# Infinidat/slimfastq

Measured on AMD Instinct MI355X. Metric: MB/s FASTQ compressed, higher is better.
Workload: dtype u8/u32 integer; 1 GPU; synthetic 10M x 150 bp Illumina reads per GPU, full qlts+gens+recs, frozen tables (one chain per lane), -l 3; level=3, block_reads=1024, prior_step=-1, blocks_per_gpu=9766, tables=frozen, chains_per_gpu=253906, raw_bytes_per_gpu=3702038404, parallelism=1 GPU

## Files before the change

slimfastq_amd/csrc/api.cpp:

```cpp
#include <hip/hip_runtime.h>

#include <algorithm>
#include <cstdarg>
#include <cstdlib>
#include <cstdio>
#include <cstring>
#include <string>
#include <vector>
#include <chrono>
#include <functional>
#include <future>
#include <thread>
#include <atomic>
#include <mutex>
#include <condition_variable>

#include "kernels.h"

namespace {

struct HostTimes {
    bool on; std::chrono::steady_clock::time_point t0; std::vector<std::pair<const char*, double>> marks;
    HostTimes() : on(getenv("SFQ_HOST_TIMING") != nullptr), t0(std::chrono::steady_clock::now()) {}
    void mark(const char* what) { if (on) marks.push_back({ what, std::chrono::duration<double, std::milli>(std::chrono::steady_clock::now() - t0).count() }); }
    ~HostTimes() { if (on) { for (auto& m : marks) fprintf(stderr, "  [host] %-28s %8.3f ms\n", m.first, m.second); } }
};
struct DevBuf {
    void*  p = nullptr;
    size_t cap = 0;
};

struct Tables {
    DevBuf q_slots, q_hdr, p_slots, p_hdr, g_tab;
    u32 slots = 0;
    u32 q_rows = 0;
    u32 g_bits = 0;
};

}

struct HostWorker {
    std::thread th; std::mutex mu; std::condition_variable cv;
    std::function<int()> job; bool has_job = false, done = true, quit = false; int result = 0;
    void loop() {
        std::unique_lock<std::mutex> lk(mu);
        for (;;) {
            cv.wait(lk, [&] { return has_job || quit; });
            if (quit) return;
            std::function<int()> j = std::move(job); has_job = false;
            lk.unlock();
            int r;
            try { r = j(); }
            catch (const std::bad_alloc&) { r = SFQ_E_NOMEM; }
            catch (...) { r = SFQ_E_CORRUPT; }
            lk.lock();
            result = r; done = true;
            cv.notify_all();
        }
    }
    void submit(std::function<int()> j) {
        std::unique_lock<std::mutex> lk(mu);
        if (!th.joinable()) th = std::thread([this] { loop(); });
        job = std::move(j); has_job = true; done = false;
        cv.notify_all();
    }
    bool busy() { std::unique_lock<std::mutex> lk(mu); return !done; }
    int wait() { std::unique_lock<std::mutex> lk(mu); cv.wait(lk, [&] { return done; }); return result; }
    ~HostWorker() {
        { std::unique_lock<std::mutex> lk(mu); cv.wait(lk, [&] { return done; }); quit = true; cv.notify_all(); }
        if (th.joinable()) th.join();
    }
};
enum {
    EE_BEGIN,
    EE_HEAD_END,
    EE_M0_BEGIN, EE_M0_END, EE_M1_BEGIN, EE_M1_END, EE_M2_BEGIN, EE_M2_END, EE_M3_BEGIN, EE_M3_END,
    EE_PACK_BEGIN, EE_PACK_END,
    EE_FRAME_K_BEGIN,
    EE_TEXT_FORK,
    EE_QLT_CODE_BEGIN, EE_QLT_CODE_END,
    EE_GEN_CODE_BEGIN, EE_GEN_CODE_END,
    EE_REC_CODE_BEGIN,
    EE_NEVER_READ,
    EE_QLT_LIST_HOME,
    EE_QLT_ROWS_BUILT,
    EE_LINES_INDEXED,
    EE_FRAME_K_END,
    EE_REC_FREQS_HOME,
    EE_REC_CODE_END,
    EE_COUNT
};
enum {
    ED_BEGIN,
    ED_HEAD_END,
    ED_FORK,
    ED_QLT_END,
    ED_GEN_END,
    ED_REC_END,
    ED_END,
    ED_GEN_BEGIN,
    ED_OVER_FORK,
    ED_OVER_LINES_END,
    ED_LISTS_COPIED,
    ED_COUNT
};
enum { EV_COUNT = EE_COUNT > ED_COUNT ? (int)EE_COUNT : (int)ED_COUNT };
enum { CRC_EV_FORK, CRC_EV_DONE, CRC_EV_COUNT };
struct sfq_ctx {
    int dev = 0;
    HostWorker worker;
    hipStream_t st = nullptr;
    hipStream_t st_aux[3] = {nullptr, nullptr, nullptr};
    hipEvent_t ev[EV_COUNT] = {};
    bool rec_copy_pending = false;
    bool rec_blob_pending = false;
    std::string err;
    u64 table_budget = 0;
    u64 dev_total = 0;
    u32 wave_slots = 8192;
    u32 epoch_base = 0;
    Tables tab;
    DevBuf chunk_base, scan_tmp, line_off, status, blocks, arena, blk_stream_off, stream_total,
           lens, blob_off, blob, in_stage, out_stage;
    DevBuf slen, qlen, pfg, pfq, soff, qoff, seq_stage, qual_stage, hdr_stage, hlen, hoff, hso, hsc, rsize, roff, d_first;
    DevBuf hist, rows66, ptmp, prior_w, prior_wovf, prior_ls, prior_lh, tickets;
    DevBuf gm_T, gm_slen, gm_boff, gm_soff, gm_scan, gm_stage, gm_tok, gm_csz, gm_idx;
    DevBuf qrows, qdec, qesc, qw, csz, coff, gcnt, grows, glog, gcost, gbins, gfill, hcnt, hfreq, rrows, rdec, rmap, rflags, rtok, excf, cflags;
    DevBuf chn_len, chn_off, chn_out;
    DevBuf pslot, plist;
    DevBuf segn, segoff, segrec;
    DevBuf oflags, okbytes, ofpos, okoff, ofilt, orecmap, olist, line_off_o, ono, opiece, otxt[3], osize_all, oroff_all, oroff_k, ocnt;
    u32 r_hot = 0, r_hot_dec = 0;
    bool blobs_from_encode = false;
    bool unsettled = false;
    bool counts_only = false; u32 sample_scale = 1;
    struct { const u8* ptr = nullptr; u64 nbytes = 0, nrec = 0, print = 0; bool marks = false, valid = false; } framed;
    struct { bool valid = false, rec = false; u32 q_rows = 0; } counts;
    void* pin = nullptr; size_t pin_cap = 0;
    void* pin2 = nullptr; size_t pin2_cap = 0;
    std::vector<u8> chain_blob;
    std::vector<u8> rec_prior_blob;
    std::vector<u8> chain_tmp;
    bool prior_on = false;
    std::vector<u8> prior_blob;
    std::vector<sfq_block_info> index;
    std::vector<u8> first_hdrs;
    bool crc_on = false;
    hipStream_t st_crc = nullptr;
    hipEvent_t crc_ev[CRC_EV_COUNT] = {};
    DevBuf crc_tab, crc_tiles, crc_grps, crc_bounds, crc_out;
    void* crc_pin = nullptr; size_t crc_pin_cap = 0;
    std::vector<u32> crcs; u32 text_crc = 0;
    std::vector<u32> crc_expect; bool crc_expect_set = false;
};

namespace {

int fail(sfq_ctx* c, int code, const char* fmt, ...) {
    char b[512];
    va_list ap; va_start(ap, fmt); vsnprintf(b, sizeof b, fmt, ap); va_end(ap);
    if (c) c->err = b;
    return code;
}
#define HIPC(call) do { hipError_t e_ = (call); if (e_ != hipSuccess) \
    return fail(ctx, e_ == hipErrorOutOfMemory ? SFQ_E_NOMEM : SFQ_E_HIP, "%s: %s", #call, hipGetErrorString(e_)); } while (0)

int reserve(sfq_ctx* ctx, DevBuf& b, size_t bytes, bool zero_new = false) {
    if (bytes <= b.cap && b.p) return SFQ_OK;
    if (b.p) { HIPC(hipStreamSynchronize(ctx->st)); HIPC(hipFree(b.p)); b.p = nullptr; b.cap = 0; }
    size_t want = bytes < 256 ? 256 : bytes;
    HIPC(hipMalloc(&b.p, want));
    b.cap = want;
    if (zero_new) HIPC(hipMemsetAsync(b.p, 0, want, ctx->st));
    return SFQ_OK;
}
void release(DevBuf& b) { if (b.p) { (void)hipDeviceSynchronize(); (void)hipFree(b.p); } b.p = nullptr; b.cap = 0; }

int level_gen_bits(int level) {
    switch (level) { case 1: return 18; case 2: return 22; case 3: return 24; default: return 26; }
}
int clamp_level(int level) { return level > 4 ? 4 : level < 1 ? 1 : level; }

int reserve_pinned_buf(sfq_ctx* ctx, void*& p, size_t& cap, size_t bytes) {
    if (bytes <= cap && p) return SFQ_OK;
    if (p) { HIPC(hipDeviceSynchronize()); HIPC(hipHostFree(p)); p = nullptr; cap = 0; }
    bytes += bytes / 4;
    HIPC(hipHostMalloc(&p, bytes, hipHostMallocDefault));
    cap = bytes;
    return SFQ_OK;
}
int reserve_pinned(sfq_ctx* ctx, size_t bytes) { return reserve_pinned_buf(ctx, ctx->pin, ctx->pin_cap, bytes); }

int ensure_tables(sfq_ctx* ctx, u32 want, u32 q_rows, u32 g_bits, u32 models, u32* got) {
    const u64 per_q = (models & SFQ_M_QLT) ? (u64)q_rows * (L64_NSYM * 4 + sizeof(RowHdr)) : 0;
    const u64 per_p = (u64)PR_ROWS * (PW_NSYM * 4 + sizeof(RowHdr));
    const u64 per_g = (models & SFQ_M_GEN) ? ((u64)4 << g_bits) : 0;
    const u64 per = per_q + per_p + per_g;
    u64 fit = ctx->table_budget / per;
    if (fit == 0) return fail(ctx, SFQ_E_NOMEM, "table budget %llu B too small for one block slot (%llu B)",
                              (unsigned long long)ctx->table_budget, (unsigned long long)per);
    const u32 cap = 12288;
    u32 slots = (u32)std::min<u64>(std::min<u64>(want, fit), cap);
    Tables& t = ctx->tab;
    int rc;
    if (per_q) {
        const size_t need_s = (size_t)slots * q_rows * L64_NSYM * 4, need_h = (size_t)slots * q_rows * sizeof(RowHdr);
        if ((rc = reserve(ctx, t.q_slots, need_s, true))) return rc;
        if (need_h > t.q_hdr.cap || !t.q_hdr.p) { release(t.q_hdr); if ((rc = reserve(ctx, t.q_hdr, need_h, true))) return rc; }
        t.q_rows = q_rows;
    }
    {
        const size_t need_s = (size_t)slots * PR_ROWS * PW_NSYM * 4, need_h = (size_t)slots * PR_ROWS * sizeof(RowHdr);
        if ((rc = reserve(ctx, t.p_slots, need_s))) return rc;
        if (need_h > t.p_hdr.cap || !t.p_hdr.p) { release(t.p_hdr); if ((rc = reserve(ctx, t.p_hdr, need_h, true))) return rc; }
    }
    if (per_g) { if ((rc = reserve(ctx, t.g_tab, (size_t)slots * per_g))) return rc; t.g_bits = g_bits; }
    t.slots = slots;
    *got = slots;
    return SFQ_OK;
}

void fill_model_args(sfq_ctx* ctx, ModelArgs& a, u32 nblocks, int level, u32 g_bits, bool lossless) {
    memset(&a, 0, sizeof a);
    Tables& t = ctx->tab;
    a.line_off = (const u64*)ctx->line_off.p;
    a.blocks = (BlockDesc*)ctx->blocks.p;
    a.nblocks = nblocks;
    a.arena = (u8*)ctx->arena.p;
    a.level = level;
    a.lossless = lossless ? 1u : 0u;
    a.epoch_base = ctx->epoch_base;
    ctx->epoch_base += nblocks;
    a.q_slots = (u32*)t.q_slots.p; a.q_hdr = (RowHdr*)t.q_hdr.p; a.q_rows = t.q_rows;
    a.p_slots = (u32*)t.p_slots.p; a.p_hdr = (RowHdr*)t.p_hdr.p;
    a.g_tab = (u32*)t.g_tab.p; a.g_bits = g_bits;
    if (ctx->prior_on) {
        a.prior_w = (const u32*)ctx->prior_w.p; a.prior_wovf = (const u32*)ctx->prior_wovf.p;
        a.prior_ls = (const u32*)ctx->prior_ls.p; a.prior_lh = (const RowHdr*)ctx->prior_lh.p;
    }
}

int advance_epoch(sfq_ctx* ctx, u32 nblocks) {
    if ((u64)ctx->epoch_base + nblocks + 2 >= 0x3FFFFFFFull) {
        Tables& t = ctx->tab;
        if (t.q_slots.p) HIPC(hipMemsetAsync(t.q_slots.p, 0, t.q_slots.cap, ctx->st));
        if (t.q_hdr.p) HIPC(hipMemsetAsync(t.q_hdr.p, 0, t.q_hdr.cap, ctx->st));
        if (t.p_hdr.p) HIPC(hipMemsetAsync(t.p_hdr.p, 0, t.p_hdr.cap, ctx->st));
        ctx->epoch_base = 0;
    }
    return SFQ_OK;
}

void put_v(std::vector<u8>& o, u64 v) { while (v >= 0x80) { o.push_back((u8)(v | 0x80)); v >>= 7; } o.push_back((u8)v); }
bool get_v(const u8* b, size_t n, size_t& p, u64& v) {
    v = 0;
    for (int sh = 0; sh < 64; sh += 7) { if (p >= n) return false; u8 c = b[p++]; v |= (u64)(c & 0x7f) << sh; if (!(c & 0x80)) return true; }
    return false;
}
bool read_sizes(const u8* b, size_t nb, size_t& p, bool deltas, u32* out, size_t n) {
    u64 prev = 0;
    size_t i = 0;
    while (i < n) {
        if (deltas && p + 8 <= nb && n - i >= 8) {
            u64 w; memcpy(&w, b + p, 8);
            if (!(w & 0x8080808080808080ull)) {
                for (int j = 0; j < 8; j++) {
                    const u32 x = (u32)(w >> (8 * j)) & 0x7fu;
                    const i64 v = (i64)prev + ((i64)(x >> 1) ^ -(i64)(x & 1));
                    if (v < 0 || v > 0xFFFFFFFFll) return false;
                    prev = (u64)v; out[i + j] = (u32)v;
                }
                p += 8; i += 8;
                continue;
            }
        }
        u64 raw;
        if (p < nb && b[p] < 0x80u) raw = b[p++];
        else if (p + 1 < nb && b[p + 1] < 0x80u) { raw = (u64)(b[p] & 0x7fu) | ((u64)b[p + 1] << 7); p += 2; }
        else if (!get_v(b, nb, p, raw)) return false;
        if (deltas) {
            if (raw > 0x1FFFFFFFFull) return false;
            const i64 v = (i64)prev + ((i64)(raw >> 1) ^ -(i64)(raw & 1));
            if (v < 0 || v > 0xFFFFFFFFll) return false;
            raw = (u64)v;
        }
        if (raw > 0xFFFFFFFFull) return false;
        prev = raw; out[i++] = (u32)raw;
    }
    return true;
}
#define PRIOR_LIST_ROW 67u
#define PRIOR_LIST_HEAD 4u
#define PRIOR_LIST_EAGER 16384u
std::vector<u8> pack_prior(const u32* list, u32 q_rows) {
    const u32 n = list[0];
    std::vector<u8> o((size_t)n * (5 + 2 + 64 * 4) + 16);
    u8* w = o.data();
    auto put = [&](u64 v) { while (v >= 0x80) { *w++ = (u8)(v | 0x80); v >>= 7; } *w++ = (u8)v; };
    put(q_rows);
    u32 prev = 0;
    for (u32 i = 0; i < n; i++) {
        const u32* r = list + PRIOR_LIST_HEAD + (size_t)i * PRIOR_LIST_ROW;
        const u32 c = r[0], iend = r[66];
        r++;
        u32 nnz = 0;
        while (nnz < iend && (r[nnz] & 0xffff)) nnz++;
        put(c - prev + 1); prev = c;
        *w++ = (u8)iend; *w++ = (u8)nnz;
        for (u32 j = 0; j < nnz; j++) { *w++ = (u8)(r[j] >> 16); put(r[j] & 0xffff); }
    }
    put(0);
    o.resize((size_t)(w - o.data()));
    return o;
}
bool unpack_prior(const u8* b, size_t n, u32 q_rows, std::vector<u32>& ctxs, std::vector<u32>& rows) {
    size_t p = 0; u64 v;
    if (!get_v(b, n, p, v) || v != q_rows) return false;
    ctxs.clear(); rows.clear();
    u64 c = 0; bool first = true;
    for (;;) {
        if (!get_v(b, n, p, v)) return false;
        if (v == 0) break;
        if (!first && v == 1) return false;
        c = first ? v - 1 : c + v - 1; first = false;
        if (c >= q_rows || p + 2 > n) return false;
        ctxs.push_back((u32)c);
        rows.resize(rows.size() + 66, 0);
        u32* r = rows.data() + rows.size() - 66;
        const u32 iend = b[p++], nnz = b[p++];
        if (iend > 64 || nnz > iend) return false;
        bool used[64] = {false};
        u32 total = 0;
        for (u32 j = 0; j < nnz; j++) {
            if (p >= n) return false;
            const u32 sym = b[p++];
            if (sym >= iend || used[sym] || !get_v(b, n, p, v) || v > 0xffff) return false;
            used[sym] = true; r[j] = (u32)v | (sym << 16); total += (u32)v;
        }
        u32 j = nnz;
        for (u32 s = 0; s < iend; s++) if (!used[s]) r[j++] = s << 16;
        r[64] = total; r[65] = iend;
    }
    return true;
}
int ensure_prior_buffers(sfq_ctx* ctx, u32 q_rows) {
    int rc;
    if ((rc = reserve(ctx, ctx->hist, (size_t)q_rows * 64 * 4))) return rc;
    if ((rc = reserve(ctx, ctx->rows66, (size_t)q_rows * 66 * 4))) return rc;
    if ((rc = reserve(ctx, ctx->prior_w, (size_t)q_rows * 64 * 4))) return rc;
    if ((rc = reserve(ctx, ctx->prior_wovf, (size_t)q_rows * 4 * 4))) return rc;
    if ((rc = reserve(ctx, ctx->prior_ls, (size_t)q_rows * 64 * 4))) return rc;
    if ((rc = reserve(ctx, ctx->prior_lh, (size_t)q_rows * sizeof(RowHdr)))) return rc;
    return SFQ_OK;
}

int upload_prior(sfq_ctx* ctx, u32 q_rows, hipStream_t st, bool spread = true) {
    std::vector<u32> ctxs, rows;
    if (!unpack_prior(ctx->prior_blob.data(), ctx->prior_blob.size(), q_rows, ctxs, rows)) return fail(ctx, SFQ_E_CORRUPT, "bad quality prior (qlt.pri)");
    int rc;
    if ((rc = ensure_prior_buffers(ctx, q_rows))) return rc;
    HIPC(hipMemsetAsync(ctx->rows66.p, 0, (size_t)q_rows * 66 * 4, st));
    if (!ctxs.empty()) {
        if ((rc = reserve(ctx, ctx->ptmp, (ctxs.size() + rows.size()) * 4))) return rc;
        u32* d_ctx = (u32*)ctx->ptmp.p; u32* d_rows = d_ctx + ctxs.size();
        HIPC(hipMemcpyAsync(d_ctx, ctxs.data(), ctxs.size() * 4, hipMemcpyHostToDevice, st));
        HIPC(hipMemcpyAsync(d_rows, rows.data(), rows.size() * 4, hipMemcpyHostToDevice, st));
        launch_prior_scatter(d_ctx, d_rows, (u32)ctxs.size(), (u32*)ctx->rows66.p, st);
    }
    if (spread) launch_prior_spread((const u32*)ctx->rows66.p, q_rows, (u32*)ctx->prior_w.p, (u32*)ctx->prior_wovf.p, (u32*)ctx->prior_ls.p, (RowHdr*)ctx->prior_lh.p, st);
    HIPC(hipStreamSynchronize(st));
    return SFQ_OK;
}

std::vector<u8> pack_rec_prior_f(const u32* f) {
    std::vector<u8> o;
    put_v(o, PR_REC_ROWS);
    u32 prev = 0;
    for (u32 r = 0; r < PR_REC_ROWS; r++) {
        const u32* fr = f + (size_t)r * 256;
        u32 nnz = 0;
        for (u32 s = 0; s < 256; s++) nnz += fr[s] != 0;
        if (!nnz) continue;
        put_v(o, r - prev + 1); prev = r;
        put_v(o, nnz);
        for (u32 s = 0; s < 256; s++) if (fr[s]) { o.push_back((u8)s); put_v(o, fr[s]); }
    }
    put_v(o, 0);
    return o;
}
bool unpack_rec_prior(const u8* b, size_t n, std::vector<u32>& f) {
    size_t p = 0; u64 v;
    if (!get_v(b, n, p, v) || v != PR_REC_ROWS) return false;
// ... 501 lines not shown
    HIPC(hipEventRecord(ctx->ev[EE_BEGIN], st));
    if ((rc = reserve(ctx, ctx->status, 256))) return rc;
    const u32 q_rows0 = p.level == 1 ? (1u << 12) : (1u << 16);
    bool hist_cleared = false;
    if (p.block_reads && (models & SFQ_M_QLT) && (p.prior_step || p.tables == SFQ_TABLES_FROZEN) && p.kernel == 0 && p.prior_step != SFQ_PRIOR_COUNTS) {
        if ((rc = ensure_prior_buffers(ctx, q_rows0))) return rc;
        HIPC(hipMemsetAsync(ctx->hist.p, 0, (size_t)q_rows0 * 64 * 4, st));
        hist_cleared = true;
    }
    const bool legacy = p.block_reads == 0;
    const bool want_marks = p.tables == SFQ_TABLES_FROZEN && p.block_reads != 0 && p.kernel == 0 && (models & SFQ_M_GEN) && (!priors_only || ctx->counts_only);
    u64 nrec = 0;
    hipStream_t vst = legacy ? st : ctx->st_aux[0];
    auto frame = [&]() -> int {
        int rc;
        const u32 tiles = frame_tiles(nbytes);
        if ((rc = reserve(ctx, ctx->chunk_base, (size_t)tiles * 8))) return rc;
        if ((rc = reserve(ctx, ctx->scan_tmp, ((size_t)(nbytes / 16384) / 1024 + 4) * 8 + 65536))) return rc;
        u64 cap = std::max<u64>(ctx->line_off.cap / 8 > 2 ? ctx->line_off.cap / 8 - 2 : 0, nbytes / 64 + 1024);
        u64 nlines = 0;
        for (int attempt = 0; ; attempt++) {
            if ((rc = reserve(ctx, ctx->line_off, (size_t)(cap + 2) * 8))) return rc;
            const u64 ecap = cap / 4 + 2;
            if (want_marks) {
                if ((rc = reserve(ctx, ctx->excf, (size_t)ecap))) return rc;
                HIPC(hipMemsetAsync(ctx->excf.p, 0, (size_t)ecap, st));
            }
            HIPC(hipMemsetAsync(ctx->status.p, 0, 256, st));
            HIPC(hipMemsetAsync(ctx->chunk_base.p, 0, (size_t)tiles * 8, st));
            void* d_fo = (u8*)ctx->status.p + 224;
            HIPC(hipEventRecord(ctx->ev[EE_FRAME_K_BEGIN], st));
            launch_frame(d_fastq, nbytes, (u64*)ctx->chunk_base.p, (u64*)ctx->line_off.p, cap, (u32*)ctx->status.p, want_marks ? (u8*)ctx->excf.p : nullptr, ecap, d_fo, st);
            HIPC(hipEventRecord(ctx->ev[EE_FRAME_K_END], st));
            struct { u64 nlines; u32 tripped, pad; } fo = {0, 0, 0};
            u8 last_byte = 0;
            HIPC(hipMemcpyAsync(&fo, d_fo, 16, hipMemcpyDeviceToHost, st));
            HIPC(hipMemcpyAsync(&last_byte, d_fastq + nbytes - 1, 1, hipMemcpyDeviceToHost, st));
            HIPC(hipStreamSynchronize(st));
            if (fo.tripped) return fail(ctx, SFQ_E_HIP, "framing: a tile waited in vain for the tiles before it");
            if (last_byte != '\n') return fail(ctx, SFQ_E_FORMAT, "fastq file: record seems truncated (no final newline)");
            nlines = fo.nlines;
            if (nlines <= cap) break;
            if (attempt) return fail(ctx, SFQ_E_HIP, "framing: %llu lines after a pass that counted fewer", (unsigned long long)nlines);
            cap = nlines;
        }
        if (nlines == 0 || (nlines & 3)) return fail(ctx, SFQ_E_FORMAT, "fastq file: %llu lines is not a multiple of 4", (unsigned long long)nlines);
        nrec = nlines / 4;
        if (nrec >= 3000000000ULL) return fail(ctx, SFQ_E_UNSUPPORTED, "more than 3e9 records (usrs.cpp:394)");
        if (vst != st) { HIPC(hipEventRecord(ctx->ev[EE_LINES_INDEXED], st)); HIPC(hipStreamWaitEvent(vst, ctx->ev[EE_LINES_INDEXED], 0)); }
        launch_validate_lines((const u64*)ctx->line_off.p, nrec, legacy ? 0x3ffffffeu : 0x1ffeu, 0x3ffffffeu, (u32*)ctx->status.p, vst);
        return SFQ_OK;
    };
    bool reframe = !(p.prior_step == SFQ_PRIOR_COUNTS && !legacy && ctx->framed.valid && ctx->framed.ptr == d_fastq && ctx->framed.nbytes == nbytes &&
                     (!want_marks || ctx->framed.marks));
    if (!reframe) {
        u64 print = 0;
        if ((rc = text_fingerprint(ctx, d_fastq, nbytes, st, &print))) return rc;
        if (print != ctx->framed.print) reframe = true;
    }
    ctx->framed.valid = false;
    if (!reframe) nrec = ctx->framed.nrec;
    else if ((rc = frame())) return rc;
    u64 nrec_file = nrec;
    u32 n_over = 0;
    const u8* d_file = d_fastq;
    if (legacy) {
        u32 h4[4] = {0, 0, 0, 0};
        HIPC(hipMemcpyAsync(h4, ctx->status.p, 16, hipMemcpyDeviceToHost, st));
        HIPC(hipStreamSynchronize(st));
        if (h4[0] == 0 && h4[3] != 0) {
            if (nrec > 0xFFFFFFF0ull) return fail(ctx, SFQ_E_UNSUPPORTED, "oversize records in a file of more than 2^32 records");
            u32* d_first = (u32*)ctx->status.p + 8; u32* d_solid = d_first + 1; u32* d_bad = d_first + 2;
            u32 init3[3] = { 0xFFFFFFFFu, 0, 0 };
            HIPC(hipMemcpyAsync(d_first, init3, 12, hipMemcpyHostToDevice, st));
            launch_over_first((const u64*)ctx->line_off.p, nrec, d_first, st);
            u32 first = 0;
            HIPC(hipMemcpyAsync(&first, d_first, 4, hipMemcpyDeviceToHost, st));
            HIPC(hipStreamSynchronize(st));
            if (first == 0xFFFFFFFFu) return fail(ctx, SFQ_E_UNSUPPORTED, "every record is over the reference's line limits (usrs.cpp:190-197: \"all records were oversized\")");
            launch_over_solid(d_fastq, (const u64*)ctx->line_off.p, first, d_solid, st);
            u32 solid = 0;
            HIPC(hipMemcpyAsync(&solid, d_solid, 4, hipMemcpyDeviceToHost, st));
            HIPC(hipStreamSynchronize(st));
            if ((rc = reserve(ctx, ctx->oflags, (size_t)nrec * 4))) return rc;
            if ((rc = reserve(ctx, ctx->okbytes, (size_t)nrec * 4))) return rc;
            if ((rc = reserve(ctx, ctx->ofpos, ((size_t)nrec + 1) * 8))) return rc;
            if ((rc = reserve(ctx, ctx->okoff, ((size_t)nrec + 1) * 8))) return rc;
            if ((rc = reserve(ctx, ctx->scan_tmp, ((size_t)nrec / 1024 + 4) * 8 + 65536))) return rc;
            launch_over_flags((const u64*)ctx->line_off.p, nrec, solid, (u32*)ctx->oflags.p, (u32*)ctx->okbytes.p, d_bad, st);
            launch_scan_u32((const u32*)ctx->oflags.p, (u64*)ctx->ofpos.p, nrec, (u64*)ctx->scan_tmp.p, st);
            launch_scan_u32((const u32*)ctx->okbytes.p, (u64*)ctx->okoff.p, nrec, (u64*)ctx->scan_tmp.p, st);
            u64 h_nover = 0, h_kbytes = 0; u32 h_bad = 0, first_flag = 0;
            HIPC(hipMemcpyAsync(&h_nover, (u64*)ctx->ofpos.p + nrec, 8, hipMemcpyDeviceToHost, st));
            HIPC(hipMemcpyAsync(&h_kbytes, (u64*)ctx->okoff.p + nrec, 8, hipMemcpyDeviceToHost, st));
            HIPC(hipMemcpyAsync(&h_bad, d_bad, 4, hipMemcpyDeviceToHost, st));
            HIPC(hipMemcpyAsync(&first_flag, (u32*)ctx->oflags.p + first, 4, hipMemcpyDeviceToHost, st));
            HIPC(hipStreamSynchronize(st));
            if (h_bad) return fail(ctx, SFQ_E_UNSUPPORTED, "a quality line over 65534 bytes beside a base line within the limit: the reference's own archive of such a record does not decode (usrs.cpp:340-345 run before 372-373)");
            if (first_flag) return fail(ctx, SFQ_E_UNSUPPORTED, "the first record within determine_record's limits (usrs.cpp:218-229) is oversize for get_record (usrs.cpp:333-338): a base line of exactly 65535 bytes");
            if (h_nover == nrec) return fail(ctx, SFQ_E_UNSUPPORTED, "every record is over the reference's line limits");
            if (h_nover) {
                n_over = (u32)h_nover;
                if ((rc = reserve(ctx, ctx->ofilt, (size_t)h_kbytes + 16))) return rc;
                if ((rc = reserve(ctx, ctx->orecmap, (size_t)(nrec - h_nover) * 4 + 16))) return rc;
                if ((rc = reserve(ctx, ctx->olist, (size_t)h_nover * 4 + 16))) return rc;
                launch_over_split(d_fastq, (const u64*)ctx->line_off.p, nrec, (const u32*)ctx->oflags.p, (const u64*)ctx->ofpos.p, (const u64*)ctx->okoff.p,
                                  (u8*)ctx->ofilt.p, (u32*)ctx->orecmap.p, (u32*)ctx->olist.p, st);
                std::swap(ctx->line_off, ctx->line_off_o);
                d_fastq = (const u8*)ctx->ofilt.p; nbytes = h_kbytes;
                if ((rc = frame())) return rc;
                if (nrec + h_nover != nrec_file) return fail(ctx, SFQ_E_HIP, "oversize split: %llu + %llu records of %llu", (unsigned long long)nrec, (unsigned long long)h_nover, (unsigned long long)nrec_file);
            }
        }
    }

    if (p.block_reads == SFQ_BLOCK_AUTO) {
        const u64 r = std::max<u64>(1, (376ull << 10) / std::max<u64>(1, nbytes / nrec));
        p.block_reads = (u32)std::min<u64>(r >= 64 ? (r & ~63ull) : r, 4096);
    }
    const u32 block_reads = p.block_reads ? p.block_reads : (u32)std::min<u64>(nrec, 0xFFFFFFFFu);
    const u64 nblocks64 = (nrec + block_reads - 1) / block_reads;
    if (nblocks64 > (1u << 24)) return fail(ctx, SFQ_E_ARG, "too many blocks (%llu)", (unsigned long long)nblocks64);
    const u32 nblocks = (u32)nblocks64;
    const bool frozen = p.tables == SFQ_TABLES_FROZEN && p.block_reads != 0 && p.kernel == 0;
    int g_bits = p.gen_bits ? p.gen_bits : level_gen_bits(p.level);
    if (!p.gen_bits && p.block_reads) {
        const double bases = (frozen ? (double)nrec : (double)block_reads) * ((double)nbytes / (double)nrec) * 0.5;
        int cap = 12;
        while (cap < 26 && (double)(1u << cap) < bases) cap += 2;
        g_bits = std::min(g_bits, cap);
    }
    if (g_bits < 2 || g_bits > 26 ) return fail(ctx, SFQ_E_ARG, "gen_bits %d out of range", g_bits);
    if ((rc = reserve(ctx, ctx->blocks, (size_t)nblocks * sizeof(BlockDesc)))) return rc;
    launch_block_prepare(d_fastq, (const u64*)ctx->line_off.p, nrec, block_reads, (BlockDesc*)ctx->blocks.p, nblocks, nbytes, p.level, g_bits, st);
    const bool crc_pass = ctx->crc_on && !priors_only;
    if (crc_pass) {
        if ((rc = crc_reserve(ctx, d_fastq_in, 0, nbytes_in, nblocks))) return rc;
        HIPC(hipEventRecord(ctx->crc_ev[CRC_EV_FORK], st));
        HIPC(hipStreamWaitEvent(ctx->st_crc, ctx->crc_ev[CRC_EV_FORK], 0));
        launch_crc_block_bounds((const u64*)ctx->line_off.p, 4ull * block_reads, nblocks, nbytes_in, (u64*)ctx->crc_bounds.p, ctx->st_crc);
        if ((rc = crc_queue(ctx, d_fastq_in, nbytes_in, nblocks, ctx->st_crc))) return rc;
        HIPC(hipEventRecord(ctx->crc_ev[CRC_EV_DONE], ctx->st_crc));
    }
    const u64 arena_main = (((u64)nbytes * 17 / 2 + (u64)nblocks * 1024 + 4096) + 15) & ~15ull;
    const u64 over_bytes = n_over ? nbytes_in - nbytes : 0;
    const u64 over_cap = n_over ? ((over_bytes + over_bytes / 4 + 4096 + 15) & ~15ull) : 0;
    if (over_cap > 0xFFFFFFF0ull) return fail(ctx, SFQ_E_UNSUPPORTED, "more than 3.4 GB of oversize records");
    if ((rc = reserve(ctx, ctx->arena, (size_t)(arena_main + 3 * over_cap)))) return rc;
    const u32 q_rows = p.level == 1 ? (1u << 12) : (1u << 16);
    ctx->prior_on = false;
    u32 prior_step = p.block_reads ? p.prior_step : 0;
    const bool given = prior_step == SFQ_PRIOR_GIVEN;
    const bool counted = prior_step == SFQ_PRIOR_COUNTS;
    if (counted) {
        const bool need_rec = frozen && (models & SFQ_M_REC);
        if (!ctx->counts.valid || !ctx->hist.p || (need_rec && !ctx->hcnt.p))
            return fail(ctx, SFQ_E_ARG, "SFQ_PRIOR_COUNTS: no counts installed (sfq_set_prior_counts / sfq_count_priors come first; any other encode drops them)");
        if (ctx->counts.q_rows != q_rows) return fail(ctx, SFQ_E_ARG, "SFQ_PRIOR_COUNTS: the counts were installed for %u quality contexts, level %d has %u", ctx->counts.q_rows, p.level, q_rows);
        if (need_rec && !ctx->counts.rec) return fail(ctx, SFQ_E_ARG, "SFQ_PRIOR_COUNTS: the installed counts hold no header sample (they were counted for adaptive tables), frozen tables need one");
    }
    if (given && ctx->prior_blob.empty()) return fail(ctx, SFQ_E_ARG, "SFQ_PRIOR_GIVEN: no quality prior installed (sfq_set_qlt_prior)");
    if (given && frozen && (models & SFQ_M_REC) && ctx->rec_prior_blob.empty()) return fail(ctx, SFQ_E_ARG, "SFQ_PRIOR_GIVEN: no header prior installed (sfq_set_rec_prior)");
    if (!given) { ctx->prior_blob.clear(); ctx->rec_prior_blob.clear(); }
    ctx->rec_blob_pending = false; ctx->rec_copy_pending = false;
    ctx->chain_blob.clear();
    if (frozen && !prior_step) prior_step = SFQ_PRIOR_AUTO;
    u32 slots = 0;
    const u32 KR = 2;
    const u32 nblocks_r = (nblocks + KR - 1) / KR * KR;
    ModelArgs a;
    u32* tickets = nullptr;
    auto setup_tables = [&]() -> int {
        int rc;
        if ((rc = ensure_tables(ctx, nblocks_r, q_rows, (u32)g_bits, frozen ? (models & ~(SFQ_M_QLT | SFQ_M_GEN)) : models, &slots))) return rc;
        if (p.kernel == 0) {
            if (slots < KR) return fail(ctx, SFQ_E_NOMEM, "table budget %llu B holds %u block slot(s); the kernels need %u", (unsigned long long)ctx->table_budget, slots, KR);
            slots &= ~(KR - 1);
        }
        if ((rc = advance_epoch(ctx, nblocks))) return rc;
        fill_model_args(ctx, a, nblocks, p.level, (u32)g_bits, p.block_reads != 0);
        a.fq = d_fastq;
        a.rec_map = n_over ? (const u32*)ctx->orecmap.p : nullptr;
        if ((rc = reserve(ctx, ctx->tickets, 64))) return rc;
        HIPC(hipMemsetAsync(ctx->tickets.p, 0, 64, st));
        tickets = (u32*)ctx->tickets.p;
        return SFQ_OK;
    };
    const u32 order[4] = { SFQ_M_QLT, frozen ? SFQ_M_REC : SFQ_M_GEN, SFQ_M_USR, frozen ? SFQ_M_GEN : SFQ_M_REC };
    const int tslot[4] = { SFQ_T_QLT, frozen ? SFQ_T_REC : SFQ_T_GEN, SFQ_T_USR, frozen ? SFQ_T_GEN : SFQ_T_REC };
    hipStream_t mst[4] = { st, ctx->st_aux[0], ctx->st_aux[1], ctx->st_aux[2] };
    if (prior_step == SFQ_PRIOR_AUTO || (ctx->counts_only && prior_step == 0)) {
        const u64 per_rec = std::min<u64>(std::max<u64>(1, nbytes / nrec / 2), PRIOR_SYMBOLS);
        prior_step = (u32)std::min<u64>(std::max<u64>(1, nrec * per_rec / 24000000ull), 0x7FFFFFFFull);
        if (nbytes / nrec <= 4000) prior_step = (u32)std::max<u64>(prior_step, (nrec + 131071) / 131072);
    }
    if (ctx->counts_only && prior_step && prior_step < SFQ_PRIOR_COUNTS)
        prior_step = (u32)std::min<u64>((u64)prior_step * std::max<u32>(1u, ctx->sample_scale), 0x7FFFFFFFull);
    bool hist_launched = false;
    if (frozen && !given && !counted && prior_step && (models & SFQ_M_QLT)) {
        if ((rc = ensure_prior_buffers(ctx, q_rows))) return rc;
        if (!hist_cleared) { HIPC(hipMemsetAsync(ctx->hist.p, 0, (size_t)q_rows * 64 * 4, st)); hist_cleared = true; }
        launch_qlt_hist(d_fastq, nbytes, (const u64*)ctx->line_off.p, (const BlockDesc*)ctx->blocks.p, block_reads, nrec, prior_step, p.level, PRIOR_SYMBOLS, (u32*)ctx->hist.p, st);
        hist_launched = true;
    }
    u32 h_status2[5] = {0, 0, 0, 0, 0};
    HIPC(hipMemcpyAsync(h_status2, ctx->status.p, 20, hipMemcpyDeviceToHost, vst));
    HIPC(hipEventRecord(ctx->ev[EE_HEAD_END], st));
    if (vst != st) HIPC(hipStreamSynchronize(vst));
    else HIPC(hipStreamSynchronize(st));
    const u32 h_status = h_status2[0], max_hdr = h_status2[1], max_line = h_status2[2], min_hdr = ~h_status2[4];
    if (h_status == (u32)(-SFQ_E_FORMAT)) return fail(ctx, SFQ_E_FORMAT, "fastq file: expecting '@' / '+' line prefixes (usrs.cpp:162-167)");
    if (h_status) return fail(ctx, -(int)h_status, "record over the line limits: headers up to 8190 bytes; base and quality lines up to 65534 in format 6 (-B 0; the reference would write oversize side streams, usrs.cpp:269-301, which this library does not), up to 1 Gi in the block format; or an empty base line");

    ChainArgs ca;
    memset(&ca, 0, sizeof ca);
    u32 nchains = 0, nsub = 0;
    GenPlan gplan; GmPlan gmplan;
    ChainGeoArgs ggeo; memset(&ggeo, 0, sizeof ggeo);
    const u32* gen_csz = nullptr;
    const bool flat_quads_req = getenv("SFQ_FLAT_QUADS") != nullptr;
    const bool gm = frozen && !exc_classic;
    u32 seg_len = 0;
    std::vector<u32> seg_blk;
    if (frozen) {
        u32 cr = p.chain_reads ? p.chain_reads : (u32)default_chain_reads(nrec, nbytes);
        if (p.chain_reads & SFQ_CHAIN_SEGMENT_FLAG) { seg_len = p.chain_reads & ~SFQ_CHAIN_SEGMENT_FLAG; cr = 1; if (!seg_len) return fail(ctx, SFQ_E_ARG, "SFQ_CHAIN_SEGMENT(0)"); }
        else if (!p.chain_reads && cr == 1 && nrec < 204800) {
            const u64 segs_want = SFQ_CHAINS_WANT - 8192 - std::min<u64>(nrec / 2, 100000);
            const u64 want = std::min<u64>(std::max<u64>(4096, nbytes / 2 / segs_want), 1u << 20);
            if (max_line > want) seg_len = (u32)want;
        }
        if (!p.chain_reads && !seg_len)
            while (cr < block_reads && (u64)nblocks * ((block_reads + cr - 1) / cr) > SFQ_CHAINS_WANT) cr++;
        ca.geo.chain_reads = (u32)std::min<u64>(std::min(cr, block_reads), nrec);
        ca.geo.cpb = (block_reads + ca.geo.chain_reads - 1) / ca.geo.chain_reads;
        if (!p.chain_reads) ca.geo.chain_reads = std::max<u32>(1u, (u32)((std::min<u64>(block_reads, nrec) + ca.geo.cpb - 1) / ca.geo.cpb));
        const u32 last_nrec = (u32)(nrec - (u64)(nblocks - 1) * block_reads);
        const u64 nc = (u64)(nblocks - 1) * ca.geo.cpb + (last_nrec + ca.geo.chain_reads - 1) / ca.geo.chain_reads;
        if (nc > 0x7FFFFFFFull) return fail(ctx, SFQ_E_ARG, "too many chains (%llu)", (unsigned long long)nc);
        nchains = ca.geo.nchains = (u32)nc;
        ca.nbytes = nbytes; ca.block_reads = block_reads;
        if (seg_len) {
            if ((rc = reserve(ctx, ctx->segn, (size_t)nrec * 4))) return rc;
            if ((rc = reserve(ctx, ctx->segoff, ((size_t)nrec + 1) * 8))) return rc;
            if ((rc = reserve(ctx, ctx->scan_tmp, ((size_t)nrec / 1024 + 4) * 8 + 65536))) return rc;
            launch_seg_count((const u64*)ctx->line_off.p, (const BlockDesc*)ctx->blocks.p, block_reads, nrec, seg_len, (u32*)ctx->segn.p, st);
            launch_scan_u32((const u32*)ctx->segn.p, (u64*)ctx->segoff.p, nrec, (u64*)ctx->scan_tmp.p, st);
            std::vector<u64> h_off((size_t)nrec + 1);
            HIPC(hipMemcpyAsync(h_off.data(), ctx->segoff.p, ((size_t)nrec + 1) * 8, hipMemcpyDeviceToHost, st));
            HIPC(hipStreamSynchronize(st));
            if (h_off[nrec] > 0x7FFFFFFFull) return fail(ctx, SFQ_E_ARG, "too many chains (%llu segments)", (unsigned long long)h_off[nrec]);
            nchains = ca.geo.nchains = (u32)h_off[nrec];
            seg_blk.resize(nblocks);
            for (u32 b = 0; b < nblocks; b++) seg_blk[b] = (u32)(h_off[std::min<u64>((u64)(b + 1) * block_reads, nrec)] - h_off[(u64)b * block_reads]);
            if ((rc = reserve(ctx, ctx->segrec, (size_t)nchains * 4 + 16))) return rc;
            launch_seg_fill((const u64*)ctx->segoff.p, nrec, (u32*)ctx->segrec.p, st);
            ca.seg_len = seg_len; ca.seg_off = (const u64*)ctx->segoff.p; ca.seg_rec = (const u32*)ctx->segrec.p;
        }
        {
            const u32 cpb_want = std::max<u32>(1u, 61440u / nblocks);
            const u32 rfloor = nbytes / nrec > 4000 ? 16u : 128u;
            const u32 rcr0 = std::max<u32>(rfloor, (block_reads + cpb_want - 1) / cpb_want);
            const u32 rcr = (u32)std::min<u64>(std::min<u32>(std::max<u32>(rcr0, ca.geo.chain_reads), block_reads), nrec);
            ca.rgeo.chain_reads = rcr;
            ca.rgeo.cpb = (block_reads + rcr - 1) / rcr;
            nsub = ca.rgeo.nchains = (u32)((u64)(nblocks - 1) * ca.rgeo.cpb + (last_nrec + rcr - 1) / rcr);
        }
        if ((rc = reserve(ctx, ctx->csz, ((size_t)nchains * 2 + (size_t)nsub * 2) * 4))) return rc;
        HIPC(hipMemsetAsync(ctx->csz.p, 0, ((size_t)nchains * 2 + (size_t)nsub * 2) * 4, st));
        ggeo = ca.geo;
        if (gm && !seg_len) {
            const u64 per_rec = std::max<u64>(1, nbytes / std::max<u64>(1, nrec));
            const u64 gwant = std::max<u64>((GM_CHAIN_FLOOR + per_rec - 1) / per_rec, (nrec + GM_CHAIN_WANT - 1) / GM_CHAIN_WANT);
            const u32 gfloor = (u32)std::min<u64>(gwant, ca.geo.chain_reads);
            ggeo.cpb = (block_reads + gfloor - 1) / gfloor;
            ggeo.chain_reads = std::max<u32>(1u, (u32)((std::min<u64>(block_reads, nrec) + ggeo.cpb - 1) / ggeo.cpb));
            ggeo.cpb = (block_reads + ggeo.chain_reads - 1) / ggeo.chain_reads;
            const u64 ngc = (u64)(nblocks - 1) * ggeo.cpb + (last_nrec + ggeo.chain_reads - 1) / ggeo.chain_reads;
            if (ngc > 0x7FFFFFFFull || ggeo.chain_reads >= ca.geo.chain_reads) ggeo = ca.geo;
            else {
                ggeo.nchains = (u32)ngc;
                if ((rc = reserve(ctx, ctx->gm_csz, (size_t)ggeo.nchains * 4))) return rc;
                HIPC(hipMemsetAsync(ctx->gm_csz.p, 0, (size_t)ggeo.nchains * 4, st));
            }
        }
        if ((rc = reserve_pinned(ctx, PIN_BYTES + (size_t)q_rows * 66 * 4))) return rc;
        if ((rc = setup_tables())) return rc;
        HIPC(hipEventRecord(ctx->ev[EE_TEXT_FORK], st));
        if (!priors_only) {
            for (int m = 1; m < 4; m++) { HIPC(hipStreamWaitEvent(mst[m], ctx->ev[EE_TEXT_FORK], 0)); HIPC(hipEventRecord(ev_model_begin(ctx, m), mst[m])); }
            a.batch0 = 0; a.nbatch = std::min(slots, nblocks_r);
            ca.m = a;
            if (models & SFQ_M_REC) { if ((rc = rec_prior_begin(ctx, a, nrec, given, counted, mst[1], max_hdr))) return rc; }
            if (models & SFQ_M_GEN) {
                if (gm) { if ((rc = gm_begin(ctx, ca, nblocks, nrec, max_line, mst[3], gmplan))) return rc; }
                else if ((rc = gen_tables_begin(ctx, ca, nblocks, (u32)g_bits, max_line, mst[3], gplan))) return rc;
            }
        } else if (models & SFQ_M_REC) {
            HIPC(hipStreamWaitEvent(mst[1], ctx->ev[EE_TEXT_FORK], 0));
            if ((rc = rec_prior_begin(ctx, a, nrec, given, counted, mst[1], max_hdr))) return rc;
        }
    }
    u32* h_rows66 = nullptr;
    if (given && (models & SFQ_M_QLT)) {
        if ((rc = ensure_prior_buffers(ctx, q_rows))) return rc;
        if (!hist_cleared) HIPC(hipMemsetAsync(ctx->hist.p, 0, (size_t)q_rows * 64 * 4, st));
        if ((rc = upload_prior(ctx, q_rows, st, !frozen))) return rc;
        HIPC(hipEventRecord(ctx->ev[EE_HEAD_END], st));
        ctx->prior_on = true;
    } else if (prior_step && (models & SFQ_M_QLT)) {
        if ((rc = ensure_prior_buffers(ctx, q_rows))) return rc;
        if (!counted && !hist_launched) {
            if (!hist_cleared) HIPC(hipMemsetAsync(ctx->hist.p, 0, (size_t)q_rows * 64 * 4, st));
            launch_qlt_hist(d_fastq, nbytes, (const u64*)ctx->line_off.p, (const BlockDesc*)ctx->blocks.p, block_reads, nrec, prior_step, p.level, PRIOR_SYMBOLS, (u32*)ctx->hist.p, st);
        }
        if (ctx->counts_only) {
            HIPC(hipStreamSynchronize(mst[1]));
            HIPC(hipStreamSynchronize(st));
            res->n_records = nrec; res->n_blocks = nblocks;
            ctx->counts.valid = true; ctx->counts.q_rows = q_rows; ctx->counts.rec = frozen && (models & SFQ_M_REC);
            if (!legacy && !n_over) {
                u64 print = 0;
                if ((rc = text_fingerprint(ctx, d_fastq, nbytes, st, &print))) return rc;
                ctx->framed.ptr = d_fastq; ctx->framed.nbytes = nbytes; ctx->framed.nrec = nrec; ctx->framed.marks = want_marks; ctx->framed.print = print; ctx->framed.valid = true;
            }
            return SFQ_OK;
        }

        launch_prior_rows((const u32*)ctx->hist.p, q_rows, (u32*)ctx->rows66.p, (u32*)ctx->prior_w.p, (u32*)ctx->prior_wovf.p,
                          (u32*)ctx->prior_ls.p, (RowHdr*)ctx->prior_lh.p, st);
        if ((rc = reserve(ctx, ctx->pslot, (size_t)q_rows * 4))) return rc;
        if ((rc = reserve(ctx, ctx->plist, ((size_t)PRIOR_LIST_HEAD + (size_t)q_rows * PRIOR_LIST_ROW) * 4))) return rc;
        if ((rc = reserve_pinned(ctx, PIN_BYTES + ((size_t)PRIOR_LIST_HEAD + (size_t)q_rows * PRIOR_LIST_ROW) * 4))) return rc;
        h_rows66 = (u32*)((u8*)ctx->pin + PIN_BYTES);
        HIPC(hipEventRecord(ctx->ev[EE_QLT_ROWS_BUILT], st));
        HIPC(hipStreamWaitEvent(mst[2], ctx->ev[EE_QLT_ROWS_BUILT], 0));
        launch_prior_list((const u32*)ctx->rows66.p, q_rows, (u32*)ctx->pslot.p, (u32*)ctx->plist.p, mst[2]);
        HIPC(hipMemcpyAsync(h_rows66, ctx->plist.p, ((size_t)PRIOR_LIST_HEAD + (size_t)std::min<u32>(q_rows, PRIOR_LIST_EAGER) * PRIOR_LIST_ROW) * 4, hipMemcpyDeviceToHost, mst[2]));
        HIPC(hipEventRecord(ctx->ev[EE_QLT_LIST_HOME], mst[2]));
        HIPC(hipEventRecord(ctx->ev[EE_HEAD_END], st));
        ctx->prior_on = true;
    }
    if (frozen) {
        if (models & SFQ_M_QLT) {
            if ((rc = reserve(ctx, ctx->qrows, (size_t)q_rows * 64 * 4))) return rc;
            if ((rc = build_qesc(ctx, st))) return rc;
            launch_qlt_frozen_rows((const u32*)ctx->rows66.p, q_rows, (u32*)ctx->qrows.p, nullptr, st);
            ca.qrows = (const u32*)ctx->qrows.p; ca.qesc = (const u32*)ctx->qesc.p;
            ca.q_hot = 0; ca.q_rows = q_rows;
            const u32 want_hot = (p.lds_rows == SFQ_LDS_ROWS_NONE || given || !prior_step) ? 0u : p.lds_rows ? std::min<u32>(p.lds_rows, 1024u)
                                 : nchains >= 150000u ? 800u : 0u;
            if (want_hot) {
                const size_t img_bytes = (size_t)q_rows / 4 + (size_t)want_hot * 100 + 64;
                if ((rc = reserve(ctx, ctx->qw, img_bytes + (size_t)q_rows * 4 + 256))) return rc;
                u8* img = (u8*)ctx->qw.p; u32* info = (u32*)(img + ((img_bytes + 15) & ~(size_t)15)); u32* ctot = info + 16;
                launch_hot_rows((const u32*)ctx->hist.p, (const u32*)ctx->rows66.p, (const u32*)ctx->qrows.p, q_rows, want_hot, ctot, img, info, st);
                ca.q_hot = want_hot; ca.qh_img = img; ca.qh_info = info;
            }
            HIPC(hipEventRecord(ctx->ev[EE_HEAD_END], st));
        }
    }
    if (!frozen) { if ((rc = setup_tables())) return rc; }
    if (priors_only) {
        if (ctx->prior_on && !given) {
            if ((rc = qlt_prior_blob_now(ctx, h_rows66, q_rows, st))) return rc;
        }
        if (frozen && (models & SFQ_M_REC)) { if ((rc = rec_prior_finish(ctx, given, mst[1]))) return rc; if ((rc = rec_prior_copy_back(ctx, mst[1]))) return rc; if ((rc = rec_prior_blob_now(ctx))) return rc; }
        HIPC(hipStreamSynchronize(mst[1]));
        HIPC(hipStreamSynchronize(st));
        ctx->prior_on = false;
        res->n_records = nrec; res->n_blocks = nblocks;
        return SFQ_OK;
    }
    u32 gen_on = 0;
    const bool exc_rice = frozen && !exc_classic;
    if (frozen) {
        a.batch0 = 0; a.nbatch = std::min(slots, nblocks_r);
        HIPC(hipEventRecord(ev_model_begin(ctx, 0), st));
        if (models & SFQ_M_REC) {
            if ((rc = rec_prior_finish(ctx, given, mst[1]))) return rc;
            ca.m = a; ca.rrows = (const u32*)ctx->rrows.p; ca.rdec = (const u16*)ctx->rdec.p;
            ca.rmap = (const u16*)ctx->rmap.p; ca.rhot = ca.rmap + PR_REC_ROWS; ca.r_hot = ctx->r_hot;
            if ((rc = reserve(ctx, ctx->rflags, (size_t)nsub * 4 * 3))) return rc;
            if ((rc = reserve(ctx, ctx->rtok, rec_token_bytes(nrec)))) return rc;
            HIPC(hipMemsetAsync(ctx->rflags.p, 0, (size_t)nsub * 4 * 2, mst[1]));
            ca.csz = (u32*)ctx->csz.p + 2 * (size_t)nchains; ca.rhb = ca.csz + nsub;
            HIPC(hipEventRecord(ctx->ev[EE_REC_CODE_BEGIN], mst[1]));
            if (nbytes / nrec <= 4000) HIPC(hipStreamWaitEvent(st, ctx->ev[EE_REC_CODE_BEGIN], 0));
            launch_rec_encode_c(ca, (u32*)ctx->rflags.p, (u32*)ctx->rflags.p + nsub, (u32*)ctx->rtok.p, (u32*)ctx->rflags.p + 2 * (size_t)nsub, ctx->r_hot_dec, max_hdr, mst[1], min_hdr, min_hdr > 127 ? nullptr : ctx->ev[EE_REC_CODE_END]);
            HIPC(hipEventRecord(min_hdr > 127 ? ctx->ev[EE_REC_CODE_END] : ctx->ev[EE_NEVER_READ], mst[1]));
            HIPC(hipEventRecord(ev_model_end(ctx, 1), mst[1]));
            if ((rc = rec_prior_copy_back(ctx, mst[1]))) return rc;
        } else HIPC(hipEventRecord(ev_model_end(ctx, 1), mst[1]));
        if (models & SFQ_M_GEN) {
            ca.m = a; ca.csz = (u32*)ctx->csz.p + nchains;
            if (gm) {
                gmplan.ggeo = ggeo; gmplan.gcsz = ggeo.nchains != ca.geo.nchains ? (u32*)ctx->gm_csz.p : nullptr;
                if ((rc = gm_finish(ctx, ca, nrec, max_line, mst[3], gmplan, &gen_on))) return rc;
                if (!gen_on) ggeo = ca.geo;
            }
            else if ((rc = gen_tables_finish(ctx, ca, (u32)g_bits, max_line, mst[3], gplan, &gen_on))) return rc;
            gen_csz = (gm && gen_on && ggeo.nchains != ca.geo.nchains) ? (const u32*)ctx->gm_csz.p : (const u32*)ctx->csz.p + nchains;
            HIPC(hipEventRecord(ctx->ev[EE_GEN_CODE_BEGIN], mst[3]));
            if (gm && gen_on) launch_gm_code(gmplan.cg, (const u8*)ctx->gm_tok.p, mst[3]);
            else { ca.flat_quads = (gm && !gen_on && flat_quads_req) ? 1u : 0u; ca.flat_raw = (gm && !gen_on && !flat_quads_req) ? 1u : 0u; launch_gen_encode_c(ca, mst[3], 0, 0, !gen_on); }
            HIPC(hipEventRecord(ctx->ev[EE_GEN_CODE_END], mst[3]));
        }
        HIPC(hipEventRecord(ev_model_end(ctx, 3), mst[3]));
        if (models & SFQ_M_QLT) {
            ca.m = a; ca.csz = (u32*)ctx->csz.p;
            HIPC(hipEventRecord(ctx->ev[EE_QLT_CODE_BEGIN], st)); launch_qlt_encode_c(ca, st); HIPC(hipEventRecord(ctx->ev[EE_QLT_CODE_END], st));
        }
        HIPC(hipEventRecord(ev_model_end(ctx, 0), st));
        if (models & SFQ_M_GEN) {
            if (exc_rice) launch_gen_exc_r(a, want_marks ? (const u8*)ctx->excf.p : nullptr, tickets + 1, mst[2]);
            else launch_gen_exc_w(a, want_marks ? (const u8*)ctx->excf.p : nullptr, tickets + 1, mst[2]);
        }
        if (models & SFQ_M_USR)
            for (u32 b0 = 0; b0 < nblocks; b0 += slots) { ModelArgs ua = a; ua.batch0 = b0; ua.nbatch = std::min(slots, nblocks - b0); launch_usr_encode_w(ua, mst[2]); }
        HIPC(hipEventRecord(ev_model_end(ctx, 2), mst[2]));
        HIPC(hipStreamWaitEvent(st, ev_model_end(ctx, 1), 0));
        HIPC(hipStreamWaitEvent(st, ev_model_end(ctx, 3), 0));
        HIPC(hipStreamWaitEvent(st, ev_model_end(ctx, 2), 0));
    } else {
    if ((models & SFQ_M_GEN) && p.kernel == 1)
        launch_fill_u32((u32*)ctx->tab.g_tab.p, (u64)std::min(slots, nblocks) << g_bits, 0x03030303u, st);
    HIPC(hipEventRecord(ctx->ev[EE_HEAD_END], st));
    for (int m = 0; m < 4; m++) {
        if (m) HIPC(hipStreamWaitEvent(mst[m], ctx->ev[EE_HEAD_END], 0));
        HIPC(hipEventRecord(ev_model_begin(ctx, m), mst[m]));
        if (models & order[m]) {
            const bool batched = p.kernel == 1 || order[m] == SFQ_M_USR;
            if (!batched) {
                a.batch0 = 0; a.nbatch = std::min(slots, nblocks_r);
                if ((models & (SFQ_M_QLT | SFQ_M_GEN | SFQ_M_REC)) == (SFQ_M_QLT | SFQ_M_GEN | SFQ_M_REC) &&
                    (order[m] == SFQ_M_QLT || order[m] == SFQ_M_GEN))
                {
                    const u32 pct = order[m] == SFQ_M_GEN ? ADAPT_GEN_PCT : ADAPT_QLT_PCT;
                    a.nbatch = std::min<u32>(a.nbatch, std::max<u32>(KR, ((u32)((u64)ctx->wave_slots * pct / 100) * KR) & ~(KR - 1)));
                }
                switch (order[m]) {
                case SFQ_M_QLT: launch_qlt_encode_k(a, tickets + 0, mst[m]); break;
                case SFQ_M_GEN: launch_gen_encode_k(a, tickets + 1, mst[m]); break;
                case SFQ_M_REC: launch_rec_encode_w(a, tickets + 2, tickets + 3, mst[m]); break;
                }
            } else {
                for (u32 b0 = 0; b0 < nblocks; b0 += slots) {
                    a.batch0 = b0; a.nbatch = std::min(slots, nblocks - b0);
                    switch (order[m]) {
                    case SFQ_M_QLT: launch_qlt_encode_l(a, mst[m]); break;
                    case SFQ_M_GEN:
                        if (b0) launch_fill_u32((u32*)ctx->tab.g_tab.p, (u64)a.nbatch << g_bits, 0x03030303u, mst[m]);
                        launch_gen_encode_l(a, mst[m]);
                        break;
                    case SFQ_M_REC: launch_rec_encode_l(a, mst[m]); break;
                    case SFQ_M_USR: if (p.kernel == 1) launch_usr_encode_l(a, mst[m]); else launch_usr_encode_w(a, mst[m]); break;
                    }
                }
            }
        }
        if (order[m] == SFQ_M_USR && n_over) {
            const u64 ooff[3] = { arena_main, arena_main + over_cap, arena_main + 2 * over_cap };
            const u32 ocap[3] = { (u32)over_cap, (u32)over_cap, (u32)over_cap };
            launch_over_encode_w(a, d_file, (const u64*)ctx->line_off_o.p, (const u32*)ctx->olist.p, n_over, ooff, ocap, mst[m]);
        }
        HIPC(hipEventRecord(ev_model_end(ctx, m), mst[m]));
        if (m) HIPC(hipStreamWaitEvent(st, ev_model_end(ctx, m), 0));
    }
    }
    ht.mark("chains queued");
    HIPC(hipEventRecord(ctx->ev[EE_PACK_BEGIN], st));

    if ((rc = reserve(ctx, ctx->blk_stream_off, (size_t)nblocks * SFQ_NSTREAMS * 8))) return rc;
    if ((rc = reserve(ctx, ctx->stream_total, 2 * SFQ_NSTREAMS * 8 + 64))) return rc;
    u32 chain_streams = 0;
    if (frozen) {
        ca.m = a;
        if (models & SFQ_M_QLT) { launch_chain_block_sizes(ca, ca.geo, SFQ_S_QLT, (const u32*)ctx->csz.p, nullptr, st); chain_streams |= 1u << SFQ_S_QLT; }
        if (models & SFQ_M_GEN) { launch_chain_block_sizes(ca, ggeo, SFQ_S_GEN, gen_csz, nullptr, st); chain_streams |= 1u << SFQ_S_GEN; }
        if (models & SFQ_M_REC) {
            const u32* rs = (const u32*)ctx->csz.p + 2 * (size_t)nchains;
            launch_chain_block_sizes(ca, ca.rgeo, SFQ_S_REC, rs, rs + nsub, st); chain_streams |= 1u << SFQ_S_REC;
        }
    }
    launch_block_stream_offsets((BlockDesc*)ctx->blocks.p, nblocks, (u64*)ctx->blk_stream_off.p, (u64*)ctx->stream_total.p, st);
    if ((rc = reserve(ctx, ctx->lens, (size_t)nblocks * 4))) return rc;
    if ((rc = reserve(ctx, ctx->blob_off, ((size_t)nblocks + 1) * 8))) return rc;
    const u64 blob_cap = std::min<u64>(nbytes, (u64)nblocks * SFQ_MAX_ID_LLEN);
    if ((rc = reserve(ctx, ctx->blob, blob_cap))) return rc;
    launch_first_hdr_lens((const BlockDesc*)ctx->blocks.p, nblocks, (u32*)ctx->lens.p, st);
    launch_scan_u32((const u32*)ctx->lens.p, (u64*)ctx->blob_off.p, nblocks, (u64*)ctx->scan_tmp.p, st);
    launch_gather_first_hdrs((const BlockDesc*)ctx->blocks.p, nblocks, d_fastq, (const u64*)ctx->blob_off.p, (u8*)ctx->blob.p, blob_cap, st);
    const size_t p2_hb = 128, p2_off = p2_hb + (((size_t)nblocks * sizeof(BlockDesc) + 63) & ~(size_t)63);
    const size_t p2_csz = p2_off + ((((size_t)nblocks + 1) * 8 + 63) & ~(size_t)63);
    const u32 ngc = frozen ? ggeo.nchains : 0;
    const bool gsplit = frozen && ngc != nchains;
    const size_t n_sizes = (size_t)nchains + ngc + (size_t)nsub * 2;
    const u32* d_sizes = (const u32*)ctx->csz.p;
    if (gsplit) {
        if ((rc = reserve(ctx, ctx->gm_idx, n_sizes * 4 + 64))) return rc;
        u32* di = (u32*)ctx->gm_idx.p;
        HIPC(hipMemcpyAsync(di, ctx->csz.p, (size_t)nchains * 4, hipMemcpyDeviceToDevice, st));
        HIPC(hipMemcpyAsync(di + nchains, ctx->gm_csz.p, (size_t)ngc * 4, hipMemcpyDeviceToDevice, st));
        HIPC(hipMemcpyAsync(di + nchains + ngc, (const u32*)ctx->csz.p + 2 * (size_t)nchains, (size_t)nsub * 2 * 4, hipMemcpyDeviceToDevice, st));
        d_sizes = di;
    }
    const size_t p2_end = p2_csz + n_sizes * 4 + 64;
    if ((rc = reserve_pinned_buf(ctx, ctx->pin2, ctx->pin2_cap, p2_end))) return rc;
    u64* totals = (u64*)ctx->pin2;
    HIPC(hipMemcpyAsync(totals, ctx->stream_total.p, SFQ_NSTREAMS * 8, hipMemcpyDeviceToHost, st));
    auto pack_prior_now = [&]() -> int {
        if (ctx->prior_on && !given && h_rows66) {
            if ((rc = qlt_prior_blob_now(ctx, h_rows66, q_rows, mst[2]))) return rc;
            h_rows66 = nullptr;
        }
        return rec_prior_blob_now(ctx);
    };
    BlockDesc* hb = (BlockDesc*)((u8*)ctx->pin2 + p2_hb);
    u64* hboff = (u64*)((u8*)ctx->pin2 + p2_off);
    u32* h_csz = (u32*)((u8*)ctx->pin2 + p2_csz);
    const bool rec_chains = (chain_streams >> SFQ_S_REC) & 1;
    const u32 chn_n = frozen ? nchains + ngc + (rec_chains ? nsub * 2 : 0u) : 0u;
    const size_t chn_eager = std::min<size_t>((size_t)chn_n * 5, n_sizes * 4 + 64 - 16);
    u32* d_gate = (u32*)((u64*)ctx->stream_total.p + 2 * SFQ_NSTREAMS);
    const u64 blob_guess = std::min<u64>(blob_cap, (u64)nblocks * 256);
    launch_stream_gate((const BlockDesc*)ctx->blocks.p, nblocks, (const u64*)ctx->stream_total.p, out_cap, (u64*)ctx->stream_total.p + SFQ_NSTREAMS, d_gate, st);
    launch_compact((const BlockDesc*)ctx->blocks.p, nblocks, (const u8*)ctx->arena.p, (const u64*)ctx->blk_stream_off.p,
                   (const u64*)ctx->stream_total.p + SFQ_NSTREAMS, d_out, chain_streams, st, d_gate);
    if (frozen) {
        if (chain_streams & (1u << SFQ_S_QLT))
            launch_compact_chains(ca, ca.geo, SFQ_S_QLT, 2, 1, (const u32*)ctx->csz.p, (const u64*)ctx->blk_stream_off.p, (const u64*)ctx->stream_total.p + SFQ_NSTREAMS, d_out, st, d_gate);
        if (chain_streams & (1u << SFQ_S_GEN))
            launch_compact_chains(ca, ggeo, SFQ_S_GEN, 3, 4, gen_csz, (const u64*)ctx->blk_stream_off.p, (const u64*)ctx->stream_total.p + SFQ_NSTREAMS, d_out, st, d_gate);
        if (chain_streams & (1u << SFQ_S_REC))
            launch_compact_chains(ca, ca.rgeo, SFQ_S_REC, 3, 2, (const u32*)ctx->csz.p + 2 * (size_t)nchains, (const u64*)ctx->blk_stream_off.p, (const u64*)ctx->stream_total.p + SFQ_NSTREAMS, d_out, st, d_gate);
        {
            const u32 b1 = nchains, b2 = nchains + ngc, b3 = rec_chains ? nchains + ngc + nsub : chn_n;
            if ((rc = reserve(ctx, ctx->chn_len, (size_t)chn_n * 4 + 16))) return rc;
            if ((rc = reserve(ctx, ctx->chn_off, ((size_t)chn_n + 4) * 8))) return rc;
            if ((rc = reserve(ctx, ctx->chn_out, (size_t)chn_n * 5 + 64))) return rc;
            if ((rc = reserve(ctx, ctx->scan_tmp, ((size_t)chn_n / 1024 + 4) * 8 + 65536))) return rc;
            u64* d_info = (u64*)ctx->chn_off.p + chn_n + 1;
            launch_chain_index_bytes(d_sizes, chn_n, b1, b2 > chn_n ? chn_n : b2, b3, (u32*)ctx->chn_len.p, (u64*)ctx->chn_off.p, (u64*)ctx->scan_tmp.p,
                                     (u8*)ctx->chn_out.p, d_info, st);
            HIPC(hipMemcpyAsync(h_csz, d_info, 16, hipMemcpyDeviceToHost, st));
            if (chn_eager) HIPC(hipMemcpyAsync((u8*)h_csz + 16, ctx->chn_out.p, chn_eager, hipMemcpyDeviceToHost, st));
        }
    }
    HIPC(hipEventRecord(ctx->ev[EE_PACK_END], st));
    if ((rc = pack_prior_now())) return rc;
    ctx->first_hdrs.resize((size_t)blob_guess);
    if (blob_guess) HIPC(hipMemcpyAsync(ctx->first_hdrs.data(), ctx->blob.p, (size_t)blob_guess, hipMemcpyDeviceToHost, st));
    HIPC(hipMemcpyAsync(hb, ctx->blocks.p, (size_t)nblocks * sizeof(BlockDesc), hipMemcpyDeviceToHost, st));
    HIPC(hipMemcpyAsync(hboff, ctx->blob_off.p, ((size_t)nblocks + 1) * 8, hipMemcpyDeviceToHost, st));
    ht.mark("packing queued");
    if ((rc = pack_prior_now())) return rc;
    ht.mark("priors packed");
    HIPC(hipStreamSynchronize(st));
    ht.mark("device through");
    u64 bases[SFQ_NSTREAMS], run = 0;
    for (int s = 0; s < SFQ_NSTREAMS; s++) { bases[s] = run; run += totals[s]; res->stream_bytes[s] = totals[s]; res->stream_offset[s] = bases[s]; }
    res->total_bytes = run;
    int worst = 0;
    for (u32 b = 0; b < nblocks; b++) if (hb[b].status) worst = std::max<int>(worst, (int)hb[b].status);
    if (worst) return fail(ctx, -worst, "block kernel reported error %d (%s)", -worst,
                           -worst == SFQ_E_OVERFLOW ? "stream arena too small" : -worst == SFQ_E_GENCHAR ? "unexpected genome char / switched N byte" :
                           -worst == SFQ_E_UNSUPPORTED ? "a '+' line that is neither empty nor its record's header: the block format refuses what it could not give back (usrs.cpp:236-239)" : "see status codes");
    ht.mark("  statuses looked at");
    if (run > out_cap) return fail(ctx, SFQ_E_OVERFLOW, "output needs %llu bytes, caller gave %llu", (unsigned long long)run, (unsigned long long)out_cap);
    if (hboff[nblocks] > blob_cap) return fail(ctx, SFQ_E_OVERFLOW, "first-header blob overflow");
    if (hboff[nblocks] > blob_guess) {
        ctx->first_hdrs.resize((size_t)hboff[nblocks]);
        HIPC(hipMemcpyAsync(ctx->first_hdrs.data() + blob_guess, (const u8*)ctx->blob.p + blob_guess, (size_t)(hboff[nblocks] - blob_guess), hipMemcpyDeviceToHost, st));
        HIPC(hipStreamSynchronize(st));
    } else ctx->first_hdrs.resize((size_t)hboff[nblocks]);

    ht.mark("  first headers home");
    ctx->prior_on = false;
    ctx->chain_blob.clear();
    if (frozen) {
        std::vector<u8>& o = ctx->chain_tmp;
        const size_t o_need = ((size_t)nchains + ngc + (size_t)nsub * 2 + (seg_len ? nblocks : 0)) * 5 + 64;
        if (o.size() < o_need) o.resize(o_need);
        u8* w = o.data();
        auto put = [&w](u32 v) { while (v >= 0x80) { *w++ = (u8)(v | 0x80); v >>= 7; } *w++ = (u8)v; };
        put(ca.geo.chain_reads);
        put((gen_on ? CHN_GEN_ON : 0u) | (rec_chains ? CHN_REC_CHAINS : 0u) | CHN_DELTAS | (seg_len ? CHN_SEGMENTS : 0u) | (exc_rice ? CHN_EXC_RICE : 0u) | ((gm && gen_on) ? CHN_GEN_MATCH : 0u)
            | ((gm && !gen_on) ? (flat_quads_req ? CHN_FLAT_QUADS : CHN_FLAT_RAW) : 0u));
        if (gm && gen_on) { put(gmplan.tb); put(ggeo.chain_reads); put(ngc); }
        put(nchains);
        if (seg_len) { put(seg_len); for (u32 b = 0; b < nblocks; b++) put(seg_blk[b]); }
        const u64* info = (const u64*)h_csz;
        const u8* lb = (const u8*)h_csz + 16;
        const u64 la = info[0], lall = info[1];
        if (la > lall || lall > (u64)chn_n * 5) return fail(ctx, SFQ_E_HIP, "chain index: %llu / %llu bytes of lists for %u sizes", (unsigned long long)la, (unsigned long long)lall, chn_n);
        std::vector<u8> rest;
        if (lall > chn_eager) {
            rest.resize((size_t)lall);
            HIPC(hipMemcpyAsync(rest.data(), ctx->chn_out.p, (size_t)lall, hipMemcpyDeviceToHost, st));
            HIPC(hipStreamSynchronize(st));
            lb = rest.data();
        }
        if (o.size() < o_need + (size_t)lall) { const size_t used = (size_t)(w - o.data()); o.resize(o_need + (size_t)lall); w = o.data() + used; }
        memcpy(w, lb, (size_t)la); w += la;
        if (rec_chains) { put(ca.rgeo.chain_reads); put(nsub); memcpy(w, lb + la, (size_t)(lall - la)); w += lall - la; }
        ctx->chain_blob.assign(o.data(), w);
    }
    ht.mark("chain index written");
    res->n_chains = nchains;
    ctx->index.resize(nblocks);
    for (u32 b = 0; b < nblocks; b++) {
        sfq_block_info& bi = ctx->index[b];
        const BlockDesc& d = hb[b];
        memset(&bi, 0, sizeof bi);
        bi.first_record = d.rec0; bi.n_records = n_over ? (u32)nrec_file : d.nrec; bi.llen = d.llen;
        bi.solid = d.solid; bi.two_id = d.two_id; bi.n_byte = (u8)d.n_byte; bi.gen_bits = d.gen_bits;
        bi.extra_hi = d.extra_hi; bi.first_hdr_len = d.first_hdr_len; bi.first_hdr_off = hboff[b];
        for (int s = 0; s < SFQ_NSTREAMS; s++) bi.size[s] = d.size[s];
        bi.status = 0; bi.hdr_bytes = d.hdr_bytes;
    }
    res->n_records = nrec_file; res->n_blocks = nblocks; res->first_hdr_bytes = hboff[nblocks];
    res->kernel_ms[SFQ_T_FRAME] = ev_ms(ctx->ev[EE_BEGIN], ctx->ev[EE_HEAD_END]);
    for (int m = 0; m < 4; m++) res->kernel_ms[tslot[m]] = ev_ms(ev_model_begin(ctx, m), ev_model_end(ctx, m));
    res->kernel_ms[SFQ_T_PACK] = ev_ms(ctx->ev[EE_PACK_BEGIN], ctx->ev[EE_PACK_END]);
    res->kernel_ms[SFQ_T_TOTAL] = ev_ms(ctx->ev[EE_BEGIN], ctx->ev[EE_PACK_END]);
    if (reframe) res->coder_ms[3] = ev_ms(ctx->ev[EE_FRAME_K_BEGIN], ctx->ev[EE_FRAME_K_END]);
    ht.mark("block index built");
    if (frozen) {
        if (models & SFQ_M_QLT) res->coder_ms[0] = ev_ms(ctx->ev[EE_QLT_CODE_BEGIN], ctx->ev[EE_QLT_CODE_END]);
        if (models & SFQ_M_GEN) res->coder_ms[1] = ev_ms(ctx->ev[EE_GEN_CODE_BEGIN], ctx->ev[EE_GEN_CODE_END]);
        if (models & SFQ_M_REC) res->coder_ms[2] = ev_ms(ctx->ev[EE_REC_CODE_BEGIN], ctx->ev[EE_REC_CODE_END]);
    } else {
        res->coder_ms[0] = res->kernel_ms[SFQ_T_QLT]; res->coder_ms[1] = res->kernel_ms[SFQ_T_GEN]; res->coder_ms[2] = res->kernel_ms[SFQ_T_REC];
    }
    if (crc_pass) {
        HIPC(hipEventSynchronize(ctx->crc_ev[CRC_EV_DONE]));
        crc_take(ctx, nblocks);
    }
    return SFQ_OK;
}

int sfq_encode_blocks(sfq_ctx* ctx, const uint8_t* d_fastq, uint64_t nbytes, const sfq_params* params,
                      uint8_t* d_out, uint64_t out_cap, sfq_result* result) {
    return encode_impl(ctx, d_fastq, nbytes, params, d_out, out_cap, result, 0);
}
int sfq_encode_qlt_blocks(sfq_ctx* ctx, const uint8_t* d_fastq, uint64_t nbytes, const sfq_params* params,
                          uint8_t* d_out, uint64_t out_cap, sfq_result* result) {
    return encode_impl(ctx, d_fastq, nbytes, params, d_out, out_cap, result, SFQ_M_QLT);
}
int sfq_build_priors(sfq_ctx* ctx, const uint8_t* d_fastq, uint64_t nbytes, const sfq_params* params) {
    sfq_result res;
    return encode_impl(ctx, d_fastq, nbytes, params, nullptr, 0, &res, 0, true);
}
int sfq_count_priors(sfq_ctx* ctx, const uint8_t* d_fastq, uint64_t nbytes, const sfq_params* params, uint32_t sample_scale) {
    if (!ctx || !params) return fail(ctx, SFQ_E_ARG, "null argument");
    if (params->prior_step == SFQ_PRIOR_GIVEN || params->prior_step == SFQ_PRIOR_COUNTS || !params->block_reads)
        return fail(ctx, SFQ_E_ARG, "sfq_count_priors: a sample of this text's own, in the block format (prior_step: a step or SFQ_PRIOR_AUTO)");
    sfq_result res;
    ctx->counts_only = true; ctx->sample_scale = sample_scale ? sample_scale : 1;
    const int rc = encode_impl(ctx, d_fastq, nbytes, params, nullptr, 0, &res, 0, true);
    ctx->counts_only = false; ctx->sample_scale = 1;
    return rc;
}
void sfq_prior_counts_words(int level, uint64_t* qlt_words, uint64_t* rec_words) {
    if (qlt_words) *qlt_words = (uint64_t)(clamp_level(level) == 1 ? (1u << 12) : (1u << 16)) * 64;
    if (rec_words) *rec_words = (uint64_t)PR_REC_ROWS * 256;
}
int sfq_get_prior_counts(sfq_ctx* ctx, int level, uint32_t* d_qlt, uint32_t* d_rec) {
    if (!ctx || !d_qlt || !d_rec) return fail(ctx, SFQ_E_ARG, "null argument");
    uint64_t nq, nr; sfq_prior_counts_words(level, &nq, &nr);
    if (!ctx->counts.valid || !ctx->hist.p || ctx->counts.q_rows != (u32)(nq / 64)) return fail(ctx, SFQ_E_ARG, "no counts for level %d (sfq_count_priors comes first)", level);
    HIPC(hipSetDevice(ctx->dev));
    HIPC(hipMemcpyAsync(d_qlt, ctx->hist.p, nq * 4, hipMemcpyDeviceToDevice, ctx->st));
    if (ctx->counts.rec && ctx->hcnt.p) HIPC(hipMemcpyAsync(d_rec, ctx->hcnt.p, nr * 4, hipMemcpyDeviceToDevice, ctx->st));
    else HIPC(hipMemsetAsync(d_rec, 0, nr * 4, ctx->st));
    HIPC(hipStreamSynchronize(ctx->st));
    return SFQ_OK;
}
int sfq_set_prior_counts(sfq_ctx* ctx, int level, const uint32_t* d_qlt, const uint32_t* d_rec) {
    if (!ctx || !d_qlt || !d_rec) return fail(ctx, SFQ_E_ARG, "null argument");
    uint64_t nq, nr; sfq_prior_counts_words(level, &nq, &nr);
    HIPC(hipSetDevice(ctx->dev));
    int rc;
    const bool own_rec = ctx->counts.valid && ctx->counts.q_rows == (u32)(nq / 64) ? ctx->counts.rec : true;
    ctx->counts.valid = false;
    if ((rc = ensure_prior_buffers(ctx, (u32)(nq / 64)))) return rc;
    if ((rc = reserve(ctx, ctx->hcnt, (size_t)REC_COUNT_COPIES * PR_REC_ROWS * 256 * 4))) return rc;
    HIPC(hipMemcpyAsync(ctx->hist.p, d_qlt, nq * 4, hipMemcpyDeviceToDevice, ctx->st));
    HIPC(hipMemcpyAsync(ctx->hcnt.p, d_rec, nr * 4, hipMemcpyDeviceToDevice, ctx->st));
    HIPC(hipStreamSynchronize(ctx->st));
    ctx->counts.valid = true; ctx->counts.q_rows = (u32)(nq / 64); ctx->counts.rec = own_rec;
    return SFQ_OK;
}
int sfq_encode_blocks_host(sfq_ctx* ctx, const uint8_t* h_fastq, uint64_t nbytes, const sfq_params* params,
                           uint8_t* h_out, uint64_t out_cap, sfq_result* result) {
    if (!ctx || !h_fastq || !h_out) return fail(ctx, SFQ_E_ARG, "null argument");
    HIPC(hipSetDevice(ctx->dev));
    int rc;
    if ((rc = reserve(ctx, ctx->in_stage, (size_t)nbytes + 16))) return rc;
    const u64 bound = sfq_encode_bound(nbytes);
    if ((rc = reserve(ctx, ctx->out_stage, (size_t)bound))) return rc;
    HIPC(hipMemcpyAsync(ctx->in_stage.p, h_fastq, (size_t)nbytes, hipMemcpyHostToDevice, ctx->st));
    rc = encode_impl(ctx, (const u8*)ctx->in_stage.p, nbytes, params, (u8*)ctx->out_stage.p, bound, result, 0);
    if (rc) return rc;
    if (result->total_bytes > out_cap) return fail(ctx, SFQ_E_OVERFLOW, "output needs %llu bytes", (unsigned long long)result->total_bytes);
    HIPC(hipMemcpyAsync(h_out, ctx->out_stage.p, (size_t)result->total_bytes, hipMemcpyDeviceToHost, ctx->st));
    HIPC(hipStreamSynchronize(ctx->st));
    return SFQ_OK;
}

int sfq_get_block_index(sfq_ctx* ctx, sfq_block_info* h_blocks, uint32_t cap) {
    if (!ctx || !h_blocks) return SFQ_E_ARG;
    if (cap < ctx->index.size()) return fail(ctx, SFQ_E_ARG, "index has %zu blocks", ctx->index.size());
    if (!ctx->index.empty()) memcpy(h_blocks, ctx->index.data(), ctx->index.size() * sizeof(sfq_block_info));
    return (int)ctx->index.size();
}
int sfq_get_first_headers(sfq_ctx* ctx, uint8_t* h_blob, uint64_t cap) {
    if (!ctx || !h_blob) return SFQ_E_ARG;
    if (cap < ctx->first_hdrs.size()) return fail(ctx, SFQ_E_ARG, "blob has %zu bytes", ctx->first_hdrs.size());
    if (!ctx->first_hdrs.empty()) memcpy(h_blob, ctx->first_hdrs.data(), ctx->first_hdrs.size());
    return SFQ_OK;
}

int64_t sfq_get_qlt_prior(sfq_ctx* ctx, uint8_t* h_blob, uint64_t cap) {
    if (!ctx) return SFQ_E_ARG;
    if (h_blob && cap >= ctx->prior_blob.size() && !ctx->prior_blob.empty()) memcpy(h_blob, ctx->prior_blob.data(), ctx->prior_blob.size());
    return (int64_t)ctx->prior_blob.size();
}
static void drop_encode_blobs(sfq_ctx* ctx) {
    if (!ctx->blobs_from_encode) return;
    ctx->prior_blob.clear(); ctx->rec_prior_blob.clear(); ctx->chain_blob.clear();
    ctx->blobs_from_encode = false;
}
int sfq_set_qlt_prior(sfq_ctx* ctx, const uint8_t* h_blob, uint64_t n) {
    if (!ctx || (n && !h_blob)) return SFQ_E_ARG;
    drop_encode_blobs(ctx);
    ctx->prior_blob.assign(h_blob, h_blob + n);
    return SFQ_OK;
}
int64_t sfq_get_rec_prior(sfq_ctx* ctx, uint8_t* h_blob, uint64_t cap) {
    if (!ctx) return SFQ_E_ARG;
    if (h_blob && cap >= ctx->rec_prior_blob.size() && !ctx->rec_prior_blob.empty()) memcpy(h_blob, ctx->rec_prior_blob.data(), ctx->rec_prior_blob.size());
    return (int64_t)ctx->rec_prior_blob.size();
}
int sfq_set_rec_prior(sfq_ctx* ctx, const uint8_t* h_blob, uint64_t n) {
    if (!ctx || (n && !h_blob)) return SFQ_E_ARG;
    drop_encode_blobs(ctx);
    ctx->rec_prior_blob.assign(h_blob, h_blob + n);
    return SFQ_OK;
}
int64_t sfq_get_chain_index(sfq_ctx* ctx, uint8_t* h_blob, uint64_t cap) {
    if (!ctx) return SFQ_E_ARG;
    if (h_blob && cap >= ctx->chain_blob.size() && !ctx->chain_blob.empty()) memcpy(h_blob, ctx->chain_blob.data(), ctx->chain_blob.size());
    return (int64_t)ctx->chain_blob.size();
}
int sfq_set_chain_index(sfq_ctx* ctx, const uint8_t* h_blob, uint64_t n) {
    if (!ctx || (n && !h_blob)) return SFQ_E_ARG;
    drop_encode_blobs(ctx);
    ctx->chain_blob.assign(h_blob, h_blob + n);
    return SFQ_OK;
}

static int decode_body(sfq_ctx* ctx, const sfq_params* pp, const sfq_block_info* h_blocks, uint32_t nblocks,
                       const uint8_t* h_first_hdrs, uint64_t first_hdr_bytes,
                       const uint8_t* d_streams, const uint64_t stream_offset[SFQ_NSTREAMS],
                       uint8_t* d_out, uint64_t out_cap, uint64_t* out_bytes, sfq_result* res, const u32* expect);
struct Expected {
    std::vector<u32> crc; bool set = false;
    explicit Expected(sfq_ctx* ctx) { crc.swap(ctx->crc_expect); set = ctx->crc_expect_set; ctx->crc_expect_set = false; }
};
static int decode_device(sfq_ctx* ctx, const sfq_params* pp, const sfq_block_info* h_blocks, uint32_t nblocks,
                         const uint8_t* h_first_hdrs, uint64_t first_hdr_bytes,
                         const uint8_t* d_streams, const uint64_t stream_offset[SFQ_NSTREAMS],
                         uint8_t* d_out, uint64_t out_cap, uint64_t* out_bytes, sfq_result* res, const Expected& ex) {
    if (!pp || !h_blocks || !nblocks || !d_streams || !stream_offset || !d_out || !out_bytes)
        return fail(ctx, SFQ_E_ARG, "null argument");
    HIPC(hipSetDevice(ctx->dev));
    Settle settle(ctx);
    drop_encode_blobs(ctx);
    ctx->crcs.clear(); ctx->text_crc = 0;
    const bool check = ex.set;
    const std::vector<u32>& expect = ex.crc;
    if (check && expect.size() != nblocks) return fail(ctx, SFQ_E_ARG, "%zu block checksums installed for a call of %u blocks", expect.size(), nblocks);
    const int rc = decode_body(ctx, pp, h_blocks, nblocks, h_first_hdrs, first_hdr_bytes, d_streams, stream_offset, d_out, out_cap, out_bytes, res,
                               check ? expect.data() : nullptr);
    settle.ok = rc == SFQ_OK;
    return rc;
}
int sfq_decode_blocks(sfq_ctx* ctx, const sfq_params* pp, const sfq_block_info* h_blocks, uint32_t nblocks,
                      const uint8_t* h_first_hdrs, uint64_t first_hdr_bytes,
                      const uint8_t* d_streams, const uint64_t stream_offset[SFQ_NSTREAMS],
                      uint8_t* d_out, uint64_t out_cap, uint64_t* out_bytes, sfq_result* res) {
    if (!ctx) return SFQ_E_ARG;
    const Expected ex(ctx);
    return decode_device(ctx, pp, h_blocks, nblocks, h_first_hdrs, first_hdr_bytes, d_streams, stream_offset, d_out, out_cap, out_bytes, res, ex);
}
static int decode_body(sfq_ctx* ctx, const sfq_params* pp, const sfq_block_info* h_blocks, uint32_t nblocks,
                       const uint8_t* h_first_hdrs, uint64_t first_hdr_bytes,
                       const uint8_t* d_streams, const uint64_t stream_offset[SFQ_NSTREAMS],
                       uint8_t* d_out, uint64_t out_cap, uint64_t* out_bytes, sfq_result* res, const u32* expect) {
    sfq_params p = *pp;
    HostTimes ht;
    p.level = clamp_level(p.level);
    ctx->framed.valid = false;
    const u32 version = p.version ? p.version : 6;
    if (p.kernel == 2) p.kernel = 0;
    if (p.kernel > 1) return fail(ctx, SFQ_E_ARG, "kernel %u: 0 = default kernels, 1 = lane-per-block cross-check kernels", p.kernel);
    if (version > 6) return fail(ctx, SFQ_E_UNSUPPORTED, "archive version %u is newer than 6 (config.cpp:373-377)", version);
    hipStream_t st = ctx->st;
    int rc;
    sfq_result local; if (!res) res = &local;
    memset(res, 0, sizeof *res);
    res->abi_version = SFQ_ABI_VERSION;
    HIPC(hipEventRecord(ctx->ev[ED_BEGIN], st));

    Bump bump;
    {
        const size_t cn = ctx->chain_blob.size();
        const size_t need = (size_t)nblocks * (sizeof(BlockDesc) + 8 * SFQ_NSTREAMS + 12) + (cn + 64) * 24 + 4096;
        if ((rc = reserve_pinned_buf(ctx, ctx->pin2, ctx->pin2_cap, need))) return rc;
        bump.p = (u8*)ctx->pin2; bump.off = 0; bump.cap = need;
    }
    BlockDesc* hb = bump.take<BlockDesc>(nblocks);
    const size_t nbso = (size_t)nblocks * SFQ_NSTREAMS;
    u64* bso = bump.take<u64>(nbso);
    if (!hb || !bso) return fail(ctx, SFQ_E_NOMEM, "decode: host scratch");
    u64 run[SFQ_NSTREAMS];
    for (int s = 0; s < SFQ_NSTREAMS; s++) run[s] = stream_offset[s];
    u64 nrec = 0; u32 block_reads = h_blocks[0].n_records; int g_bits = 0, g_bits_min = 64;
    for (u32 b = 0; b < nblocks; b++) {
        const sfq_block_info& bi = h_blocks[b];
        BlockDesc& d = hb[b];
        memset(&d, 0, sizeof d);
        if (bi.first_record != nrec) return fail(ctx, SFQ_E_ARG, "block %u: first_record %llu, expected %llu", b, (unsigned long long)bi.first_record, (unsigned long long)nrec);
        if (b + 1 < nblocks && bi.n_records != block_reads) return fail(ctx, SFQ_E_ARG, "block %u: non-uniform block size", b);
        if (bi.n_records == 0 || (b + 1 == nblocks && bi.n_records > block_reads)) return fail(ctx, SFQ_E_ARG, "block %u: bad record count", b);
        if (bi.first_hdr_off + bi.first_hdr_len > first_hdr_bytes) return fail(ctx, SFQ_E_ARG, "block %u: first header outside the blob", b);
        if (bi.first_hdr_len > SFQ_MAX_ID_LLEN) return fail(ctx, SFQ_E_CORRUPT, "block %u: first header of %u bytes (limit %u, usrs.hpp:34)", b, bi.first_hdr_len, (u32)SFQ_MAX_ID_LLEN);
        if (bi.gen_bits < 2 || bi.gen_bits > 26) return fail(ctx, SFQ_E_ARG, "block %u: gen_bits %u", b, bi.gen_bits);
        d.rec0 = nrec; d.nrec = bi.n_records; d.llen = bi.llen; d.solid = bi.solid; d.two_id = bi.two_id;
        d.gen_bits = bi.gen_bits; d.n_byte = bi.n_byte; d.first_hdr_off = bi.first_hdr_off; d.first_hdr_len = bi.first_hdr_len;
        g_bits = std::max<int>(g_bits, bi.gen_bits); g_bits_min = std::min<int>(g_bits_min, bi.gen_bits);
        for (int s = 0; s < SFQ_NSTREAMS; s++) {
            if (bi.size[s] > 0xFFFFFFFFull) return fail(ctx, SFQ_E_UNSUPPORTED, "block %u: stream %s has %llu bytes (the kernels take streams below 4 GiB)", b, sfq_stream_name(s), (unsigned long long)bi.size[s]);
            d.size[s] = (u32)bi.size[s]; bso[(size_t)b * SFQ_NSTREAMS + s] = run[s]; run[s] += bi.size[s];
        }
        nrec += bi.n_records;
    }
    const bool has_over = h_blocks[0].size[SFQ_S_USR_LREC] != 0;
    for (u32 b = has_over ? 1u : 0u; b < nblocks; b++)
        if (h_blocks[b].size[SFQ_S_USR_LREC] | h_blocks[b].size[SFQ_S_USR_LGEN] | h_blocks[b].size[SFQ_S_USR_LQLT])
            return fail(ctx, SFQ_E_UNSUPPORTED, "block %u holds oversize records (usr.lrec): only a one-block (format 6) archive does", b);
    if (has_over && nblocks != 1) return fail(ctx, SFQ_E_UNSUPPORTED, "oversize records (usr.lrec) in an archive of %u blocks: only a one-block (format 6) archive has them", nblocks);
    ht.mark("blocks checked");
    const bool frozen = !ctx->chain_blob.empty();
    u32 chain_reads = 0, cpb = 0, nchains = 0, gen_on = 0, rec_chains = 0, rchain_reads = 0, rcpb = 0, nsub = 0, gm_on = 0, gm_tb = 0;
    u32 flat_quads = 0, flat_raw = 0;
    u32 gchain_reads = 0, gcpb = 0, ngc = 0; u64 gm_ngc = 0;
    bool exc_rice = false;
    u32 seg_len = 0; std::vector<u32> seg_c0;
    std::vector<u32> h_rsz, h_rhb, rec_prior_f;
// ... 589 lines not shown
```

slimfastq_amd/csrc/chains.hip:

```cpp
#include "kernels.h"
#include "dev_chain.h"
#include "dev_walk.h"
typedef u32 __attribute__((aligned(1))) u32_any;

#define LAST_QLT 63u
#define QROW_BYTES 256u
#define B2_INIT 0x03030303u

#define QDEC_ROW 72u
__device__ __forceinline__ void qdec_store(u16* row, u32 s, u32 cum) {
    if (s) row[8 + s - 1] = (u16)cum;
    if ((s & 7u) == 0) row[s >> 3] = (u16)cum;
    if (s == 63) row[8 + 63] = 0;
}
__global__ __launch_bounds__(256) void k_qlt_frozen_rows(const u32* __restrict__ rows66, u32 q_rows, u32* __restrict__ qrows, u16* __restrict__ qdec) {
    const u32 lane = threadIdx.x & 63;
    const u32 ctx = blockIdx.x * 4 + (threadIdx.x >> 6);
    if (ctx >= q_rows) return;
    const u32* r = rows66 + (size_t)ctx * 66;
    const u32 slot = r[lane], iend = r[65];
    if (iend == 0) {
        qrows[(size_t)ctx * 64 + lane] = (lane << 10) | (1024u << 16);
        if (qdec) qdec_store(qdec + (size_t)ctx * QDEC_ROW, lane, lane << 10);
        return;
    }
    const u32 sym = slot >> 16, fslot = lane < iend ? (slot & 0xffffu) : 0u;
    const u32 f = (u32)__builtin_amdgcn_ds_permute((int)((lane < iend ? sym : lane) * 4), (int)fslot);
    const u32 x = f + 1;
    u32 S = x;
#pragma unroll
    for (int d = 32; d > 0; d >>= 1) S += (u32)__shfl_xor((int)S, d, 64);
    u32 g = (x << 16) / S;
    g = g ? g : 1u;
    u32 sum = g, best = (g << 6) | (63u - lane);
#pragma unroll
    for (int d = 32; d > 0; d >>= 1) {
        sum += (u32)__shfl_xor((int)sum, d, 64);
        const u32 o = (u32)__shfl_xor((int)best, d, 64); best = o > best ? o : best;
    }
    if (lane == 63u - (best & 63u)) g += 65536u - sum;
    u32 incl = g;
#pragma unroll
    for (int d = 1; d < 64; d <<= 1) { const u32 o = (u32)__shfl_up((int)incl, d, 64); if (lane >= (u32)d) incl += o; }
    qrows[(size_t)ctx * 64 + lane] = (incl - g) | (g << 16);
    if (qdec) qdec_store(qdec + (size_t)ctx * QDEC_ROW, lane, incl - g);
}
void launch_qlt_frozen_rows(const u32* rows66, u32 q_rows, u32* qrows, u16* qdec, hipStream_t st) {
    hipLaunchKernelGGL(k_qlt_frozen_rows, dim3((q_rows + 3) / 4), dim3(256), 0, st, rows66, q_rows, qrows, qdec);
}

#define QH_SYMS 48u
#define QH_ROW_U16 50u
#define QH_MAP_BYTES(q_rows) ((q_rows) / 32u * 8u)
#define QH_EMPTY 0xFFFFFFFFu
__global__ __launch_bounds__(256) void k_hot_totals(const u32* __restrict__ hist, const u32* __restrict__ rows66, u32 q_rows, u32* __restrict__ ctot) {
    const u32 lane = threadIdx.x & 63;
    const u32 ctx = blockIdx.x * 4 + (threadIdx.x >> 6);
    if (ctx >= q_rows) return;
    u32 c = hist[(size_t)ctx * 64 + lane];
#pragma unroll
    for (int d = 32; d > 0; d >>= 1) c += (u32)__shfl_xor((int)c, d, 64);
    const u32 iend = rows66[(size_t)ctx * 66 + 65];
    if (lane == 0) ctot[ctx] = (iend != 0 && iend <= QH_SYMS) ? c : 0u;
}
__global__ __launch_bounds__(1024) void k_hot_select(const u32* __restrict__ ctot, u32 q_rows, u32 want, uint2* __restrict__ map, u32* __restrict__ info) {
    __shared__ u32 red[16];
    __shared__ u32 wbits[2048];
    const u32 t = threadIdx.x, lane = t & 63, wave = t >> 6;
    const u32 nwords = q_rows / 32u;
    u32 c[64];
    u32 mx = 0;
#pragma unroll
    for (u32 k = 0; k < 64; k++) {
        const u32 ctx = k * 1024u + t;
        c[k] = ctx < q_rows ? ctot[ctx] : 0u;
        mx = c[k] > mx ? c[k] : mx;
    }
    auto block_sum = [&](u32 v) {
#pragma unroll
        for (int d = 32; d > 0; d >>= 1) v += (u32)__shfl_xor((int)v, d, 64);
        __syncthreads();
        if (lane == 0) red[wave] = v;
        __syncthreads();
        u32 s2 = 0;
        for (u32 w = 0; w < 16; w++) s2 += red[w];
        return s2;
    };
    auto block_max = [&](u32 v) {
#pragma unroll
        for (int d = 32; d > 0; d >>= 1) { const u32 o = (u32)__shfl_xor((int)v, d, 64); v = o > v ? o : v; }
        __syncthreads();
        if (lane == 0) red[wave] = v;
        __syncthreads();
        u32 s2 = 0;
        for (u32 w = 0; w < 16; w++) s2 = red[w] > s2 ? red[w] : s2;
        return s2;
    };
    u32 lo = 1, hi = block_max(mx) + 1u;
    while (lo < hi) {
        const u32 mid = lo + (hi - lo) / 2u;
        u32 n = 0;
#pragma unroll
        for (u32 k = 0; k < 64; k++) n += c[k] >= mid;
        if (block_sum(n) <= want) hi = mid; else lo = mid + 1u;
    }
    const u32 T = lo;
#pragma unroll
    for (u32 k = 0; k < 64; k++) {
        const u64 m = __ballot(c[k] >= T);
        if (lane == 0) { wbits[k * 32u + wave * 2u] = (u32)m; wbits[k * 32u + wave * 2u + 1u] = (u32)(m >> 32); }
    }
    __syncthreads();
    const u32 b0 = 2u * t < nwords ? wbits[2u * t] : 0u, b1 = 2u * t + 1u < nwords ? wbits[2u * t + 1u] : 0u;
    const u32 mine = (u32)__popc(b0) + (u32)__popc(b1);
    u32 inc = mine;
#pragma unroll
    for (int d = 1; d < 64; d <<= 1) { const u32 o = (u32)__shfl_up((int)inc, d, 64); if (lane >= (u32)d) inc += o; }
    __syncthreads();
    if (lane == 63) red[wave] = inc;
    __syncthreads();
    u32 before = 0, all = 0;
    for (u32 w = 0; w < 16; w++) { const u32 v = red[w]; before += w < wave ? v : 0u; all += v; }
    const u32 rank = before + inc - mine;
    if (t == 0) info[0] = all;
    if (2u * t < nwords) map[2u * t] = make_uint2(b0, rank);
    if (2u * t + 1u < nwords) map[2u * t + 1u] = make_uint2(b1, rank + (u32)__popc(b0));
}
__global__ __launch_bounds__(256) void k_hot_image(const uint2* __restrict__ map, const u32* __restrict__ qrows, u32 q_rows, u16* __restrict__ rows) {
    const u32 lane = threadIdx.x & 63;
    const u32 ctx = blockIdx.x * 4 + (threadIdx.x >> 6);
    if (ctx >= q_rows) return;
    const uint2 mr = map[ctx >> 5];
    const u32 bit = 1u << (ctx & 31u);
    if (!(mr.x & bit)) return;
    const u32 slot = mr.y + (u32)__popc(mr.x & (bit - 1u));
    if (lane < QH_ROW_U16) rows[(size_t)slot * QH_ROW_U16 + lane] = lane <= QH_SYMS ? (u16)FZ_CUM(qrows[(size_t)ctx * 64 + lane]) : (u16)0;
}
void launch_hot_rows(const u32* hist, const u32* rows66, const u32* qrows, u32 q_rows, u32 want, u32* ctot, u8* img, u32* info, hipStream_t st) {
    hipLaunchKernelGGL(k_hot_totals, dim3((q_rows + 3) / 4), dim3(256), 0, st, hist, rows66, q_rows, ctot);
    hipLaunchKernelGGL(k_hot_select, dim3(1), dim3(1024), 0, st, (const u32*)ctot, q_rows, want, reinterpret_cast<uint2*>(img), info);
    hipLaunchKernelGGL(k_hot_image, dim3((q_rows + 3) / 4), dim3(256), 0, st, reinterpret_cast<const uint2*>(img), qrows, q_rows,
                       reinterpret_cast<u16*>(img + QH_MAP_BYTES(q_rows)));
}

#define QHD_ROW_U16 8u
#define QHD_MAX_ROWS 6000u
__global__ __launch_bounds__(256) void k_hot_totals_prior(const u32* __restrict__ rows66, u32 q_rows, u32* __restrict__ ctot) {
    const u32 ctx = blockIdx.x * 256 + threadIdx.x;
    if (ctx >= q_rows) return;
    const u32 iend = rows66[(size_t)ctx * 66 + 65];
    ctot[ctx] = iend != 0 ? rows66[(size_t)ctx * 66 + 64] + 1u : 0u;
}
__global__ __launch_bounds__(256) void k_hot_image_dec(const uint2* __restrict__ map, const u16* __restrict__ qdec, u32 q_rows, u16* __restrict__ rows) {
    const u32 ctx = blockIdx.x * 256 + threadIdx.x;
    if (ctx >= q_rows) return;
    const uint2 mr = map[ctx >> 5];
    const u32 bit = 1u << (ctx & 31u);
    if (!(mr.x & bit)) return;
    const u32 slot = mr.y + (u32)__popc(mr.x & (bit - 1u));
    *reinterpret_cast<uint4*>(rows + (size_t)slot * QHD_ROW_U16) = *reinterpret_cast<const uint4*>(qdec + (size_t)ctx * QDEC_ROW);
}
void launch_hot_rows_dec(const u32* rows66, const u16* qdec, u32 q_rows, u32 want, u32* ctot, u8* img, u32* info, hipStream_t st) {
    hipLaunchKernelGGL(k_hot_totals_prior, dim3((q_rows + 255) / 256), dim3(256), 0, st, rows66, q_rows, ctot);
    hipLaunchKernelGGL(k_hot_select, dim3(1), dim3(1024), 0, st, (const u32*)ctot, q_rows, want, reinterpret_cast<uint2*>(img), info);
    hipLaunchKernelGGL(k_hot_image_dec, dim3((q_rows + 255) / 256), dim3(256), 0, st, reinterpret_cast<const uint2*>(img), qdec, q_rows,
                       reinterpret_cast<u16*>(img + QH_MAP_BYTES(q_rows)));
}
u32 hot_rows_dec_max(void) { return QHD_MAX_ROWS; }

__global__ __launch_bounds__(256) void k_seg_count(const u64* __restrict__ line_off, const BlockDesc* __restrict__ blocks, u32 block_reads, u64 nrec, u32 seg_len, u32* __restrict__ nseg) {
    const u64 r = (u64)blockIdx.x * 256 + threadIdx.x;
    if (r >= nrec) return;
    nseg[r] = seg_count_of(rec_symbols(line_off, r, blocks[r / block_reads].solid), seg_len);
}
__global__ __launch_bounds__(256) void k_seg_count_dec(const u32* __restrict__ slen, const u32* __restrict__ qlen, u64 nrec, u32 seg_len, u32* __restrict__ nseg) {
    const u64 r = (u64)blockIdx.x * 256 + threadIdx.x;
    if (r >= nrec) return;
    nseg[r] = seg_count_of(slen[r] > qlen[r] ? slen[r] : qlen[r], seg_len);
}
__global__ __launch_bounds__(256) void k_seg_fill(const u64* __restrict__ seg_off, u64 nrec, u32* __restrict__ seg_rec) {
    const u64 r = (u64)blockIdx.x * 256 + threadIdx.x;
    if (r >= nrec) return;
    for (u64 c = seg_off[r]; c < seg_off[r + 1]; c++) seg_rec[c] = (u32)r;
}
void launch_seg_count(const u64* line_off, const BlockDesc* blocks, u32 block_reads, u64 nrec, u32 seg_len, u32* nseg, hipStream_t st) {
    hipLaunchKernelGGL(k_seg_count, dim3((u32)((nrec + 255) / 256)), dim3(256), 0, st, line_off, blocks, block_reads, nrec, seg_len, nseg);
}
void launch_seg_count_dec(const u32* slen, const u32* qlen, u64 nrec, u32 seg_len, u32* nseg, hipStream_t st) {
    hipLaunchKernelGGL(k_seg_count_dec, dim3((u32)((nrec + 255) / 256)), dim3(256), 0, st, slen, qlen, nrec, seg_len, nseg);
}
void launch_seg_fill(const u64* seg_off, u64 nrec, u32* seg_rec, hipStream_t st) {
    hipLaunchKernelGGL(k_seg_fill, dim3((u32)((nrec + 255) / 256)), dim3(256), 0, st, seg_off, nrec, seg_rec);
}

#ifndef QLT_STEP
#define QLT_STEP 2u
#endif
#define QLT_RING 8
template <int THREADS, bool LDS, bool MARK>
__global__ __launch_bounds__(THREADS) void k_qlt_encode_c(ChainArgs a) {
    __shared__ u32 ring[LaneEncB<THREADS, QLT_RING>::LDS_DWORDS];
    extern __shared__ u32 lds[];
    const uint2* const lmap = reinterpret_cast<const uint2*>(lds);
    const u16* const lrows = reinterpret_cast<const u16*>(lds + QH_MAP_BYTES(a.q_rows) / 4u);
    if constexpr (LDS) {
        const u32 nd = (QH_MAP_BYTES(a.q_rows) + a.qh_info[0] * QH_ROW_U16 * 2u + 3u) / 4u;
        const u32* src = reinterpret_cast<const u32*>(a.qh_img);
        for (u32 i = threadIdx.x; i < nd; i += THREADS) lds[i] = src[i];
        __syncthreads();
    }
    const u32 c = blockIdx.x * THREADS + threadIdx.x;
    const bool live = c < a.geo.nchains;
    ChainPos cp; cp.b = 0; cp.r0 = 0; cp.nrec = 0; cp.sub_lo = cp.sub_len = 0; cp.seg = 0; cp.nseg = 1;
    if (live) { cp = chain_pos(a, c); chain_seg_encode(a, cp); }
    const BlockDesc* d = &a.m.blocks[cp.b];
    LaneEncB<THREADS, QLT_RING> rc; u32 cap = 0;
    u8* outp = live ? chain_region(a, cp, SFQ_S_QLT, 2, 1, cap) : nullptr;
    rc.init(ring, threadIdx.x, outp, cap);
    const int level = a.m.level;
    const u32 mask12 = level == 1 ? 0xFFFu : 0xFFFFu;
    LineWalk lw; lw.init(a, cp.r0, cp.nrec, 3, live ? d->solid : 0u, cp.sub_lo, cp.sub_len);
    u32 last = 0, p1 = 0, p2 = 0, delta = 5;
    u32 extra = 0;
    const __amdgpu_buffer_rsrc_t qtab = __builtin_amdgcn_make_buffer_rsrc((void*)a.qrows, 0, (int)(a.q_rows * 256u), 0x00020000);
    auto look8 = [&](const Piece& p, const uint4& f, const u32 j0, u32 (&e)[QLT_STEP], u32 (&eg)[QLT_STEP], u32& lowest, u32& top) {
        if (j0 == 0 && p.newline) { last = 0; p1 = p2 = 0; delta = 5; }
        const u32 len = p.j1;
        lowest = 255; top = 0;
#pragma unroll
        for (u32 jj = 0; jj < QLT_STEP; jj++) {
            const u32 j = j0 + jj;
            const u32 vm = j < len ? ~0u : 0u;
            const u32 b = (piece_byte(f, j) - '!') & 0xffu;
            const u32 sym = b < LAST_QLT ? b : LAST_QLT;
            if constexpr (MARK) lowest = min(lowest, b | ~vm);
            top = max(top, b & vm);
            if constexpr (LDS) {
                const uint2 mr = lmap[last >> 5];
                const u32 bit = 1u << (last & 31u);
                const u32 hm = ((mr.x & bit) && sym < QH_SYMS) ? ~0u : 0u;
                const u32 ridx = ((mr.y + (u32)__popc(mr.x & (bit - 1u))) * QH_ROW_U16 + sym) & hm;
                const u32 c0 = lrows[ridx], c1 = lrows[ridx + 1];
                const u32 g = (u32)__builtin_amdgcn_raw_buffer_load_b32(qtab, (int)(((last << 8) | (sym << 2)) | hm), 0, 0);
                e[jj] = (c0 | ((c1 - c0) << 16)) & hm; eg[jj] = g;
            } else { e[jj] = a.qrows[(size_t)last * 64 + sym]; eg[jj] = 0; }
            if (level <= 2) last = (b | (last << 6)) & mask12;
            else {
                delta += max(p1, b) - b;
                const u32 d3 = delta >> 3;
                last = (b | ((p1 < p2 ? p2 : p1) << 6) | ((u32)(p1 == p2) << 12) | ((d3 < 7 ? d3 : 7) << 13)) & 0xFFFFu;
                p2 = p1; p1 = b;
            }
        }
    };
    auto code8 = [&](const Piece& p, const uint4& f, const u32 j0, const u32 (&e)[QLT_STEP], u32 lowest, u32 top) {
        const u32 len = p.j1;
        if constexpr (MARK) if (lowest == 0 && p.valid) a.exc_flag[cp.r0 + p.rk] = 1;
        if (!__any(top >= LAST_QLT)) {
#pragma unroll
            for (u32 jj = 0; jj < QLT_STEP; jj++) {
                rc.encode16_if(j0 + jj < len ? ~0u : 0u, FZ_CUM(e[jj]), FZ_FREQ(e[jj]));
                if (((j0 + jj) & 3u) == 3u) rc.drain();
            }
        } else {
#pragma unroll
            for (u32 jj = 0; jj < QLT_STEP; jj++) {
                const u32 j = j0 + jj;
                const u32 vm = j < len ? ~0u : 0u;
                rc.encode16_if(vm, FZ_CUM(e[jj]), FZ_FREQ(e[jj]));
                const u32 b = (piece_byte(f, j) - '!') & 0xffu;
                const u32 em = (b >= LAST_QLT ? ~0u : 0u) & vm;
                if (__any(em != 0)) {
                    const u32 ee = a.qesc[b];
                    rc.encode16_if(em, FZ_CUM(ee), FZ_FREQ(ee));
                    extra -= em;
                }
                if ((j & 3u) == 3u) rc.drain();
            }
        }
    };
    Piece pc = lw.next();
    uint4 w = lw.fetch(pc);
    Piece pn = lw.next();
    uint4 wn = lw.fetch(pn);
    constexpr u32 NS = 16u / QLT_STEP;
    u32 E[NS][QLT_STEP], lows[MARK ? NS : 1u], esc = 0;
#pragma unroll
    for (u32 k = 0; k < NS; k++) {
        u32 G[QLT_STEP], lowt, topt;
        look8(pc, w, k * QLT_STEP, E[k], G, lowt, topt);
#pragma unroll
        for (u32 j = 0; j < QLT_STEP; j++) E[k][j] |= G[j];
        if (__any(topt >= LAST_QLT)) esc |= 1u << k;
        if constexpr (MARK) lows[k] = lowt;
    }
    while (__any(pc.valid)) {
        const Piece pnn = lw.next();
        const uint4 wnn = lw.fetch(pnn);
        u32 escn = 0;
#pragma unroll
        for (u32 k = 0; k < NS; k++) {
            u32 T[QLT_STEP], G[QLT_STEP], lowt, topt;
            look8(pn, wn, k * QLT_STEP, T, G, lowt, topt);
            code8(pc, w, k * QLT_STEP, E[k], MARK ? lows[MARK ? k : 0u] : 255u, ((esc >> k) & 1u) ? LAST_QLT : 0u);
#pragma unroll
            for (u32 j = 0; j < QLT_STEP; j++) E[k][j] = T[j] | G[j];
            if (__any(topt >= LAST_QLT)) escn |= 1u << k;
            if constexpr (MARK) lows[k] = lowt;
        }
        esc = escn;
        pc = pn; w = wn; pn = pnn; wn = wnn;
    }
    if (live) {
        const u32 size = rc.finish();
        a.csz[c] = size;
        if (extra) atomicAdd(&a.m.blocks[cp.b].extra_hi, extra);
        if (rc.err & 2) atomicMax(&a.m.blocks[cp.b].status, (u32)(-SFQ_E_OVERFLOW));
        else if (rc.err) atomicMax(&a.m.blocks[cp.b].status, (u32)(-SFQ_E_CORRUPT));
    }
}
template <int T>
static void launch_qlt_lds(const ChainArgs& a, u32 dyn, hipStream_t st) {
    static u32 allowed = 0;
    if (dyn > allowed) { (void)hipFuncSetAttribute(reinterpret_cast<const void*>(&k_qlt_encode_c<T, true, false>), hipFuncAttributeMaxDynamicSharedMemorySize, (int)dyn); allowed = dyn; }
    hipLaunchKernelGGL((k_qlt_encode_c<T, true, false>), dim3((a.geo.nchains + T - 1) / T), dim3(T), dyn, st, a);
}
void launch_qlt_encode_c(const ChainArgs& a, hipStream_t st) {
    if (a.exc_flag) { hipLaunchKernelGGL((k_qlt_encode_c<256, false, true>), dim3((a.geo.nchains + 255) / 256), dim3(256), 0, st, a); return; }
    if (a.q_hot) {
        const u32 dyn = QH_MAP_BYTES(a.q_rows) + a.q_hot * QH_ROW_U16 * 2u;
        launch_qlt_lds<1024>(a, dyn, st);
    } else hipLaunchKernelGGL((k_qlt_encode_c<256, false, false>), dim3((a.geo.nchains + 255) / 256), dim3(256), 0, st, a);
}

template <int THREADS, bool LDS>
__global__ __launch_bounds__(THREADS) void k_qlt_decode_c(ChainArgs a, DecodeArgs da) {
    extern __shared__ u32 lds[];
    const uint2* const lmap = reinterpret_cast<const uint2*>(lds);
    const u16* const lrows = reinterpret_cast<const u16*>(lds + QH_MAP_BYTES(a.q_rows) / 4u);
    if constexpr (LDS) {
        const u32 nd = (QH_MAP_BYTES(a.q_rows) + a.qh_info[0] * QHD_ROW_U16 * 2u + 3u) / 4u;
        const u32* src = reinterpret_cast<const u32*>(a.qh_img);
        for (u32 i = threadIdx.x; i < nd; i += THREADS) lds[i] = src[i];
        __syncthreads();
    }
    const u32 c = blockIdx.x * THREADS + threadIdx.x;
    if (c >= a.geo.nchains) return;
    LaneDecQ rc; rc.init(da.streams + a.coff[c], a.csz[c], reinterpret_cast<const u8*>(a.qesc));
    const int level = a.m.level;
    const u32 mask12 = level == 1 ? 0xFFFu : 0xFFFFu;
    ChainPos cp = chain_pos(a, c);
    u32 n_next = cp.nrec ? da.qlen[cp.r0] : 0u; u64 off_next = cp.nrec ? da.qoff[cp.r0] : 0ull;
    if (a.seg_len) {
        const u32 sl = da.slen[cp.r0];
        seg_range(cp, sl > n_next ? sl : n_next);
        const u64 lo = cp.sub_lo < n_next ? cp.sub_lo : n_next;
        n_next = (u32)(n_next - lo < cp.sub_len ? n_next - lo : cp.sub_len); off_next += lo;
    }
    for (u32 k = 0; k < cp.nrec; k++) {
        const u32 n = n_next; const u64 off = off_next;
        if (k + 1 < cp.nrec) { n_next = da.qlen[cp.r0 + k + 1]; off_next = da.qoff[cp.r0 + k + 1]; }
        LaneOut32 out; out.begin(da.qual_stage + off);
        u32 last = 0, p1 = 0, p2 = 0, delta = 5;
        for (u32 i = 0; i < n; i++) {
            const u16* qd = a.qdec + (size_t)last * QDEC_ROW;
            u32 hot = ~0u;
            if constexpr (LDS) {
                const uint2 mr = lmap[last >> 5];
                asm volatile("" :: "v"(mr.x), "v"(mr.y));
                const u32 bit = 1u << (last & 31u);
                if (mr.x & bit) hot = (mr.y + (u32)__popc(mr.x & (bit - 1u))) * QHD_ROW_U16;
            }
            uint4 cv;
            if constexpr (LDS) {
                const uint4 cl = *reinterpret_cast<const uint4*>(lrows + (hot != ~0u ? hot : 0u));
                uint4 cg = make_uint4(0, 0, 0, 0);
                if (hot == ~0u) cg = *reinterpret_cast<const uint4*>(qd);
                asm volatile("" :: "v"(cl.x), "v"(cl.y), "v"(cl.z), "v"(cl.w));
                const bool st = hot != ~0u;
                cv.x = st ? cl.x : cg.x; cv.y = st ? cl.y : cg.y; cv.z = st ? cl.z : cg.z; cv.w = st ? cl.w : cg.w;
            } else cv = *reinterpret_cast<const uint4*>(qd);
            rc.top_up();
            u32 r;
            const u32 prob = rc.get_freq16(r);
            const bool t4 = (cv.z & 0xffffu) <= prob;
            const u32 A0 = t4 ? cv.z : cv.x, A1 = t4 ? cv.w : cv.y;
            const bool t2 = (A1 & 0xffffu) <= prob;
            const u32 B = t2 ? A1 : A0;
            const bool t1 = (B >> 16) <= prob;
            const u32 k8 = (t4 ? 4u : 0u) | (t2 ? 2u : 0u) | (t1 ? 1u : 0u);
            const u32 ff0 = t1 ? B >> 16 : B & 0xffffu;
            const uint4 w = *reinterpret_cast<const uint4*>(qd + 8 + k8 * 8u);
            const bool u4 = (w.y >> 16) <= prob;
            const u32 x = u4 ? w.y >> 16 : ff0, y0 = u4 ? w.z : w.x, y1 = u4 ? w.w : w.y;
            const bool u2 = (y0 >> 16) <= prob;
            const u32 x2 = u2 ? y0 >> 16 : x, z = u2 ? y1 : y0;
            const bool u1 = (z & 0xffffu) <= prob;
            const u32 win = u1 ? z : (x2 | (z << 16));
            const u32 s = k8 * 8u + ((u4 ? 4u : 0u) | (u2 ? 2u : 0u) | (u1 ? 1u : 0u));
            const u32 cum = win & 0xffffu;
            rc.decode(r, cum, ((win >> 16) - cum) & 0xffffu);
            u32 b = s;
            if (s == LAST_QLT) {
                rc.top_up();
                u32 re;
                const u32 pe = rc.get_freq16(re);
                b = pe >> 8; b = b > 255u ? 255u : b;
                rc.decode(re, b << 8, 256u);
            }
            out.put(('!' + b) & 0xffu);
            if (level <= 2) last = (b | (last << 6)) & mask12;
            else {
                delta += max(p1, b) - b;
                const u32 d3 = delta >> 3;
                last = (b | ((p1 < p2 ? p2 : p1) << 6) | ((u32)(p1 == p2) << 12) | ((d3 < 7 ? d3 : 7) << 13)) & 0xFFFFu;
                p2 = p1; p1 = b;
            }
        }
        out.end();
    }
    if (rc.err) atomicMax(&a.m.blocks[cp.b].status, (u32)(-SFQ_E_CORRUPT));
}
void launch_qlt_decode_c(const ChainArgs& a, const DecodeArgs& da, hipStream_t st) {
    if (a.q_hot) {
        constexpr int T = 1024;
        const u32 dyn = QH_MAP_BYTES(a.q_rows) + a.q_hot * QHD_ROW_U16 * 2u;
        static u32 allowed = 0;
        if (dyn > allowed) { (void)hipFuncSetAttribute(reinterpret_cast<const void*>(&k_qlt_decode_c<T, true>), hipFuncAttributeMaxDynamicSharedMemorySize, (int)dyn); allowed = dyn; }
        hipLaunchKernelGGL((k_qlt_decode_c<T, true>), dim3((a.geo.nchains + T - 1) / T), dim3(T), dyn, st, a, da);
    } else {
        constexpr int T = 256;
        hipLaunchKernelGGL((k_qlt_decode_c<T, false>), dim3((a.geo.nchains + T - 1) / T), dim3(T), 0, st, a, da);
    }
}

__global__ __launch_bounds__(256) void k_chain_block_sizes(ChainArgs a, ChainGeoArgs geo, int stream, const u32* csz, const u32* rhb) {
    const u32 b = blockIdx.x * 4 + (threadIdx.x >> 6), lane = threadIdx.x & 63;
    if (b >= a.m.nblocks) return;
    u32 sum = 0, hb = 0;
    const bool seg = a.seg_len && stream != SFQ_S_REC;
    const u64 c0 = seg ? block_chain0(a, geo, b) : (u64)b * geo.cpb;
    u64 c1 = seg ? block_chain1(a, geo, b) : c0 + geo.cpb;
    if (c1 > geo.nchains) c1 = geo.nchains;
    for (u64 cc = c0 + lane; cc < c1; cc += 64) { sum += csz[cc]; if (rhb) hb += rhb[cc]; }
#pragma unroll
    for (int d = 32; d > 0; d >>= 1) { sum += (u32)__shfl_xor((int)sum, d, 64); hb += (u32)__shfl_xor((int)hb, d, 64); }
    if (lane == 0) {
        a.m.blocks[b].size[stream] = sum;
        if (rhb) a.m.blocks[b].hdr_bytes = hb;
    }
}
void launch_chain_block_sizes(const ChainArgs& a, const ChainGeoArgs& geo, int stream, const u32* csz, const u32* rhb, hipStream_t st) {
    hipLaunchKernelGGL(k_chain_block_sizes, dim3((a.m.nblocks + 3) / 4), dim3(256), 0, st, a, geo, stream, csz, rhb);
}
__global__ __launch_bounds__(256) void k_compact_chains(ChainArgs a, ChainGeoArgs geo, int stream, u32 num, u32 den, const u32* csz,
                                                        const u64* blk_stream_off, const u64* stream_base, u8* out, const u32* gate) {
    const u32 c = blockIdx.x * 4 + (threadIdx.x >> 6), lane = threadIdx.x & 63;
    if (c >= geo.nchains) return;
    if (gate && !gate[0]) return;
    const bool seg = a.seg_len && stream != SFQ_S_REC;
    if (!seg) a.seg_len = 0;
    a.geo = geo;
    ChainPos cp = chain_pos(a, c);
    const u32 n = csz[c];
    if (!n) return;
    u32 before = 0;
    for (u64 cc = block_chain0(a, geo, cp.b) + lane; cc < c; cc += 64) before += csz[cc];
#pragma unroll
    for (int d = 32; d > 0; d >>= 1) before += (u32)__shfl_xor((int)before, d, 64);
    u32 cap;
    const u8* src = chain_region(a, cp, stream, num, den, cap);
    u8* dst = out + stream_base[stream] + blk_stream_off[(u64)cp.b * SFQ_NSTREAMS + stream] + before;
    const u32 n16 = n >> 4;
    for (u32 i = lane; i < n16; i += 64) {
        const u32* q = reinterpret_cast<const u32*>(src + 16 * i);
        const uint4 v = make_uint4(q[0], q[1], q[2], q[3]);
        u32* w = reinterpret_cast<u32*>(dst + 16 * i);
        w[0] = v.x; w[1] = v.y; w[2] = v.z; w[3] = v.w;
    }
    for (u32 i = (n16 << 4) + lane; i < n; i += 64) dst[i] = src[i];
}
void launch_compact_chains(const ChainArgs& a, const ChainGeoArgs& geo, int stream, u32 num, u32 den, const u32* csz, const u64* blk_stream_off,
                           const u64* stream_base, u8* out, hipStream_t st, const u32* gate) {
    hipLaunchKernelGGL(k_compact_chains, dim3((geo.nchains + 3) / 4), dim3(256), 0, st, a, geo, stream, num, den, csz, blk_stream_off, stream_base, out, gate);
}

template <typename LOOK, typename CODE>
__device__ __forceinline__ void walk_bases(const ChainArgs& a, u64 r0, u32 nrec, u32 solid, u32 mask, LOOK&& look, CODE&& code, u32 seg = 0, u32 seg_len = 0) {
    const u32 warm = (seg_len && seg) ? 16u : 0u;
    LineWalk lw;
    if (seg_len) lw.init(a, r0, nrec, 1, solid, (u64)seg * seg_len - warm, (u64)seg_len + warm);
    else lw.init(a, r0, nrec, 1, solid);
    u32 last = 0, seen = 0;
    Piece pc = lw.next();
    uint4 w = lw.fetch(pc);
    while (__any(pc.valid)) {
        const Piece pn = lw.next();
        const uint4 wn = lw.fetch(pn);
        if (pc.newline) last = 0x007616c7u;
        u32 codes = 0;
        const u32 seen0 = seen;
#pragma unroll
        for (u32 j = 0; j < 16; j++) {
            if (j >= pc.j0 && j < pc.j1) {
                const u32 cd = gen_code_of(piece_byte(w, j)) & 3u;
                if (seen >= warm) look(j, last & mask);
                seen++;
                last = (last << 2) | cd;
                codes |= cd << (2 * j);
            }
        }
        seen = seen0;
#pragma unroll
        for (u32 j = 0; j < 16; j++) if (j >= pc.j0 && j < pc.j1) { if (seen >= warm) code(j, (codes >> (2 * j)) & 3u); seen++; }
        pc = pn; w = wn;
    }
}

template <typename LOOK, typename CODE, typename PEND>
__device__ __forceinline__ u32 walk_bases_b(const ChainArgs& a, u64 r0, u32 nrec, u32 solid, u32 mask, const u8* lut, LOOK&& look, CODE&& code, PEND&& piece_end, u8* exc_flag,
                                            u64 sub_lo = 0, u64 sub_len = 0) {
    LineWalk lw; lw.init(a, r0, nrec, 1, solid, sub_lo, sub_len);
    u32 last = 0, illegal = 0;
    Piece pc = lw.next();
    uint4 w = lw.fetch(pc);
    while (__any(pc.valid)) {
        const Piece pn = lw.next();
        const uint4 wn = lw.fetch(pn);
        if (pc.newline) last = 0x007616c7u;
        const uint4& f = w;
        const u32 len = pc.j1;
        u32 cd4[16];
#pragma unroll
        for (u32 j = 0; j < 16; j++) cd4[j] = lut[piece_byte(f, j)];
        u32 codes = 0, odd = 0;
#pragma unroll
        for (u32 j = 0; j < 16; j++) {
            look(j, last & mask);
            last = (last << 2) | (cd4[j] & 3u);
            codes |= (cd4[j] & 3u) << (2 * j);
            odd |= cd4[j] & (j < len ? ~0u : 0u);
        }
        if (exc_flag && (odd & 0x34u) && pc.valid) exc_flag[r0 + pc.rk] = 1;
        illegal |= odd & 0x10u;
#pragma unroll
        for (u32 j = 0; j < 16; j++) {
            code(j, (codes >> (2 * j)) & 3u, j < len ? ~0u : 0u);
            if ((j & 3u) == 3u) piece_end();
        }
        pc = pn; w = wn;
    }
    return illegal;
}

template <typename QUAD>
__device__ __forceinline__ u32 walk_bases_q(const ChainArgs& a, u64 r0, u32 nrec, u32 solid, const u8* lut, QUAD&& quad, u8* exc_flag, u64 sub_lo = 0, u64 sub_len = 0) {
    LineWalk lw; lw.init(a, r0, nrec, 1, solid, sub_lo, sub_len);
    u32 illegal = 0;
    Piece pc = lw.next();
    uint4 w = lw.fetch(pc);
    while (__any(pc.valid)) {
        const Piece pn = lw.next();
        const uint4 wn = lw.fetch(pn);
        const u32 len = pc.j1;
        u32 codes = 0, odd = 0;
#pragma unroll
        for (u32 j = 0; j < 16; j++) {
            const u32 cd = lut[piece_byte(w, j)];
            codes |= (cd & 3u) << (2 * j);
            odd |= cd & (j < len ? ~0u : 0u);
        }
        if (exc_flag && (odd & 0x34u) && pc.valid) exc_flag[r0 + pc.rk] = 1;
        illegal |= odd & 0x10u;
#pragma unroll
        for (u32 q = 0; q < 4; q++) {
            const u32 k = len > 4u * q ? (len - 4u * q < 4u ? len - 4u * q : 4u) : 0u;
            quad((codes >> (8u * q)) & 0xffu, k);
        }
        pc = pn; w = wn;
    }
    return illegal;
}

__global__ __launch_bounds__(256) void k_gen_count(ChainArgs a, u32 b0, u32 b1, u32 stride, u32 seg_len, u32 segs, u32* __restrict__ cnt, const u32* __restrict__ rows,
                                                  const u16* __restrict__ log2fp, u64* cost, u32 sub, u32 do_count) {
    const u64 first = a.m.blocks[b0].rec0, endr = a.m.blocks[b1 - 1].rec0 + a.m.blocks[b1 - 1].nrec;
    u32 mybases = 0;
    const u64 id = (u64)blockIdx.x * 256 + threadIdx.x;
    const u64 r = first + (id / segs) * stride;
    const u32 seg = (u32)(id % segs);
    const bool live = r < endr && (sub == 0 || (id / segs) % GEN_PRE != 0);
    u32 solid = 0, mask = 0;
    if (live) {
        const u32 b = (u32)(r / a.block_reads);
        solid = a.m.blocks[b].solid; mask = (1u << a.m.blocks[b].gen_bits) - 1u;
    }
    u64 mycost = 0;
    u32 cx[16], rv[16];
    walk_bases(a, r, live ? 1u : 0u, solid, mask,
        [&](u32 j, u32 ctx) { cx[j] = ctx; rv[j] = rows ? rows[ctx] : 0u; },
        [&](u32 j, u32 code) {
            if (do_count == 1) atomicAdd(&cnt[((size_t)cx[j] << 2) | code], 1u);
            if (rows) {
                const u32 v = rv[j];
                const u32 f0 = v & 0xff, f1 = (v >> 8) & 0xff, f2 = (v >> 16) & 0xff, f3 = v >> 24;
                if (do_count) {
                    mybases++;
                    mycost += (u32)log2fp[(f0 + f1) + (f2 + f3)] - (u32)log2fp[(v >> (8 * code)) & 0xff];
                } else if (v != 0x03030303u) {
                    const u32 m = ((f0 + f1) + (f2 + f3) - 12u) >> 2;
                    mybases += m;
                    mycost += (u64)(long long)((int)((v >> (8 * code)) & 0xff) - 3 - (int)m);
                }
            }
        }, seg, seg_len);
    if (rows) {
#pragma unroll
        for (int d = 32; d > 0; d >>= 1) mycost += __shfl_xor(mycost, d, 64);
#pragma unroll
        for (int d = 32; d > 0; d >>= 1) mybases += (u32)__shfl_xor((int)mybases, d, 64);
        if ((threadIdx.x & 63) == 0 && mybases) {
            atomicAdd((unsigned long long*)cost, (unsigned long long)mycost);
            atomicAdd((unsigned long long*)cost + 1, (unsigned long long)mybases);
        }
    }
}
void launch_gen_count(const ChainArgs& a, u32 b0, u32 b1, u64 nrec_range, u32 max_line, u32* cnt, const u32* rows, const u16* log2fp, u64* cost, hipStream_t st, u32 sub, u32 do_count) {
    if (!nrec_range) return;
    u32 stride = gen_count_stride(nrec_range);
    if (sub == 1) { stride *= GEN_PRE; sub = 0; }
    u32 seg_len = 0;
    if (max_line >= 64u) {
        const u64 nsel = (nrec_range + stride - 1) / stride;
        for (u32 sl = 32u; sl < max_line && sl <= 512u; sl *= 2u)
            if (nsel * ((max_line + sl - 1) / sl) <= 524288ull) { seg_len = sl; break; }
    }
    if (!seg_len && max_line > 1024u) seg_len = 512u;
    const u32 segs = seg_len ? (max_line + seg_len - 1) / seg_len : 1u;
    const u64 lanes = ((nrec_range + stride - 1) / stride) * segs;
    hipLaunchKernelGGL(k_gen_count, dim3((u32)((lanes + 255) / 256)), dim3(256), 0, st, a, b0, b1, stride, seg_len, segs, cnt, rows, log2fp, cost, sub, do_count);
}
#define GB_T 256u
#define GB_ROUNDS 2u
#define GB_TILE (GB_T * 16u * GB_ROUNDS)
#define GB_SLICE_BITS 14u
__host__ __device__ __forceinline__ u32 gb_slice_bits(u32 g_bits) { return g_bits < GB_SLICE_BITS ? g_bits : GB_SLICE_BITS; }

__global__ __launch_bounds__(GB_T) void k_gen_bin(ChainArgs a, u32 b0, u32 b1, u32 stride, u32 seg_len, u32 segs, u32 sub, u64 id0, u64 id1, u32 g_bits,
                                                  u16* __restrict__ bins, u32* __restrict__ fill, u32 cap, u32* __restrict__ cnt) {
    extern __shared__ u32 lds[];
    const u32 sb = gb_slice_bits(g_bits), nb = 1u << (g_bits - sb), sh = sb + 2u;
    u32* keys = lds;
    u32* hist = lds + GB_TILE;
    u32* base = hist + nb;
    const u32 tid = threadIdx.x;
    const u64 first = a.m.blocks[b0].rec0, endr = a.m.blocks[b1 - 1].rec0 + a.m.blocks[b1 - 1].nrec;
    const u64 id = id0 + (u64)blockIdx.x * GB_T + tid;
    const u64 r = first + (id / segs) * stride;
    const u32 seg = (u32)(id % segs);
    const bool live = id < id1 && r < endr && (sub == 0 || (id / segs) % GEN_PRE != 0);
    u32 solid = 0; const u32 mask = (1u << g_bits) - 1u;
    if (live) solid = a.m.blocks[(u32)(r / a.block_reads)].solid;
    const u32 warm = (seg_len && seg) ? 16u : 0u;
    LineWalk lw;
    if (seg_len) lw.init(a, r, live ? 1u : 0u, 1, solid, (u64)seg * seg_len - warm, (u64)seg_len + warm);
    else lw.init(a, r, live ? 1u : 0u, 1, solid);
    u32 last = 0, seen = 0;
    Piece pc = lw.next();
    uint4 w = lw.fetch(pc);
    for (;;) {
        for (u32 i = tid; i < nb; i += GB_T) hist[i] = 0;
        __syncthreads();
        int any = 0;
#pragma unroll
        for (u32 rd = 0; rd < GB_ROUNDS; rd++) {
            const Piece pn = lw.next();
            const uint4 wn = lw.fetch(pn);
            if (pc.newline) last = 0x007616c7u;
#pragma unroll
            for (u32 j = 0; j < 16; j++) {
                u32 k = ~0u;
                if (j < pc.j1) {
                    const u32 cd = gen_code_of(piece_byte(w, j)) & 3u;
                    if (seen >= warm) k = ((last & mask) << 2) | cd;
                    seen++;
                    last = (last << 2) | cd;
                }
                keys[(rd * 16u + j) * GB_T + tid] = k;
                if (k != ~0u) atomicAdd(&hist[k >> sh], 1u);
            }
            any |= pc.valid ? 1 : 0;
            pc = pn; w = wn;
        }
        if (!__syncthreads_or(any)) break;
        for (u32 i = tid; i < nb; i += GB_T) { const u32 n = hist[i]; base[i] = n ? atomicAdd(&fill[i], n) : 0u; hist[i] = 0; }
        __syncthreads();
        for (u32 i = tid; i < GB_TILE; i += GB_T) {
            const u32 k = keys[i];
            if (k == ~0u) continue;
            const u32 b = k >> sh;
            const u32 pos = base[b] + atomicAdd(&hist[b], 1u);
            if (pos < cap) bins[(size_t)b * cap + pos] = (u16)(k & ((1u << sh) - 1u));
            else atomicAdd(&cnt[k], 1u);
        }
        __syncthreads();
    }
}
__device__ __forceinline__ u32 gen_row_of(uint4 n, u32 step) {
    u64 f0 = 3 + (u64)step * n.x, f1 = 3 + (u64)step * n.y, f2 = 3 + (u64)step * n.z, f3 = 3 + (u64)step * n.w;
    while ((f0 | f1 | f2 | f3) > 255) {
        f0 = (f0 >> 1) | (f0 & 1); f1 = (f1 >> 1) | (f1 & 1); f2 = (f2 >> 1) | (f2 & 1); f3 = (f3 >> 1) | (f3 & 1);
    }
    return (u32)f0 | (u32)f1 << 8 | (u32)f2 << 16 | (u32)f3 << 24;
}
__global__ __launch_bounds__(1024) void k_gen_bin_count(const u16* __restrict__ bins, u32* __restrict__ fill, u32 cap, u32 g_bits, u32* __restrict__ cnt,
                                                        u32* __restrict__ rows_out, u32 step) {
    extern __shared__ u32 lds[];
    const u32 sb = gb_slice_bits(g_bits), nctx = 1u << sb, b = blockIdx.x, tid = threadIdx.x;
    u32 n = fill[b]; if (n > cap) n = cap;
    const u16* bin = bins + (size_t)b * cap;
    uint4* slice = reinterpret_cast<uint4*>(cnt + ((size_t)b << (sb + 2)));
    if (!n && !rows_out) return;
    for (u32 at = 0; ; at += 65535u) {
        for (u32 i = tid; i < 2u * nctx; i += 1024u) lds[i] = 0;
        __syncthreads();
        const u32 m = n - at < 65535u ? n - at : 65535u;
        for (u32 i = tid; i < m; i += 1024u) {
            const u32 k = bin[at + i];
            atomicAdd(&lds[k >> 1], 1u << ((k & 1u) * 16u));
        }
        __syncthreads();
        const bool last_chunk = at + m >= n;
        for (u32 i = tid; i < nctx; i += 1024u) {
            const u32 w0 = lds[2 * i], w1 = lds[2 * i + 1];
            if (!(w0 | w1) && !(rows_out && last_chunk)) continue;
            uint4 c = slice[i];
            c.x += w0 & 0xffffu; c.y += w0 >> 16; c.z += w1 & 0xffffu; c.w += w1 >> 16;
            if (w0 | w1) slice[i] = c;
            if (rows_out && last_chunk) rows_out[((size_t)b << sb) + i] = gen_row_of(c, step);
        }
        if (last_chunk) break;
        __syncthreads();
    }
    if (tid == 0) fill[b] = 0;
}
GenBins gen_bins_plan(u32 g_bits, u64 max_keys) {
    GenBins gb; gb.bins = nullptr; gb.fill = nullptr;
    gb.g_bits = g_bits;
    gb.batch = max_keys < GEN_BIN_BATCH ? (max_keys ? max_keys : 1) : GEN_BIN_BATCH;
    const u32 nb = 1u << (g_bits - gb_slice_bits(g_bits));
    gb.cap = (u32)((2ull * ((gb.batch + nb - 1) / nb) + 4096ull + 63ull) & ~63ull);
    gb.bins_bytes = (u64)gb.cap * 2ull * nb; gb.fill_bytes = 4ull * nb;
    return gb;
}
void launch_gen_count_binned(const ChainArgs& a, u32 b0, u32 b1, u64 nrec_range, u32 max_line, const GenBins& gb, u32* cnt, u32* rows_out, u32 step,
                             hipStream_t st, u32 sub) {
    const u32 g_bits = gb.g_bits, sb = gb_slice_bits(g_bits), nb = 1u << (g_bits - sb), cap = gb.cap;
    const u32 dyn2 = (2u << sb) * 4u;
    static u32 allowed = 0;
    if (dyn2 > 65536u && dyn2 > allowed) { (void)hipFuncSetAttribute(reinterpret_cast<const void*>(&k_gen_bin_count), hipFuncAttributeMaxDynamicSharedMemorySize, (int)dyn2); allowed = dyn2; }
    if (nrec_range) {
        u32 stride = gen_count_stride(nrec_range);
        if (sub == 1) { stride *= GEN_PRE; sub = 0; }
        u32 seg_len = 0;
        if (max_line >= 64u) {
            const u64 nsel = (nrec_range + stride - 1) / stride;
            for (u32 sl = 32u; sl < max_line && sl <= 512u; sl *= 2u)
                if (nsel * ((max_line + sl - 1) / sl) <= 524288ull) { seg_len = sl; break; }
        }
        if (!seg_len && max_line > 1024u) seg_len = 512u;
        const u32 segs = seg_len ? (max_line + seg_len - 1) / seg_len : 1u;
        const u64 lanes = ((nrec_range + stride - 1) / stride) * segs;
        const u64 per_lane = seg_len ? seg_len : (max_line ? max_line : 1u);
        u64 lanes_per_batch = gb.batch / per_lane; if (!lanes_per_batch) lanes_per_batch = 1;
        lanes_per_batch = (lanes_per_batch + GB_T - 1) / GB_T * GB_T;
        const u32 dyn1 = (GB_TILE + 2u * nb) * 4u;
        for (u64 id0 = 0; id0 < lanes; id0 += lanes_per_batch) {
            const u64 id1 = id0 + lanes_per_batch < lanes ? id0 + lanes_per_batch : lanes;
            const bool last = id1 >= lanes;
            hipLaunchKernelGGL(k_gen_bin, dim3((u32)((id1 - id0 + GB_T - 1) / GB_T)), dim3(GB_T), dyn1, st, a, b0, b1, stride, seg_len, segs, sub, id0, id1, g_bits, gb.bins, gb.fill, cap, cnt);
            hipLaunchKernelGGL(k_gen_bin_count, dim3(nb), dim3(1024), dyn2, st, (const u16*)gb.bins, gb.fill, cap, g_bits, cnt, last ? rows_out : nullptr, step);
        }
    } else if (rows_out) hipLaunchKernelGGL(k_gen_bin_count, dim3(nb), dim3(1024), dyn2, st, (const u16*)gb.bins, gb.fill, cap, g_bits, cnt, rows_out, step);
}

__global__ __launch_bounds__(256) void k_gen_rows(const u32* __restrict__ cnt, u32* __restrict__ rows, u64 nctx, u32 step) {
    const u64 c = (u64)blockIdx.x * 256 + threadIdx.x;
// ... 1485 lines not shown
```

slimfastq_amd/csrc/kernels.h:

```cpp
#pragma once
#include <hip/hip_runtime.h>
#include "dev_common.h"

struct ModelArgs {
    const u8*  fq;
    const u64* line_off;
    BlockDesc* blocks;
    u32 nblocks;
    u32 batch0, nbatch;
    u8* arena;
    i32 level;
    u32 lossless;
    u32 epoch_base;
    u32* q_slots; RowHdr* q_hdr; u32 q_rows;
    u32* p_slots; RowHdr* p_hdr;
    u32* g_tab;   u32 g_bits;
    const u32* prior_w; const u32* prior_wovf;
    const u32* prior_ls; const RowHdr* prior_lh;
    const u32* rec_map;
};
__device__ __forceinline__ u64 rec_count_of(const ModelArgs& a, u64 r, u64 base) { return a.rec_map ? (u64)a.rec_map[r] + 1 : r - base + 1; }

struct DecodeArgs {
    ModelArgs m;
    const u8*  streams;
    const u64* blk_stream_off;
    const u8*  first_hdrs;
    u32* slen; u32* qlen;
    u8*  pfg;  u8* pfq;
    const u64* soff; const u64* qoff;
    const u64* boff;
    u8*  seq_stage; u8* qual_stage;
    u8*  hdr_stage; u32* hlen;
    const u64* hdr_stage_off;
    const u32* hdr_stage_cap;
    u64* hoff;
    u32  block_reads;
    u32  version;
    u32  max_line;
};

struct ChainGeoArgs { u32 chain_reads, cpb, nchains; };
#define RDEC_LDS_ROWS 16u
#define GEN_MAX_GENERATIONS 40
struct ChainArgs {
    ModelArgs m;
    ChainGeoArgs geo;
    ChainGeoArgs rgeo;
    u32* rhb;
    u64 nbytes;
    u32 block_reads;
    u32* csz;
    const u64* coff;
    const u32* qrows;
    const u16* qdec;
    u32 q_rows;
    u32 q_hot;
    const u8* qh_img;
    const u32* qh_info;
    const u32* qesc;
    const u32* rrows;
    const u16* rdec;
    const u16* rmap; const u16* rhot; u32 r_hot;
    u8* exc_flag;
    u32 seg_len;
    const u64* seg_off;
    const u32* seg_rec;
    const u8* st_buf; u64 st_bytes; const u64* st_off; const u32* st_len;
    u32 g_ngen;
    u32 g_bound[GEN_MAX_GENERATIONS + 1];
    const u32* g_rows[GEN_MAX_GENERATIONS];
    const u32* g_init;
    u32 flat_quads;
    u32 flat_raw;
};
void launch_hot_rows(const u32* hist, const u32* rows66, const u32* qrows, u32 q_rows, u32 want, u32* ctot ,
                     u8* img , u32* info, hipStream_t st);
void launch_hot_rows_dec(const u32* rows66, const u16* qdec, u32 q_rows, u32 want, u32* ctot ,
                         u8* img , u32* info, hipStream_t st);
u32 hot_rows_dec_max(void);
void launch_qlt_frozen_rows(const u32* rows66, u32 q_rows, u32* qrows, u16* qdec , hipStream_t st);
void launch_qlt_encode_c(const ChainArgs& a, hipStream_t st);
void launch_gen_count(const ChainArgs& a, u32 b0, u32 b1, u64 nrec_range, u32 max_line ,
                      u32* cnt, const u32* rows, const u16* log2fp, u64* cost, hipStream_t st,
                      u32 sub = 0 , u32 do_count = 1 );
void launch_gen_rows(const u32* cnt, u32* rows, u64 nctx, u32 step, hipStream_t st);
void launch_gm_lens(const u64* line_off, const BlockDesc* blocks, u32 block_reads, u64 n, u32* slen, hipStream_t st);
void launch_gm_soff(const u64* boff, u64 n, u64* soff, hipStream_t st);
void launch_gm_sentinels(u8* stage, const u64* soff, const u32* slen, u64 n, hipStream_t st);
void launch_gm_stage(const ModelArgs& m, u32 block_reads, u64 r0, u64 r1, u64 nbytes , u8* stage, const u64* soff, const u32* slen, u8* exc_flag , hipStream_t st);
void launch_gm_insert(const ChainArgs& a, u32 b0, u32 b1, u64 nrec_range, u32 max_line, u64* T, u32 tb, hipStream_t st);
void launch_gm_plan(const ChainArgs& a, u64 nlanes , const u8* stage, u64 stage_bytes, const u64* soff, const u32* slen,
                    const u64* T, u32 tb, u8* tok, hipStream_t st);
void launch_gm_price(const ChainArgs& a, u64 r0, u64 r1, u64 step, u32 max_line , u64 lim_rec, const u8* stage, u64 stage_bytes, const u64* soff, const u32* slen, const u64* T, u32 tb,
                     const u16* costs , u64* cost , hipStream_t st);
void launch_gm_code(const ChainArgs& a, const u8* tok, hipStream_t st);
void launch_gm_decode_c(const ChainArgs& a, const struct DecodeArgs& da, u32 c0, u32 c1, u64 lim_rec, const u64* T, u32 tb, u64 stage_bytes, hipStream_t st);
#define GEN_BIN_BATCH (1ull << 27)
struct GenBins { u16* bins; u32* fill; u32 cap, g_bits; u64 batch, bins_bytes, fill_bytes; };
GenBins gen_bins_plan(u32 g_bits, u64 max_keys );
void launch_gen_count_binned(const ChainArgs& a, u32 b0, u32 b1, u64 nrec_range, u32 max_line, const GenBins& gb, u32* cnt, u32* rows_out, u32 step,
                             hipStream_t st, u32 sub = 0);
void launch_gen_encode_c(const ChainArgs& a, hipStream_t st, u32 c0 = 0, u32 c1 = 0 , bool flat = false );
enum ChnFlag : u32 {
    CHN_GEN_ON     = 1u << 0,
    CHN_REC_CHAINS = 1u << 1,
    CHN_DELTAS     = 1u << 2,
    CHN_SEGMENTS   = 1u << 3,
    CHN_EXC_RICE   = 1u << 4,
    CHN_GEN_MATCH  = 1u << 5,
    CHN_FLAT_QUADS = 1u << 6,
    CHN_FLAT_RAW   = 1u << 7,
    CHN_KNOWN      = (1u << 8) - 1
};
void launch_chain_index_bytes(const u32* csz, u32 n, u32 b1, u32 b2, u32 b3, u32* len, u64* off, u64* scan_tmp, u8* out, u64* info, hipStream_t st);
void launch_gen_exc_w(const ModelArgs& a, const u8* flags, u32* ticket, hipStream_t st);
void launch_gen_exc_r(const ModelArgs& a, const u8* flags, u32* ticket, hipStream_t st);
void launch_gen_exc_decode_r(const struct DecodeArgs& a, u32 nblocks, hipStream_t st);
#define REC_COUNT_COPIES 32u
void launch_rec_count(const ModelArgs& a, u64 nrec, u64 stride, u32 run, u32 nruns, u32* cnt ,
                      u32* flags , hipStream_t st);
void launch_rec_frozen_rows(const u32* f, u32 nrows, u32* rrows, u16* rdec , hipStream_t st);
void launch_rec_prior_freqs(const u32* cnt, u32 nrows, u32* f, u32* rtot, u32 nh, u16* map, u16* hot, hipStream_t st);
void launch_rec_encode_c(const ChainArgs& a, u32* flags , u32* flags2 , u32* tok , u32* ntok ,
                         u32 n_hot, u32 max_hdr, hipStream_t st,
                         u32 min_hdr = 0 ,
                         hipEvent_t after_tokens = nullptr );
u64 rec_token_bytes(u64 nrec);
void launch_seg_count(const u64* line_off, const BlockDesc* blocks, u32 block_reads, u64 nrec, u32 seg_len, u32* nseg, hipStream_t st);
void launch_seg_count_dec(const u32* slen, const u32* qlen, u64 nrec, u32 seg_len, u32* nseg, hipStream_t st);
void launch_seg_fill(const u64* seg_off, u64 nrec, u32* seg_rec, hipStream_t st);
void launch_chain_block_sizes(const ChainArgs& a, const ChainGeoArgs& geo, int stream, const u32* csz, const u32* rhb , hipStream_t st);
void launch_compact_chains(const ChainArgs& a, const ChainGeoArgs& geo, int stream, u32 num, u32 den, const u32* csz, const u64* blk_stream_off,
                           const u64* stream_base, u8* out, hipStream_t st, const u32* gate );
#define GEN_STEP 4u
#ifndef GEN_COUNT_CAP
#define GEN_COUNT_CAP 524288ull
#endif
#define GEN_PRE 8u
static inline u32 gen_count_stride(u64 n) { return (u32)((n + GEN_COUNT_CAP - 1) / GEN_COUNT_CAP ? (n + GEN_COUNT_CAP - 1) / GEN_COUNT_CAP : 1); }

void launch_max_u32(const u32* v, u64 n, u32* out , hipStream_t st);
void launch_over_first(const u64* line_off, u64 nrec, u32* first , hipStream_t st);
void launch_over_solid(const u8* fq, const u64* line_off, u64 r, u32* out, hipStream_t st);
void launch_over_flags(const u64* line_off, u64 nrec, u32 solid, u32* flags, u32* kbytes, u32* status, hipStream_t st);
void launch_over_split(const u8* fq, const u64* line_off, u64 nrec, const u32* flags, const u64* fpos, const u64* koff, u8* filt, u32* rec_map, u32* over_list, hipStream_t st);
void launch_over_encode_w(const ModelArgs& a, const u8* fq, const u64* line_off, const u32* over_list, u32 n_over, const u64 out_off[3], const u32 out_cap[3], hipStream_t st);
void launch_over_mark(const u64* over_no, u32 n_over, u64 total, u32* flags , u32* status, hipStream_t st);
void launch_over_map(const u32* flags, const u64* fpos, u64 total, u32* rec_map, hipStream_t st);
void launch_over_decode_w(const ModelArgs& a, const u8* stream, u32 size, u32 which, u32 store, u32 n_over, u64* cnt, u64* no, u64* piece, u8* txt, u64 cap, hipStream_t st);
void launch_over_place(u32 n_over, const u64* no, const u64* piece, const u8* lrec_txt, const u8* lgen_txt, const u8* lqlt_txt, const u64* roff_all, u8* out, hipStream_t st);
void launch_over_sizes(const u32* rec_map, const u32* rsize, u64 n_kept, const u64* no, const u64* piece, u32 n_over, u32* size_all, hipStream_t st);
void launch_gather_u64(const u64* src, const u32* idx, u64 n, u64* dst, hipStream_t st);
void launch_block_prepare(const u8* fq, const u64* line_off, u64 nrec, u32 block_reads, BlockDesc* blocks, u32 nblocks,
                          u64 nbytes, i32 level, i32 gen_bits_req, hipStream_t st);
u32 frame_tiles(u64 n);
void launch_frame(const u8* fq, u64 n, u64* tstat , u64* line_off, u64 cap, u32* status, u8* exc_flag , u64 ecap ,
                  void* frame_out , hipStream_t st);
void launch_validate_lines(const u64* line_off, u64 nrec, u32 max_hdr, u32 max_line, u32* status, hipStream_t st);
void launch_text_fingerprint(const u8* fq, u64 n, u64* out , hipStream_t st);
#define FRAME_CHUNK 16384u

void launch_scan_u32(const u32* in, u64* out, u64 n, u64* tmp , hipStream_t st, u32 pad = 0 );

void launch_qlt_encode_l(const ModelArgs& a, hipStream_t st);
void launch_gen_encode_l(const ModelArgs& a, hipStream_t st);
void launch_rec_encode_l(const ModelArgs& a, hipStream_t st);
void launch_usr_encode_l(const ModelArgs& a, hipStream_t st);
void launch_fill_u32(u32* p, u64 n, u32 v, hipStream_t st);

void launch_qlt_encode_k(const ModelArgs& a, u32* ticket, hipStream_t st);
void launch_gen_encode_k(const ModelArgs& a, u32* ticket, hipStream_t st);
void launch_rec_encode_w(const ModelArgs& a, u32* ticket_fast, u32* ticket_slow, hipStream_t st);
void launch_usr_encode_w(const ModelArgs& a, hipStream_t st);

void launch_qlt_decode_c(const ChainArgs& a, const DecodeArgs& da, hipStream_t st);
void launch_gen_decode_c(const ChainArgs& a, const DecodeArgs& da, u32 c0, u32 c1 , hipStream_t st);
void launch_rec_decode_c(const ChainArgs& a, const DecodeArgs& da, u32* flags , hipStream_t st,
                         u32* dtok = nullptr , u32* dtoff = nullptr , u32* dflags = nullptr );
u64 rec_dtok_bytes(u64 nrec);
void launch_gen_exc_decode_l(const DecodeArgs& a, hipStream_t st);
void launch_gen_exc_decode_w(const DecodeArgs& a, hipStream_t st);
void launch_usr_decode_l(const DecodeArgs& a, hipStream_t st, u32 prefilled = 0);
void launch_usr_decode_w(const DecodeArgs& a, hipStream_t st, u32 prefilled);
void launch_usr_fill(const DecodeArgs& a, u64 nrec, hipStream_t st);
void launch_qlt_decode_l(const DecodeArgs& a, hipStream_t st);
void launch_gen_decode_l(const DecodeArgs& a, hipStream_t st);
void launch_rec_decode_l(const DecodeArgs& a, hipStream_t st);
void launch_qlt_decode_w(const DecodeArgs& a, hipStream_t st);
void launch_gen_decode_w(const DecodeArgs& a, hipStream_t st);
void launch_rec_decode_w(const DecodeArgs& a, hipStream_t st);

void launch_block_stream_offsets(BlockDesc* blocks, u32 nblocks, u64* blk_stream_off, u64* stream_total, hipStream_t st);
void launch_compact(const BlockDesc* blocks, u32 nblocks, const u8* arena, const u64* blk_stream_off,
                    const u64* stream_base, u8* out, u32 skip_streams , hipStream_t st, const u32* gate);
void launch_stream_gate(const BlockDesc* blocks, u32 nblocks, const u64* stream_total, u64 out_cap, u64* stream_base , u32* gate , hipStream_t st);
void launch_record_sizes(const DecodeArgs& a, u64 nrec, u32* rsize, hipStream_t st);
void launch_assemble(const DecodeArgs& a, u64 nrec, const u64* roff, u8* out, hipStream_t st);
void launch_first_hdr_lens(const BlockDesc* blocks, u32 nblocks, u32* lens, hipStream_t st);
void launch_gather_first_hdrs(const BlockDesc* blocks, u32 nblocks, const u8* fq, const u64* blob_off, u8* blob, u64 cap, hipStream_t st);

void launch_qlt_hist(const u8* fq, u64 nbytes, const u64* line_off, const BlockDesc* blocks, u32 block_reads, u64 nrec, u32 step,
                     int level, u32 cap , u32* hist, hipStream_t st);
#define PRIOR_SYMBOLS 4096u
void launch_prior_rows(const u32* hist, u32 q_rows, u32* rows66, u32* w_rows, u32* w_ovf, u32* l_slots, RowHdr* l_hdr, hipStream_t st);
void launch_prior_list(const u32* rows66, u32 q_rows, u32* slot, u32* list, hipStream_t st);
void launch_prior_scatter(const u32* ctxs, const u32* rows , u32 n, u32* rows66 , hipStream_t st);
void launch_prior_spread(const u32* rows66, u32 q_rows, u32* w_rows, u32* w_ovf, u32* l_slots, RowHdr* l_hdr, hipStream_t st);

struct CrcScratch { u64 ntiles = 0, ngroups = 0; };
CrcScratch crc_scratch_words(u64 lo, u64 hi, const u8* d);
u32  crc_table_words();
void crc_build_tables(u32* tab);
u32  crc32_combine_host(u32 crc_a, u32 crc_b, u64 len_b);
void launch_crc32(const u8* d, const u64* d_bounds, u32 n_ranges, u32 whole, u64 lo, u64 hi, u32* tile_crc, u32* grp_crc, u32* out,
                  const u32* tab, hipStream_t st);
void launch_crc_block_bounds(const u64* offs, u64 stride, u32 nblocks, u64 total, u64* bounds, hipStream_t st);
```

slimfastq_amd/csrc/prior.hip:

```cpp
#include "kernels.h"
#include "dev_wave.h"

__device__ __forceinline__ u32 p_calc_last_delta(u32& delta, u32 q, u32 q1, u32 q2) {
    if (q1 > q) delta += q1 - q;
    u32 d3 = delta >> 3;
    return (q | ((q1 < q2 ? q2 : q1) << 6) | ((u32)(q1 == q2) << 12) | ((d3 < 7 ? d3 : 7) << 13)) & 0xFFFFu;
}
#ifndef HIST_S
#define HIST_S 16384u
#endif
#ifndef HIST_T
#define HIST_T 256
#endif
#define HIST_SLOTS HIST_S
#define HIST_EMPTY 0xFFFFFFFFu
#define HIST_CBITS 10u
#define HIST_CMASK ((1u << HIST_CBITS) - 1u)
#define HIST_HARVEST 256u
typedef __attribute__((address_space(3))) u32 lds_u32;
typedef __attribute__((address_space(1))) u32 glb_u32;
__device__ __forceinline__ void hist_add(lds_u32* slots, glb_u32* hist, u32 key) {
    u32 slot = ((key * 2654435761u) >> 16) & (HIST_SLOTS - 1);
    for (int probe = 0; probe < 128; probe++) {
        u32 v = slots[slot];
        if (v == HIST_EMPTY) {
            u32 expect = HIST_EMPTY;
            if (__hip_atomic_compare_exchange_strong(&slots[slot], &expect, (key << HIST_CBITS) | 1u, __ATOMIC_RELAXED, __ATOMIC_RELAXED, __HIP_MEMORY_SCOPE_WORKGROUP)) return;
            v = expect;
        }
        if ((v >> HIST_CBITS) == key) {
            if ((v & HIST_CMASK) >= 768u) { __hip_atomic_fetch_add(&hist[key], 1u, __ATOMIC_RELAXED, __HIP_MEMORY_SCOPE_AGENT); return; }
            const u32 old = __hip_atomic_fetch_add(&slots[slot], 1u, __ATOMIC_RELAXED, __HIP_MEMORY_SCOPE_WORKGROUP);
            if ((old & (HIST_HARVEST - 1u)) == HIST_HARVEST - 1u) {
                __hip_atomic_fetch_sub(&slots[slot], HIST_HARVEST, __ATOMIC_RELAXED, __HIP_MEMORY_SCOPE_WORKGROUP);
                __hip_atomic_fetch_add(&hist[key], HIST_HARVEST, __ATOMIC_RELAXED, __HIP_MEMORY_SCOPE_AGENT);
            }
            return;
        }
        slot = (slot + 1) & (HIST_SLOTS - 1);
    }
    __hip_atomic_fetch_add(&hist[key], 1u, __ATOMIC_RELAXED, __HIP_MEMORY_SCOPE_AGENT);
}
template <u32 THREADS, u32 READS_PER_LANE>
__global__ __launch_bounds__(THREADS) void k_qlt_hist(const u8* __restrict__ fq, u64 nbytes, const u64* __restrict__ line_off,
                                                 const BlockDesc* __restrict__ blocks, u32 block_reads,
                                                 u64 nrec, u32 step, int level, u32 cap, u32* __restrict__ hist) {
#ifndef NO_SETPRIO
    __builtin_amdgcn_s_setprio(3);
#endif
    __shared__ u32 slots[HIST_SLOTS];
    for (u32 i = threadIdx.x; i < HIST_SLOTS; i += THREADS) slots[i] = HIST_EMPTY;
    __syncthreads();
    for (u32 rr = 0; rr < READS_PER_LANE; rr++) {
        const u64 r = (((u64)blockIdx.x * READS_PER_LANE + rr) * THREADS + threadIdx.x) * step;
        if (r >= nrec) break;
        const u32 solid = blocks[r / block_reads].solid;
        const u64 q0 = line_off[4 * r + 3] + solid, q1e = line_off[4 * r + 4] - 1;
        const u32 nfull = q1e > q0 ? (u32)(q1e - q0) : 0;
        const u32 n = nfull < cap ? nfull : cap;
        const u64 a0 = q0 & ~3ull;
        const u32 skip = (u32)(q0 - a0);
        const u32* wp = reinterpret_cast<const u32*>(fq + a0);
        const u64 wmax = (nbytes - a0) / 4;
        u32 last = 0, delta = 5, q1 = 0, q2 = 0, di = 0;
        u32 done = 0;
        for (u64 w = 0; done < n; w += 4) {
            u32 wd[4];
#pragma unroll
            for (int k = 0; k < 4; k++) {
                if (w + k < wmax) wd[k] = wp[w + k];
                else { wd[k] = 0; for (int j = 0; j < 4; j++) { const u64 at = a0 + (w + k) * 4 + j; if (at < nbytes) wd[k] |= (u32)fq[at] << (8 * j); } }
            }
#pragma unroll
            for (int k = 0; k < 4; k++) {
#pragma unroll
                for (int j = 0; j < 4; j++) {
                    const u32 pos = (u32)(w + k) * 4 + j;
                    if (pos < skip || done >= n) continue;
                    const u32 b = (u32)(u8)(((wd[k] >> (8 * j)) & 0xff) - '!');
                    hist_add((lds_u32*)slots, (glb_u32*)hist, last * 64 + (b < 63u ? b : 63u));
                    if (level == 1)      last = (b | (last << 6)) & 0xFFFu;
                    else if (level == 2) last = (b | (last << 6)) & 0xFFFFu;
                    else if (++di & 1) { last = p_calc_last_delta(delta, b, q1, q2); q2 = b; }
                    else               { last = p_calc_last_delta(delta, b, q2, q1); q1 = b; }
                    done++;
                }
            }
        }
    }
    __syncthreads();
    for (u32 i = threadIdx.x; i < HIST_SLOTS; i += THREADS) { const u32 v = slots[i]; if (v != HIST_EMPTY && (v & HIST_CMASK)) atomicAdd(&hist[v >> HIST_CBITS], v & HIST_CMASK); }
}
__global__ __launch_bounds__(256) void k_qlt_hist_w(const u8* __restrict__ fq, const u64* __restrict__ line_off,
                                                    const BlockDesc* __restrict__ blocks, u32 block_reads,
                                                    u64 nrec, u32 step, int level, u32 cap, u32* __restrict__ hist) {
    __shared__ u32 slots[HIST_SLOTS];
    for (u32 i = threadIdx.x; i < HIST_SLOTS; i += 256) slots[i] = HIST_EMPTY;
    __syncthreads();
    const u32 lane = threadIdx.x & 63;
    const u64 r = ((u64)blockIdx.x * 4 + (threadIdx.x >> 6)) * step;
    if (r < nrec) {
        const u32 solid = blocks[r / block_reads].solid;
        const u64 q0 = line_off[4 * r + 3] + solid, q1e = line_off[4 * r + 4] - 1;
        const u32 nfull = q1e > q0 ? (u32)(q1e - q0) : 0;
        const u32 n = nfull < cap ? nfull : cap;
        const u32 mask = level == 1 ? 0xFFFu : 0xFFFFu;
        u32 c1 = 0, c2 = 0, c3 = 0, dsum = 5;
        for (u32 base = 0; base < n; base += 64) {
            const u32 i = base + lane;
            const bool in = i < n;
            const u32 b = in ? (u32)(u8)(fq[q0 + i] - '!') : 0u;
            const u32 b1 = wave_shr1(b, c1), b2 = wave_shr1(b1, c2), b3 = wave_shr1(b2, c3);
            u32 ctx;
            if (level <= 2) ctx = (b1 | (b2 << 6) | (b3 << 12)) & mask;
            else {
                const u32 t = b1 > b ? b1 - b : 0u;
                const u32 incl = wave_incl_scan(t);
                const u32 delta = dsum + incl - t;
                const u32 d3 = delta >> 3;
                ctx = (b1 | ((b2 < b3 ? b3 : b2) << 6) | ((u32)(b2 == b3) << 12) | ((d3 < 7 ? d3 : 7) << 13)) & 0xFFFFu;
                if (i == 0) ctx = 0;
                dsum += rl(incl, 63);
            }
            if (in) hist_add((lds_u32*)slots, (glb_u32*)hist, ctx * 64 + (b < 63u ? b : 63u));
            c1 = rl(b, 63); c2 = rl(b1, 63); c3 = rl(b2, 63);
        }
    }
    __syncthreads();
    for (u32 i = threadIdx.x; i < HIST_SLOTS; i += 256) { const u32 v = slots[i]; if (v != HIST_EMPTY && (v & HIST_CMASK)) atomicAdd(&hist[v >> HIST_CBITS], v & HIST_CMASK); }
}
void launch_qlt_hist(const u8* fq, u64 nbytes, const u64* line_off, const BlockDesc* blocks, u32 block_reads, u64 nrec, u32 step,
                     int level, u32 cap, u32* hist, hipStream_t st) {
    const u64 nsamp = (nrec + step - 1) / step;
    if (nbytes / (nrec ? nrec : 1) > 4000) {
        hipLaunchKernelGGL(k_qlt_hist_w, dim3((u32)((nsamp + 3) / 4)), dim3(256), 0, st, fq, line_off, blocks, block_reads, nrec, step, level, cap, hist);
    } else {
        const u64 per_wg = HIST_T;
        hipLaunchKernelGGL((k_qlt_hist<HIST_T, 1>), dim3((u32)((nsamp + per_wg - 1) / per_wg)), dim3(HIST_T), 0, st, fq, nbytes, line_off, blocks, block_reads, nrec, step, level, cap, hist);
    }
}

__device__ __forceinline__ u32 pr_sort64(u32 key, u32 lane) {
#pragma unroll
    for (u32 k = 2; k <= 64; k <<= 1) {
#pragma unroll
        for (u32 j = k >> 1; j > 0; j >>= 1) {
            const u32 other = (u32)__shfl_xor((int)key, j, 64);
            const bool up = (lane & k) == 0, lower = (lane & j) == 0;
            const u32 lo = key < other ? key : other, hi = key < other ? other : key;
            key = (lower == up) ? lo : hi;
        }
    }
    return key;
}
__global__ __launch_bounds__(256) void k_prior_rows(const u32* hist, u32 q_rows, u32* rows66, u32* w_rows, u32* w_ovf,
                                                   u32* l_slots, RowHdr* l_hdr) {
    const u32 lane = threadIdx.x & 63;
    const u32 ctx = blockIdx.x * 4 + (threadIdx.x >> 6);
    if (ctx >= q_rows) return;
    const u32 c = hist[(size_t)ctx * 64 + lane];
    const u64 seen = __ballot(c != 0);
    const u32 iend = seen ? 64u - (u32)__clzll((long long)seen) : 0u;
    u32 mx = c;
#pragma unroll
    for (int dd = 32; dd > 0; dd >>= 1) { const u32 o = (u32)__shfl_xor((int)mx, dd, 64); mx = o > mx ? o : mx; }
    u32 sh = 0;
    while ((((u64)mx * 6) >> sh) > 32000) sh++;
    const u32 fq = (u32)(((u64)c * 6) >> sh);
    const u32 key = lane < iend ? (((0xFFFFu - fq) << 6) | lane) : (0xFFFFFFC0u | lane);
    const u32 sk = pr_sort64(key, lane);
    const u32 f = lane < iend ? 0xFFFFu - (sk >> 6) : 0u;
    const u32 sym = sk & 63u;
    const u32 slot = lane < iend ? (f | (sym << 16)) : 0u;
    u32 tot = lane < iend ? f : 0u;
#pragma unroll
    for (int d = 32; d > 0; d >>= 1) tot += (u32)__shfl_xor((int)tot, d, 64);
    u32* r = rows66 + (size_t)ctx * 66;
    r[lane] = slot;
    if (lane == 0) { r[64] = tot; r[65] = iend; }
    l_slots[(size_t)ctx * 64 + lane] = slot;
    if (lane == 0) { RowHdr h; h.total = tot; h.iend = (u16)iend; h.count = 0; h.pad = 0; h.epoch = 0; h.pad2 = 0; l_hdr[ctx] = h; }
    u32* w = w_rows + (size_t)ctx * 64;
    if (lane < 60) w[4 + lane] = slot; else w_ovf[(size_t)ctx * 4 + (lane - 60)] = slot;
    if (lane == 0) { w[0] = tot; w[1] = iend; w[2] = 0; w[3] = 0; }
}
__global__ __launch_bounds__(256) void k_prior_flags(const u32* __restrict__ rows66, u32 q_rows, u32* __restrict__ slot) {
    const u32 c = blockIdx.x * 256 + threadIdx.x;
    if (c < q_rows) slot[c] = rows66[(size_t)c * 66 + 65] != 0 ? 1u : 0u;
}
__global__ __launch_bounds__(1024) void k_prior_slots(u32 q_rows, u32* __restrict__ slot, u32* __restrict__ list) {
    __shared__ u32 wsum[16];
    const u32 t = threadIdx.x, lane = t & 63, wave = t >> 6;
    const u32 per = (((q_rows + 1023u) / 1024u) + 3u) & ~3u, c0 = t * per;
    u32 mine = 0;
    for (u32 k = 0; k < per; k += 4) {
        if (c0 + k + 4 <= q_rows) { const uint4 v = *reinterpret_cast<const uint4*>(slot + c0 + k); mine += v.x + v.y + v.z + v.w; }
        else for (u32 j = 0; j < 4; j++) if (c0 + k + j < q_rows) mine += slot[c0 + k + j];
    }
    u32 inc = mine;
#pragma unroll
    for (int d = 1; d < 64; d <<= 1) { const u32 o = (u32)__shfl_up((int)inc, d, 64); if (lane >= (u32)d) inc += o; }
    if (lane == 63) wsum[wave] = inc;
    __syncthreads();
    u32 before = 0, all = 0;
    for (u32 w = 0; w < 16; w++) { const u32 v = wsum[w]; before += w < wave ? v : 0u; all += v; }
    u32 at = before + inc - mine;
    for (u32 k = 0; k < per; k++) {
        const u32 c = c0 + k;
        if (c >= q_rows) break;
        const bool on = slot[c] != 0;
        slot[c] = on ? at : ~0u;
        at += on ? 1u : 0u;
    }
    if (t == 0) { list[0] = all; list[1] = list[2] = list[3] = 0; }
}
__global__ __launch_bounds__(256) void k_prior_gather(const u32* __restrict__ rows66, u32 q_rows, const u32* __restrict__ slot, u32* __restrict__ list) {
    const u32 lane = threadIdx.x & 63;
    const u32 c = blockIdx.x * 4 + (threadIdx.x >> 6);
    if (c >= q_rows) return;
    const u32 s = slot[c];
    if (s == ~0u) return;
    const u32* r = rows66 + (size_t)c * 66;
    u32* o = list + 4 + (size_t)s * 67;
    if (lane == 0) o[0] = c;
    o[1 + lane] = r[lane];
    if (lane < 2) o[65 + lane] = r[64 + lane];
}
void launch_prior_list(const u32* rows66, u32 q_rows, u32* slot, u32* list, hipStream_t st) {
    hipLaunchKernelGGL(k_prior_flags, dim3((q_rows + 255) / 256), dim3(256), 0, st, rows66, q_rows, slot);
    hipLaunchKernelGGL(k_prior_slots, dim3(1), dim3(1024), 0, st, q_rows, slot, list);
    hipLaunchKernelGGL(k_prior_gather, dim3((q_rows + 3) / 4), dim3(256), 0, st, rows66, q_rows, (const u32*)slot, list);
}
void launch_prior_rows(const u32* hist, u32 q_rows, u32* rows66, u32* w_rows, u32* w_ovf, u32* l_slots, RowHdr* l_hdr, hipStream_t st) {
    hipLaunchKernelGGL(k_prior_rows, dim3((q_rows + 3) / 4), dim3(256), 0, st, hist, q_rows, rows66, w_rows, w_ovf, l_slots, l_hdr);
}

__global__ __launch_bounds__(256) void k_prior_spread(const u32* rows66, u32 q_rows, u32* w_rows, u32* w_ovf, u32* l_slots, RowHdr* l_hdr) {
    const u32 lane = threadIdx.x & 63;
    const u32 ctx = blockIdx.x * 4 + (threadIdx.x >> 6);
    if (ctx >= q_rows) return;
    const u32* r = rows66 + (size_t)ctx * 66;
    const u32 slot = r[lane], tot = r[64], iend = r[65];
    l_slots[(size_t)ctx * 64 + lane] = slot;
    if (lane == 0) { RowHdr h; h.total = tot; h.iend = (u16)iend; h.count = 0; h.pad = 0; h.epoch = 0; h.pad2 = 0; l_hdr[ctx] = h; }
    u32* w = w_rows + (size_t)ctx * 64;
    if (lane < 60) w[4 + lane] = slot; else w_ovf[(size_t)ctx * 4 + (lane - 60)] = slot;
    if (lane == 0) { w[0] = tot; w[1] = iend; w[2] = 0; w[3] = 0; }
}
__global__ __launch_bounds__(256) void k_prior_scatter(const u32* __restrict__ ctxs, const u32* __restrict__ rows, u32 n, u32* __restrict__ rows66) {
    const u32 i = blockIdx.x * 4 + (threadIdx.x >> 6), lane = threadIdx.x & 63;
    if (i >= n) return;
    u32* dst = rows66 + (size_t)ctxs[i] * 66;
    const u32* src = rows + (size_t)i * 66;
    dst[lane] = src[lane];
    if (lane < 2) dst[64 + lane] = src[64 + lane];
}
void launch_prior_scatter(const u32* ctxs, const u32* rows, u32 n, u32* rows66, hipStream_t st) {
    if (n) hipLaunchKernelGGL(k_prior_scatter, dim3((n + 3) / 4), dim3(256), 0, st, ctxs, rows, n, rows66);
}
void launch_prior_spread(const u32* rows66, u32 q_rows, u32* w_rows, u32* w_ovf, u32* l_slots, RowHdr* l_hdr, hipStream_t st) {
    hipLaunchKernelGGL(k_prior_spread, dim3((q_rows + 3) / 4), dim3(256), 0, st, rows66, q_rows, w_rows, w_ovf, l_slots, l_hdr);
}
```

Baseline: 330,800 MB/s.

## Fuse frozen prior row building and batch chain packing, overlap tail on side stream

After: 336,200 MB/s (median of 3 runs). About the same (+1.6%).

```diff
diff --git a/slimfastq_amd/csrc/api.cpp b/slimfastq_amd/csrc/api.cpp
--- a/slimfastq_amd/csrc/api.cpp
+++ b/slimfastq_amd/csrc/api.cpp
@@ -88,6 +88,9 @@
     EE_FRAME_K_END,
     EE_REC_FREQS_HOME,
     EE_REC_CODE_END,
+    EE_TAIL_FORK,
+    EE_SIZES_STAND,
+    EE_TAIL_SIDE_END,
     EE_COUNT
 };
 enum {
@@ -1195,6 +1198,11 @@
         }
     }
     u32* h_rows66 = nullptr;
+    auto hot_rows_wanted = [&](bool no_sample) -> u32 {
+        return (p.lds_rows == SFQ_LDS_ROWS_NONE || no_sample || !prior_step) ? 0u : p.lds_rows ? std::min<u32>(p.lds_rows, 1024u) : nchains >= 150000u ? 800u : 0u;
+    };
+    u32 want_hot = 0;
+    bool rows_fused = false;
     if (given && (models & SFQ_M_QLT)) {
         if ((rc = ensure_prior_buffers(ctx, q_rows))) return rc;
         if (!hist_cleared) HIPC(hipMemsetAsync(ctx->hist.p, 0, (size_t)q_rows * 64 * 4, st));
@@ -1220,6 +1228,20 @@
             return SFQ_OK;
         }
 
+        if (frozen) {
+            if ((rc = reserve(ctx, ctx->qrows, (size_t)q_rows * 64 * 4))) return rc;
+            want_hot = hot_rows_wanted(false);
+            u8* img = nullptr; u32* info = nullptr; u32* live = nullptr;
+            if (want_hot) {
+                const size_t img_bytes = (size_t)q_rows / 4 + (size_t)want_hot * 100 + 64;
+                if ((rc = reserve(ctx, ctx->qw, img_bytes + (size_t)q_rows * 8 + 256))) return rc;
+                img = (u8*)ctx->qw.p; info = (u32*)(img + ((img_bytes + 15) & ~(size_t)15)); live = info + 16;
+                HIPC(hipMemsetAsync(live, 0, 8, st));
+                ca.q_hot = want_hot; ca.qh_img = img; ca.qh_info = info;
+            }
+            launch_prior_frozen_rows((const u32*)ctx->hist.p, q_rows, (u32*)ctx->rows66.p, (u32*)ctx->qrows.p, want_hot, live, img, info, st);
+            rows_fused = true;
+        } else
         launch_prior_rows((const u32*)ctx->hist.p, q_rows, (u32*)ctx->rows66.p, (u32*)ctx->prior_w.p, (u32*)ctx->prior_wovf.p,
                           (u32*)ctx->prior_ls.p, (RowHdr*)ctx->prior_lh.p, st);
         if ((rc = reserve(ctx, ctx->pslot, (size_t)q_rows * 4))) return rc;
@@ -1236,20 +1258,14 @@
     }
     if (frozen) {
         if (models & SFQ_M_QLT) {
-            if ((rc = reserve(ctx, ctx->qrows, (size_t)q_rows * 64 * 4))) return rc;
             if ((rc = build_qesc(ctx, st))) return rc;
-            launch_qlt_frozen_rows((const u32*)ctx->rows66.p, q_rows, (u32*)ctx->qrows.p, nullptr, st);
+            if (!rows_fused) {
+                if ((rc = reserve(ctx, ctx->qrows, (size_t)q_rows * 64 * 4))) return rc;
+                launch_qlt_frozen_rows((const u32*)ctx->rows66.p, q_rows, (u32*)ctx->qrows.p, nullptr, st);
+                ca.q_hot = 0;
+            }
             ca.qrows = (const u32*)ctx->qrows.p; ca.qesc = (const u32*)ctx->qesc.p;
-            ca.q_hot = 0; ca.q_rows = q_rows;
-            const u32 want_hot = (p.lds_rows == SFQ_LDS_ROWS_NONE || given || !prior_step) ? 0u : p.lds_rows ? std::min<u32>(p.lds_rows, 1024u)
-                                 : nchains >= 150000u ? 800u : 0u;
-            if (want_hot) {
-                const size_t img_bytes = (size_t)q_rows / 4 + (size_t)want_hot * 100 + 64;
-                if ((rc = reserve(ctx, ctx->qw, img_bytes + (size_t)q_rows * 4 + 256))) return rc;
-                u8* img = (u8*)ctx->qw.p; u32* info = (u32*)(img + ((img_bytes + 15) & ~(size_t)15)); u32* ctot = info + 16;
-                launch_hot_rows((const u32*)ctx->hist.p, (const u32*)ctx->rows66.p, (const u32*)ctx->qrows.p, q_rows, want_hot, ctot, img, info, st);
-                ca.q_hot = want_hot; ca.qh_img = img; ca.qh_info = info;
-            }
+            ca.q_rows = q_rows;
             HIPC(hipEventRecord(ctx->ev[EE_HEAD_END], st));
         }
     }
@@ -1366,42 +1382,60 @@
 
     if ((rc = reserve(ctx, ctx->blk_stream_off, (size_t)nblocks * SFQ_NSTREAMS * 8))) return rc;
     if ((rc = reserve(ctx, ctx->stream_total, 2 * SFQ_NSTREAMS * 8 + 64))) return rc;
+    hipStream_t sst = mst[1];
+    HIPC(hipEventRecord(ctx->ev[EE_TAIL_FORK], st));
+    HIPC(hipStreamWaitEvent(sst, ctx->ev[EE_TAIL_FORK], 0));
     u32 chain_streams = 0;
+    ChainPackJobs jobs;
+    memset(&jobs, 0, sizeof jobs);
     if (frozen) {
         ca.m = a;
-        if (models & SFQ_M_QLT) { launch_chain_block_sizes(ca, ca.geo, SFQ_S_QLT, (const u32*)ctx->csz.p, nullptr, st); chain_streams |= 1u << SFQ_S_QLT; }
-        if (models & SFQ_M_GEN) { launch_chain_block_sizes(ca, ggeo, SFQ_S_GEN, gen_csz, nullptr, st); chain_streams |= 1u << SFQ_S_GEN; }
-        if (models & SFQ_M_REC) {
-            const u32* rs = (const u32*)ctx->csz.p + 2 * (size_t)nchains;
-            launch_chain_block_sizes(ca, ca.rgeo, SFQ_S_REC, rs, rs + nsub, st); chain_streams |= 1u << SFQ_S_REC;
-        }
+        auto job = [&](const ChainGeoArgs& geo, int stream, u32 num, u32 den, const u32* csz, const u32* rhb) {
+            ChainPackJob& j = jobs.j[jobs.n++];
+            j.geo = geo; j.stream = stream; j.num = num; j.den = den; j.csz = csz; j.rhb = rhb;
+            chain_streams |= 1u << stream;
+        };
+        const u32* rs = (const u32*)ctx->csz.p + 2 * (size_t)nchains;
+        if (models & SFQ_M_QLT) job(ca.geo, SFQ_S_QLT, 2, 1, (const u32*)ctx->csz.p, nullptr);
+        if (models & SFQ_M_GEN) job(ggeo, SFQ_S_GEN, 3, 4, gen_csz, nullptr);
+        if (models & SFQ_M_REC) job(ca.rgeo, SFQ_S_REC, 3, 2, rs, rs + nsub);
+        launch_chain_block_sizes(ca, jobs, st);
     }
     launch_block_stream_offsets((BlockDesc*)ctx->blocks.p, nblocks, (u64*)ctx->blk_stream_off.p, (u64*)ctx->stream_total.p, st);
+    u32* d_gate = (u32*)((u64*)ctx->stream_total.p + 2 * SFQ_NSTREAMS);
+    launch_stream_gate((const BlockDesc*)ctx->blocks.p, nblocks, (const u64*)ctx->stream_total.p, out_cap, (u64*)ctx->stream_total.p + SFQ_NSTREAMS, d_gate, st);
+    HIPC(hipEventRecord(ctx->ev[EE_SIZES_STAND], st));
+    launch_compact((const BlockDesc*)ctx->blocks.p, nblocks, (const u8*)ctx->arena.p, (const u64*)ctx->blk_stream_off.p,
+                   (const u64*)ctx->stream_total.p + SFQ_NSTREAMS, d_out, chain_streams, st, d_gate);
+    if (frozen) launch_compact_chains(ca, jobs, (const u64*)ctx->blk_stream_off.p, (const u64*)ctx->stream_total.p + SFQ_NSTREAMS, d_out, st, d_gate);
+
     if ((rc = reserve(ctx, ctx->lens, (size_t)nblocks * 4))) return rc;
     if ((rc = reserve(ctx, ctx->blob_off, ((size_t)nblocks + 1) * 8))) return rc;
     const u64 blob_cap = std::min<u64>(nbytes, (u64)nblocks * SFQ_MAX_ID_LLEN);
     if ((rc = reserve(ctx, ctx->blob, blob_cap))) return rc;
-    launch_first_hdr_lens((const BlockDesc*)ctx->blocks.p, nblocks, (u32*)ctx->lens.p, st);
-    launch_scan_u32((const u32*)ctx->lens.p, (u64*)ctx->blob_off.p, nblocks, (u64*)ctx->scan_tmp.p, st);
-    launch_gather_first_hdrs((const BlockDesc*)ctx->blocks.p, nblocks, d_fastq, (const u64*)ctx->blob_off.p, (u8*)ctx->blob.p, blob_cap, st);
-    const size_t p2_hb = 128, p2_off = p2_hb + (((size_t)nblocks * sizeof(BlockDesc) + 63) & ~(size_t)63);
-    const size_t p2_csz = p2_off + ((((size_t)nblocks + 1) * 8 + 63) & ~(size_t)63);
     const u32 ngc = frozen ? ggeo.nchains : 0;
     const bool gsplit = frozen && ngc != nchains;
     const size_t n_sizes = (size_t)nchains + ngc + (size_t)nsub * 2;
+    const bool rec_chains = (chain_streams >> SFQ_S_REC) & 1;
+    const u32 chn_n = frozen ? nchains + ngc + (rec_chains ? nsub * 2 : 0u) : 0u;
+    if ((rc = reserve(ctx, ctx->scan_tmp, ((size_t)std::max<u64>(chn_n, nblocks) / 1024 + 4) * 8 + 65536))) return rc;
+    launch_first_hdr_lens((const BlockDesc*)ctx->blocks.p, nblocks, (u32*)ctx->lens.p, sst);
+    launch_scan_u32((const u32*)ctx->lens.p, (u64*)ctx->blob_off.p, nblocks, (u64*)ctx->scan_tmp.p, sst);
+    launch_gather_first_hdrs((const BlockDesc*)ctx->blocks.p, nblocks, d_fastq, (const u64*)ctx->blob_off.p, (u8*)ctx->blob.p, blob_cap, sst);
+    const size_t p2_hb = 128, p2_off = p2_hb + (((size_t)nblocks * sizeof(BlockDesc) + 63) & ~(size_t)63);
+    const size_t p2_csz = p2_off + ((((size_t)nblocks + 1) * 8 + 63) & ~(size_t)63);
     const u32* d_sizes = (const u32*)ctx->csz.p;
     if (gsplit) {
         if ((rc = reserve(ctx, ctx->gm_idx, n_sizes * 4 + 64))) return rc;
         u32* di = (u32*)ctx->gm_idx.p;
-        HIPC(hipMemcpyAsync(di, ctx->csz.p, (size_t)nchains * 4, hipMemcpyDeviceToDevice, st));
-        HIPC(hipMemcpyAsync(di + nchains, ctx->gm_csz.p, (size_t)ngc * 4, hipMemcpyDeviceToDevice, st));
-        HIPC(hipMemcpyAsync(di + nchains + ngc, (const u32*)ctx->csz.p + 2 * (size_t)nchains, (size_t)nsub * 2 * 4, hipMemcpyDeviceToDevice, st));
+        HIPC(hipMemcpyAsync(di, ctx->csz.p, (size_t)nchains * 4, hipMemcpyDeviceToDevice, sst));
+        HIPC(hipMemcpyAsync(di + nchains, ctx->gm_csz.p, (size_t)ngc * 4, hipMemcpyDeviceToDevice, sst));
+        HIPC(hipMemcpyAsync(di + nchains + ngc, (const u32*)ctx->csz.p + 2 * (size_t)nchains, (size_t)nsub * 2 * 4, hipMemcpyDeviceToDevice, sst));
         d_sizes = di;
     }
     const size_t p2_end = p2_csz + n_sizes * 4 + 64;
     if ((rc = reserve_pinned_buf(ctx, ctx->pin2, ctx->pin2_cap, p2_end))) return rc;
     u64* totals = (u64*)ctx->pin2;
-    HIPC(hipMemcpyAsync(totals, ctx->stream_total.p, SFQ_NSTREAMS * 8, hipMemcpyDeviceToHost, st));
     auto pack_prior_now = [&]() -> int {
         if (ctx->prior_on && !given && h_rows66) {
             if ((rc = qlt_prior_blob_now(ctx, h_rows66, q_rows, mst[2]))) return rc;
@@ -1412,44 +1446,34 @@
     BlockDesc* hb = (BlockDesc*)((u8*)ctx->pin2 + p2_hb);
     u64* hboff = (u64*)((u8*)ctx->pin2 + p2_off);
     u32* h_csz = (u32*)((u8*)ctx->pin2 + p2_csz);
-    const bool rec_chains = (chain_streams >> SFQ_S_REC) & 1;
-    const u32 chn_n = frozen ? nchains + ngc + (rec_chains ? nsub * 2 : 0u) : 0u;
     const size_t chn_eager = std::min<size_t>((size_t)chn_n * 5, n_sizes * 4 + 64 - 16);
-    u32* d_gate = (u32*)((u64*)ctx->stream_total.p + 2 * SFQ_NSTREAMS);
     const u64 blob_guess = std::min<u64>(blob_cap, (u64)nblocks * 256);
-    launch_stream_gate((const BlockDesc*)ctx->blocks.p, nblocks, (const u64*)ctx->stream_total.p, out_cap, (u64*)ctx->stream_total.p + SFQ_NSTREAMS, d_gate, st);
-    launch_compact((const BlockDesc*)ctx->blocks.p, nblocks, (const u8*)ctx->arena.p, (const u64*)ctx->blk_stream_off.p,
-                   (const u64*)ctx->stream_total.p + SFQ_NSTREAMS, d_out, chain_streams, st, d_gate);
     if (frozen) {
-        if (chain_streams & (1u << SFQ_S_QLT))
-            launch_compact_chains(ca, ca.geo, SFQ_S_QLT, 2, 1, (const u32*)ctx->csz.p, (const u64*)ctx->blk_stream_off.p, (const u64*)ctx->stream_total.p + SFQ_NSTREAMS, d_out, st, d_gate);
-        if (chain_streams & (1u << SFQ_S_GEN))
-            launch_compact_chains(ca, ggeo, SFQ_S_GEN, 3, 4, gen_csz, (const u64*)ctx->blk_stream_off.p, (const u64*)ctx->stream_total.p + SFQ_NSTREAMS, d_out, st, d_gate);
-        if (chain_streams & (1u << SFQ_S_REC))
-            launch_compact_chains(ca, ca.rgeo, SFQ_S_REC, 3, 2, (const u32*)ctx->csz.p + 2 * (size_t)nchains, (const u64*)ctx->blk_stream_off.p, (const u64*)ctx->stream_total.p + SFQ_NSTREAMS, d_out, st, d_gate);
-        {
-            const u32 b1 = nchains, b2 = nchains + ngc, b3 = rec_chains ? nchains + ngc + nsub : chn_n;
-            if ((rc = reserve(ctx, ctx->chn_len, (size_t)chn_n * 4 + 16))) return rc;
-            if ((rc = reserve(ctx, ctx->chn_off, ((size_t)chn_n + 4) * 8))) return rc;
-            if ((rc = reserve(ctx, ctx->chn_out, (size_t)chn_n * 5 + 64))) return rc;
-            if ((rc = reserve(ctx, ctx->scan_tmp, ((size_t)chn_n / 1024 + 4) * 8 + 65536))) return rc;
-            u64* d_info = (u64*)ctx->chn_off.p + chn_n + 1;
-            launch_chain_index_bytes(d_sizes, chn_n, b1, b2 > chn_n ? chn_n : b2, b3, (u32*)ctx->chn_len.p, (u64*)ctx->chn_off.p, (u64*)ctx->scan_tmp.p,
-                                     (u8*)ctx->chn_out.p, d_info, st);
-            HIPC(hipMemcpyAsync(h_csz, d_info, 16, hipMemcpyDeviceToHost, st));
-            if (chn_eager) HIPC(hipMemcpyAsync((u8*)h_csz + 16, ctx->chn_out.p, chn_eager, hipMemcpyDeviceToHost, st));
-        }
-    }
+        const u32 b1 = nchains, b2 = nchains + ngc, b3 = rec_chains ? nchains + ngc + nsub : chn_n;
+        if ((rc = reserve(ctx, ctx->chn_len, (size_t)chn_n * 4 + 16))) return rc;
+        if ((rc = reserve(ctx, ctx->chn_off, ((size_t)chn_n + 4) * 8))) return rc;
+        if ((rc = reserve(ctx, ctx->chn_out, (size_t)chn_n * 5 + 64))) return rc;
+        u64* d_info = (u64*)ctx->chn_off.p + chn_n + 1;
+        launch_chain_index_bytes(d_sizes, chn_n, b1, b2 > chn_n ? chn_n : b2, b3, (u32*)ctx->chn_len.p, (u64*)ctx->chn_off.p, (u64*)ctx->scan_tmp.p,
+                                 (u8*)ctx->chn_out.p, d_info, sst);
+        HIPC(hipMemcpyAsync(h_csz, d_info, 16, hipMemcpyDeviceToHost, sst));
+        if (chn_eager) HIPC(hipMemcpyAsync((u8*)h_csz + 16, ctx->chn_out.p, chn_eager, hipMemcpyDeviceToHost, sst));
+    }
+    HIPC(hipMemcpyAsync(hboff, ctx->blob_off.p, ((size_t)nblocks + 1) * 8, hipMemcpyDeviceToHost, sst));
+    HIPC(hipStreamWaitEvent(sst, ctx->ev[EE_SIZES_STAND], 0));
+    HIPC(hipMemcpyAsync(totals, ctx->stream_total.p, SFQ_NSTREAMS * 8, hipMemcpyDeviceToHost, sst));
+    HIPC(hipMemcpyAsync(hb, ctx->blocks.p, (size_t)nblocks * sizeof(BlockDesc), hipMemcpyDeviceToHost, sst));
+    HIPC(hipEventRecord(ctx->ev[EE_TAIL_SIDE_END], sst));
+    HIPC(hipStreamWaitEvent(st, ctx->ev[EE_TAIL_SIDE_END], 0));
     HIPC(hipEventRecord(ctx->ev[EE_PACK_END], st));
     if ((rc = pack_prior_now())) return rc;
     ctx->first_hdrs.resize((size_t)blob_guess);
-    if (blob_guess) HIPC(hipMemcpyAsync(ctx->first_hdrs.data(), ctx->blob.p, (size_t)blob_guess, hipMemcpyDeviceToHost, st));
-    HIPC(hipMemcpyAsync(hb, ctx->blocks.p, (size_t)nblocks * sizeof(BlockDesc), hipMemcpyDeviceToHost, st));
-    HIPC(hipMemcpyAsync(hboff, ctx->blob_off.p, ((size_t)nblocks + 1) * 8, hipMemcpyDeviceToHost, st));
+    if (blob_guess) HIPC(hipMemcpyAsync(ctx->first_hdrs.data(), ctx->blob.p, (size_t)blob_guess, hipMemcpyDeviceToHost, sst));
     ht.mark("packing queued");
     if ((rc = pack_prior_now())) return rc;
     ht.mark("priors packed");
     HIPC(hipStreamSynchronize(st));
+    HIPC(hipStreamSynchronize(sst));
     ht.mark("device through");
     u64 bases[SFQ_NSTREAMS], run = 0;
     for (int s = 0; s < SFQ_NSTREAMS; s++) { bases[s] = run; run += totals[s]; res->stream_bytes[s] = totals[s]; res->stream_offset[s] = bases[s]; }
diff --git a/slimfastq_amd/csrc/chains.hip b/slimfastq_amd/csrc/chains.hip
--- a/slimfastq_amd/csrc/chains.hip
+++ b/slimfastq_amd/csrc/chains.hip
@@ -1,6 +1,7 @@
 #include "kernels.h"
 #include "dev_chain.h"
 #include "dev_walk.h"
+#include "dev_prior.h"
 typedef u32 __attribute__((aligned(1))) u32_any;
 
 #define LAST_QLT 63u
@@ -24,26 +25,10 @@
         if (qdec) qdec_store(qdec + (size_t)ctx * QDEC_ROW, lane, lane << 10);
         return;
     }
-    const u32 sym = slot >> 16, fslot = lane < iend ? (slot & 0xffffu) : 0u;
-    const u32 f = (u32)__builtin_amdgcn_ds_permute((int)((lane < iend ? sym : lane) * 4), (int)fslot);
-    const u32 x = f + 1;
-    u32 S = x;
-#pragma unroll
-    for (int d = 32; d > 0; d >>= 1) S += (u32)__shfl_xor((int)S, d, 64);
-    u32 g = (x << 16) / S;
-    g = g ? g : 1u;
-    u32 sum = g, best = (g << 6) | (63u - lane);
-#pragma unroll
-    for (int d = 32; d > 0; d >>= 1) {
-        sum += (u32)__shfl_xor((int)sum, d, 64);
-        const u32 o = (u32)__shfl_xor((int)best, d, 64); best = o > best ? o : best;
-    }
-    if (lane == 63u - (best & 63u)) g += 65536u - sum;
-    u32 incl = g;
-#pragma unroll
-    for (int d = 1; d < 64; d <<= 1) { const u32 o = (u32)__shfl_up((int)incl, d, 64); if (lane >= (u32)d) incl += o; }
-    qrows[(size_t)ctx * 64 + lane] = (incl - g) | (g << 16);
-    if (qdec) qdec_store(qdec + (size_t)ctx * QDEC_ROW, lane, incl - g);
+    u32 g;
+    const u32 cum = frozen_entry_of(slot, iend, lane, g);
+    qrows[(size_t)ctx * 64 + lane] = cum | (g << 16);
+    if (qdec) qdec_store(qdec + (size_t)ctx * QDEC_ROW, lane, cum);
 }
 void launch_qlt_frozen_rows(const u32* rows66, u32 q_rows, u32* qrows, u16* qdec, hipStream_t st) {
     hipLaunchKernelGGL(k_qlt_frozen_rows, dim3((q_rows + 3) / 4), dim3(256), 0, st, rows66, q_rows, qrows, qdec);
@@ -53,15 +38,48 @@
 #define QH_ROW_U16 50u
 #define QH_MAP_BYTES(q_rows) ((q_rows) / 32u * 8u)
 #define QH_EMPTY 0xFFFFFFFFu
-__global__ __launch_bounds__(256) void k_hot_totals(const u32* __restrict__ hist, const u32* __restrict__ rows66, u32 q_rows, u32* __restrict__ ctot) {
+__global__ __launch_bounds__(256) void k_prior_frozen_rows(const u32* __restrict__ hist, u32 q_rows, u32* __restrict__ rows66, u32* __restrict__ qrows,
+                                                           u32* __restrict__ live) {
     const u32 lane = threadIdx.x & 63;
     const u32 ctx = blockIdx.x * 4 + (threadIdx.x >> 6);
     if (ctx >= q_rows) return;
-    u32 c = hist[(size_t)ctx * 64 + lane];
-#pragma unroll
-    for (int d = 32; d > 0; d >>= 1) c += (u32)__shfl_xor((int)c, d, 64);
-    const u32 iend = rows66[(size_t)ctx * 66 + 65];
-    if (lane == 0) ctot[ctx] = (iend != 0 && iend <= QH_SYMS) ? c : 0u;
+    u32* r = rows66 + (size_t)ctx * 66;
+    const u32 c = hist[(size_t)ctx * 64 + lane];
+    if (!__ballot(c != 0)) {
+        r[lane] = 0;
+        if (lane < 2) r[64 + lane] = 0;
+        qrows[(size_t)ctx * 64 + lane] = (lane << 10) | (1024u << 16);
+        return;
+    }
+    u32 tot, iend, g;
+    const u32 slot = prior_row_of(c, lane, tot, iend);
+    r[lane] = slot;
+    if (lane == 0) { r[64] = tot; r[65] = iend; }
+    const u32 cum = frozen_entry_of(slot, iend, lane, g);
+    qrows[(size_t)ctx * 64 + lane] = cum | (g << 16);
+    if (live && iend <= QH_SYMS) {
+        u32 n = c;
+#pragma unroll
+        for (int d = 32; d > 0; d >>= 1) n += (u32)__shfl_xor((int)n, d, 64);
+        if (lane == 0) { const u32 at = atomicAdd(live, 1u); live[2 + 2 * (size_t)at] = ctx; live[3 + 2 * (size_t)at] = n; }
+    }
+}
+__device__ __forceinline__ void hot_map_write(const u32* wbits, u32* red, u32 nwords, uint2* __restrict__ map, u32* __restrict__ info) {
+    const u32 t = threadIdx.x, lane = t & 63, wave = t >> 6;
+    const u32 b0 = 2u * t < nwords ? wbits[2u * t] : 0u, b1 = 2u * t + 1u < nwords ? wbits[2u * t + 1u] : 0u;
+    const u32 mine = (u32)__popc(b0) + (u32)__popc(b1);
+    u32 inc = mine;
+#pragma unroll
+    for (int d = 1; d < 64; d <<= 1) { const u32 o = (u32)__shfl_up((int)inc, d, 64); if (lane >= (u32)d) inc += o; }
+    __syncthreads();
+    if (lane == 63) red[wave] = inc;
+    __syncthreads();
+    u32 before = 0, all = 0;
+    for (u32 w = 0; w < 16; w++) { const u32 v = red[w]; before += w < wave ? v : 0u; all += v; }
+    const u32 rank = before + inc - mine;
+    if (t == 0) info[0] = all;
+    if (2u * t < nwords) map[2u * t] = make_uint2(b0, rank);
+    if (2u * t + 1u < nwords) map[2u * t + 1u] = make_uint2(b1, rank + (u32)__popc(b0));
 }
 __global__ __launch_bounds__(1024) void k_hot_select(const u32* __restrict__ ctot, u32 q_rows, u32 want, uint2* __restrict__ map, u32* __restrict__ info) {
     __shared__ u32 red[16];
@@ -111,20 +129,62 @@
         if (lane == 0) { wbits[k * 32u + wave * 2u] = (u32)m; wbits[k * 32u + wave * 2u + 1u] = (u32)(m >> 32); }
     }
     __syncthreads();
-    const u32 b0 = 2u * t < nwords ? wbits[2u * t] : 0u, b1 = 2u * t + 1u < nwords ? wbits[2u * t + 1u] : 0u;
-    const u32 mine = (u32)__popc(b0) + (u32)__popc(b1);
-    u32 inc = mine;
-#pragma unroll
-    for (int d = 1; d < 64; d <<= 1) { const u32 o = (u32)__shfl_up((int)inc, d, 64); if (lane >= (u32)d) inc += o; }
+    hot_map_write(wbits, red, nwords, map, info);
+}
+#define QH_LIVE_REGS 8u
+__global__ __launch_bounds__(1024) void k_hot_select_live(const u32* __restrict__ live, u32 q_rows, u32 want, uint2* __restrict__ map, u32* __restrict__ info) {
+    __shared__ u32 red[16];
+    __shared__ u32 wbits[2048];
+    const u32 t = threadIdx.x, lane = t & 63, wave = t >> 6;
+    const u32 nwords = q_rows / 32u;
+    const u32 n = live[0] < q_rows ? live[0] : q_rows;
+    const uint2* __restrict__ e = reinterpret_cast<const uint2*>(live + 2);
+    for (u32 i = t; i < 2048u; i += 1024u) wbits[i] = 0;
+    u32 c[QH_LIVE_REGS], cx[QH_LIVE_REGS];
+    u32 mx = 0;
+#pragma unroll
+    for (u32 k = 0; k < QH_LIVE_REGS; k++) {
+        const u32 i = k * 1024u + t;
+        const uint2 v = i < n ? e[i] : make_uint2(0u, 0u);
+        cx[k] = v.x; c[k] = v.y;
+        mx = c[k] > mx ? c[k] : mx;
+    }
+    for (u32 i = QH_LIVE_REGS * 1024u + t; i < n; i += 1024u) { const u32 v = e[i].y; mx = v > mx ? v : mx; }
+    auto block_sum = [&](u32 v) {
+#pragma unroll
+        for (int d = 32; d > 0; d >>= 1) v += (u32)__shfl_xor((int)v, d, 64);
+        __syncthreads();
+        if (lane == 0) red[wave] = v;
+        __syncthreads();
+        u32 s2 = 0;
+        for (u32 w = 0; w < 16; w++) s2 += red[w];
+        return s2;
+    };
+    auto block_max = [&](u32 v) {
+#pragma unroll
+        for (int d = 32; d > 0; d >>= 1) { const u32 o = (u32)__shfl_xor((int)v, d, 64); v = o > v ? o : v; }
+        __syncthreads();
+        if (lane == 0) red[wave] = v;
+        __syncthreads();
+        u32 s2 = 0;
+        for (u32 w = 0; w < 16; w++) s2 = red[w] > s2 ? red[w] : s2;
+        return s2;
+    };
+    u32 lo = 1, hi = block_max(mx) + 1u;
+    while (lo < hi) {
+        const u32 mid = lo + (hi - lo) / 2u;
+        u32 m = 0;
+#pragma unroll
+        for (u32 k = 0; k < QH_LIVE_REGS; k++) m += c[k] >= mid;
+        for (u32 i = QH_LIVE_REGS * 1024u + t; i < n; i += 1024u) m += e[i].y >= mid;
+        if (block_sum(m) <= want) hi = mid; else lo = mid + 1u;
+    }
+    const u32 T = lo;
+#pragma unroll
+    for (u32 k = 0; k < QH_LIVE_REGS; k++) if (c[k] >= T && cx[k] < q_rows) atomicOr(&wbits[cx[k] >> 5], 1u << (cx[k] & 31u));
+    for (u32 i = QH_LIVE_REGS * 1024u + t; i < n; i += 1024u) { const uint2 v = e[i]; if (v.y >= T && v.x < q_rows) atomicOr(&wbits[v.x >> 5], 1u << (v.x & 31u)); }
     __syncthreads();
-    if (lane == 63) red[wave] = inc;
-    __syncthreads();
-    u32 before = 0, all = 0;
-    for (u32 w = 0; w < 16; w++) { const u32 v = red[w]; before += w < wave ? v : 0u; all += v; }
-    const u32 rank = before + inc - mine;
-    if (t == 0) info[0] = all;
-    if (2u * t < nwords) map[2u * t] = make_uint2(b0, rank);
-    if (2u * t + 1u < nwords) map[2u * t + 1u] = make_uint2(b1, rank + (u32)__popc(b0));
+    hot_map_write(wbits, red, nwords, map, info);
 }
 __global__ __launch_bounds__(256) void k_hot_image(const uint2* __restrict__ map, const u32* __restrict__ qrows, u32 q_rows, u16* __restrict__ rows) {
     const u32 lane = threadIdx.x & 63;
@@ -136,10 +196,11 @@
     const u32 slot = mr.y + (u32)__popc(mr.x & (bit - 1u));
     if (lane < QH_ROW_U16) rows[(size_t)slot * QH_ROW_U16 + lane] = lane <= QH_SYMS ? (u16)FZ_CUM(qrows[(size_t)ctx * 64 + lane]) : (u16)0;
 }
-void launch_hot_rows(const u32* hist, const u32* rows66, const u32* qrows, u32 q_rows, u32 want, u32* ctot, u8* img, u32* info, hipStream_t st) {
-    hipLaunchKernelGGL(k_hot_totals, dim3((q_rows + 3) / 4), dim3(256), 0, st, hist, rows66, q_rows, ctot);
-    hipLaunchKernelGGL(k_hot_select, dim3(1), dim3(1024), 0, st, (const u32*)ctot, q_rows, want, reinterpret_cast<uint2*>(img), info);
-    hipLaunchKernelGGL(k_hot_image, dim3((q_rows + 3) / 4), dim3(256), 0, st, reinterpret_cast<const uint2*>(img), qrows, q_rows,
+void launch_prior_frozen_rows(const u32* hist, u32 q_rows, u32* rows66, u32* qrows, u32 want, u32* live, u8* img, u32* info, hipStream_t st) {
+    hipLaunchKernelGGL(k_prior_frozen_rows, dim3((q_rows + 3) / 4), dim3(256), 0, st, hist, q_rows, rows66, qrows, want ? live : nullptr);
+    if (!want) return;
+    hipLaunchKernelGGL(k_hot_select_live, dim3(1), dim3(1024), 0, st, (const u32*)live, q_rows, want, reinterpret_cast<uint2*>(img), info);
+    hipLaunchKernelGGL(k_hot_image, dim3((q_rows + 3) / 4), dim3(256), 0, st, reinterpret_cast<const uint2*>(img), (const u32*)qrows, q_rows,
                        reinterpret_cast<u16*>(img + QH_MAP_BYTES(q_rows)));
 }
 
@@ -434,7 +495,11 @@
     }
 }
 
-__global__ __launch_bounds__(256) void k_chain_block_sizes(ChainArgs a, ChainGeoArgs geo, int stream, const u32* csz, const u32* rhb) {
+__global__ __launch_bounds__(256) void k_chain_block_sizes(ChainArgs a, ChainPackJobs jobs) {
+    const ChainPackJob& j = jobs.j[blockIdx.y];
+    const ChainGeoArgs geo = j.geo;
+    const int stream = j.stream;
+    const u32* csz = j.csz; const u32* rhb = j.rhb;
     const u32 b = blockIdx.x * 4 + (threadIdx.x >> 6), lane = threadIdx.x & 63;
     if (b >= a.m.nblocks) return;
     u32 sum = 0, hb = 0;
@@ -450,11 +515,15 @@
         if (rhb) a.m.blocks[b].hdr_bytes = hb;
     }
 }
-void launch_chain_block_sizes(const ChainArgs& a, const ChainGeoArgs& geo, int stream, const u32* csz, const u32* rhb, hipStream_t st) {
-    hipLaunchKernelGGL(k_chain_block_sizes, dim3((a.m.nblocks + 3) / 4), dim3(256), 0, st, a, geo, stream, csz, rhb);
-}
-__global__ __launch_bounds__(256) void k_compact_chains(ChainArgs a, ChainGeoArgs geo, int stream, u32 num, u32 den, const u32* csz,
-                                                        const u64* blk_stream_off, const u64* stream_base, u8* out, const u32* gate) {
+void launch_chain_block_sizes(const ChainArgs& a, const ChainPackJobs& jobs, hipStream_t st) {
+    if (jobs.n) hipLaunchKernelGGL(k_chain_block_sizes, dim3((a.m.nblocks + 3) / 4, jobs.n), dim3(256), 0, st, a, jobs);
+}
+__global__ __launch_bounds__(256) void k_compact_chains(ChainArgs a, ChainPackJobs jobs, const u64* blk_stream_off, const u64* stream_base, u8* out, const u32* gate) {
+    const ChainPackJob& j = jobs.j[blockIdx.y];
+    const ChainGeoArgs geo = j.geo;
+    const int stream = j.stream;
+    const u32 num = j.num, den = j.den;
+    const u32* csz = j.csz;
     const u32 c = blockIdx.x * 4 + (threadIdx.x >> 6), lane = threadIdx.x & 63;
     if (c >= geo.nchains) return;
     if (gate && !gate[0]) return;
@@ -480,9 +549,10 @@
     }
     for (u32 i = (n16 << 4) + lane; i < n; i += 64) dst[i] = src[i];
 }
-void launch_compact_chains(const ChainArgs& a, const ChainGeoArgs& geo, int stream, u32 num, u32 den, const u32* csz, const u64* blk_stream_off,
-                           const u64* stream_base, u8* out, hipStream_t st, const u32* gate) {
-    hipLaunchKernelGGL(k_compact_chains, dim3((geo.nchains + 3) / 4), dim3(256), 0, st, a, geo, stream, num, den, csz, blk_stream_off, stream_base, out, gate);
+void launch_compact_chains(const ChainArgs& a, const ChainPackJobs& jobs, const u64* blk_stream_off, const u64* stream_base, u8* out, hipStream_t st, const u32* gate) {
+    u32 widest = 0;
+    for (u32 k = 0; k < jobs.n; k++) widest = jobs.j[k].geo.nchains > widest ? jobs.j[k].geo.nchains : widest;
+    if (widest) hipLaunchKernelGGL(k_compact_chains, dim3((widest + 3) / 4, jobs.n), dim3(256), 0, st, a, jobs, blk_stream_off, stream_base, out, gate);
 }
 
 template <typename LOOK, typename CODE>
diff --git a/slimfastq_amd/csrc/dev_prior.h b/slimfastq_amd/csrc/dev_prior.h
--- /dev/null
+++ b/slimfastq_amd/csrc/dev_prior.h
@@ -0,0 +1,55 @@
+#pragma once
+#include "dev_common.h"
+
+__device__ __forceinline__ u32 pr_sort64(u32 key, u32 lane) {
+#pragma unroll
+    for (u32 k = 2; k <= 64; k <<= 1) {
+#pragma unroll
+        for (u32 j = k >> 1; j > 0; j >>= 1) {
+            const u32 other = (u32)__shfl_xor((int)key, j, 64);
+            const bool up = (lane & k) == 0, lower = (lane & j) == 0;
+            const u32 lo = key < other ? key : other, hi = key < other ? other : key;
+            key = (lower == up) ? lo : hi;
+        }
+    }
+    return key;
+}
+__device__ __forceinline__ u32 prior_row_of(u32 c, u32 lane, u32& tot, u32& iend) {
+    const u64 seen = __ballot(c != 0);
+    iend = seen ? 64u - (u32)__clzll((long long)seen) : 0u;
+    u32 mx = c;
+#pragma unroll
+    for (int dd = 32; dd > 0; dd >>= 1) { const u32 o = (u32)__shfl_xor((int)mx, dd, 64); mx = o > mx ? o : mx; }
+    u32 sh = 0;
+    while ((((u64)mx * 6) >> sh) > 32000) sh++;
+    const u32 fq = (u32)(((u64)c * 6) >> sh);
+    const u32 key = lane < iend ? (((0xFFFFu - fq) << 6) | lane) : (0xFFFFFFC0u | lane);
+    const u32 sk = pr_sort64(key, lane);
+    const u32 f = lane < iend ? 0xFFFFu - (sk >> 6) : 0u;
+    const u32 sym = sk & 63u;
+    tot = lane < iend ? f : 0u;
+#pragma unroll
+    for (int d = 32; d > 0; d >>= 1) tot += (u32)__shfl_xor((int)tot, d, 64);
+    return lane < iend ? (f | (sym << 16)) : 0u;
+}
+__device__ __forceinline__ u32 frozen_entry_of(u32 slot, u32 iend, u32 lane, u32& g) {
+    const u32 sym = slot >> 16, fslot = lane < iend ? (slot & 0xffffu) : 0u;
+    const u32 f = (u32)__builtin_amdgcn_ds_permute((int)((lane < iend ? sym : lane) * 4), (int)fslot);
+    const u32 x = f + 1;
+    u32 S = x;
+#pragma unroll
+    for (int d = 32; d > 0; d >>= 1) S += (u32)__shfl_xor((int)S, d, 64);
+    g = (x << 16) / S;
+    g = g ? g : 1u;
+    u32 sum = g, best = (g << 6) | (63u - lane);
+#pragma unroll
+    for (int d = 32; d > 0; d >>= 1) {
+        sum += (u32)__shfl_xor((int)sum, d, 64);
+        const u32 o = (u32)__shfl_xor((int)best, d, 64); best = o > best ? o : best;
+    }
+    if (lane == 63u - (best & 63u)) g += 65536u - sum;
+    u32 incl = g;
+#pragma unroll
+    for (int d = 1; d < 64; d <<= 1) { const u32 o = (u32)__shfl_up((int)incl, d, 64); if (lane >= (u32)d) incl += o; }
+    return incl - g;
+}
diff --git a/slimfastq_amd/csrc/kernels.h b/slimfastq_amd/csrc/kernels.h
--- a/slimfastq_amd/csrc/kernels.h
+++ b/slimfastq_amd/csrc/kernels.h
@@ -74,8 +74,8 @@
     u32 flat_quads;
     u32 flat_raw;
 };
-void launch_hot_rows(const u32* hist, const u32* rows66, const u32* qrows, u32 q_rows, u32 want, u32* ctot ,
-                     u8* img , u32* info, hipStream_t st);
+void launch_prior_frozen_rows(const u32* hist, u32 q_rows, u32* rows66, u32* qrows, u32 want, u32* live ,
+                              u8* img , u32* info, hipStream_t st);
 void launch_hot_rows_dec(const u32* rows66, const u16* qdec, u32 q_rows, u32 want, u32* ctot ,
                          u8* img , u32* info, hipStream_t st);
 u32 hot_rows_dec_max(void);
@@ -130,9 +130,11 @@
 void launch_seg_count(const u64* line_off, const BlockDesc* blocks, u32 block_reads, u64 nrec, u32 seg_len, u32* nseg, hipStream_t st);
 void launch_seg_count_dec(const u32* slen, const u32* qlen, u64 nrec, u32 seg_len, u32* nseg, hipStream_t st);
 void launch_seg_fill(const u64* seg_off, u64 nrec, u32* seg_rec, hipStream_t st);
-void launch_chain_block_sizes(const ChainArgs& a, const ChainGeoArgs& geo, int stream, const u32* csz, const u32* rhb , hipStream_t st);
-void launch_compact_chains(const ChainArgs& a, const ChainGeoArgs& geo, int stream, u32 num, u32 den, const u32* csz, const u64* blk_stream_off,
-                           const u64* stream_base, u8* out, hipStream_t st, const u32* gate );
+struct ChainPackJob { ChainGeoArgs geo; int stream; u32 num, den ; const u32* csz; const u32* rhb ; };
+struct ChainPackJobs { u32 n; ChainPackJob j[3]; };
+void launch_chain_block_sizes(const ChainArgs& a, const ChainPackJobs& jobs, hipStream_t st);
+void launch_compact_chains(const ChainArgs& a, const ChainPackJobs& jobs, const u64* blk_stream_off, const u64* stream_base, u8* out, hipStream_t st,
+                           const u32* gate );
 #define GEN_STEP 4u
 #ifndef GEN_COUNT_CAP
 #define GEN_COUNT_CAP 524288ull
diff --git a/slimfastq_amd/csrc/prior.hip b/slimfastq_amd/csrc/prior.hip
--- a/slimfastq_amd/csrc/prior.hip
+++ b/slimfastq_amd/csrc/prior.hip
@@ -1,5 +1,6 @@
 #include "kernels.h"
 #include "dev_wave.h"
+#include "dev_prior.h"
 
 __device__ __forceinline__ u32 p_calc_last_delta(u32& delta, u32 q, u32 q1, u32 q2) {
     if (q1 > q) delta += q1 - q;
@@ -140,41 +141,13 @@
     }
 }
 
-__device__ __forceinline__ u32 pr_sort64(u32 key, u32 lane) {
-#pragma unroll
-    for (u32 k = 2; k <= 64; k <<= 1) {
-#pragma unroll
-        for (u32 j = k >> 1; j > 0; j >>= 1) {
-            const u32 other = (u32)__shfl_xor((int)key, j, 64);
-            const bool up = (lane & k) == 0, lower = (lane & j) == 0;
-            const u32 lo = key < other ? key : other, hi = key < other ? other : key;
-            key = (lower == up) ? lo : hi;
-        }
-    }
-    return key;
-}
 __global__ __launch_bounds__(256) void k_prior_rows(const u32* hist, u32 q_rows, u32* rows66, u32* w_rows, u32* w_ovf,
                                                    u32* l_slots, RowHdr* l_hdr) {
     const u32 lane = threadIdx.x & 63;
     const u32 ctx = blockIdx.x * 4 + (threadIdx.x >> 6);
     if (ctx >= q_rows) return;
-    const u32 c = hist[(size_t)ctx * 64 + lane];
-    const u64 seen = __ballot(c != 0);
-    const u32 iend = seen ? 64u - (u32)__clzll((long long)seen) : 0u;
-    u32 mx = c;
-#pragma unroll
-    for (int dd = 32; dd > 0; dd >>= 1) { const u32 o = (u32)__shfl_xor((int)mx, dd, 64); mx = o > mx ? o : mx; }
-    u32 sh = 0;
-    while ((((u64)mx * 6) >> sh) > 32000) sh++;
-    const u32 fq = (u32)(((u64)c * 6) >> sh);
-    const u32 key = lane < iend ? (((0xFFFFu - fq) << 6) | lane) : (0xFFFFFFC0u | lane);
-    const u32 sk = pr_sort64(key, lane);
-    const u32 f = lane < iend ? 0xFFFFu - (sk >> 6) : 0u;
-    const u32 sym = sk & 63u;
-    const u32 slot = lane < iend ? (f | (sym << 16)) : 0u;
-    u32 tot = lane < iend ? f : 0u;
-#pragma unroll
-    for (int d = 32; d > 0; d >>= 1) tot += (u32)__shfl_xor((int)tot, d, 64);
+    u32 tot, iend;
+    const u32 slot = prior_row_of(hist[(size_t)ctx * 64 + lane], lane, tot, iend);
     u32* r = rows66 + (size_t)ctx * 66;
     r[lane] = slot;
     if (lane == 0) { r[64] = tot; r[65] = iend; }
```
